# amazon-science/gnn-tail-generalization

Hardware: AMD Instinct MI355X
Metric: teachergnn_fullgraph_train_steps_per_sec (higher is better)
Workload: dtype f32

## Files before the change

gnn-tail-generalization_amd/_lib.py:

```python
import ctypes
import os

import torch

_HERE = os.path.dirname(os.path.abspath(__file__))
LIB_PATH = os.path.join(_HERE, 'lib', 'libcoldbrew_hip.so')

_c_i32p = ctypes.c_void_p
_c_f32p = ctypes.c_void_p
_I64 = ctypes.c_int64
_I32 = ctypes.c_int32
_SZ = ctypes.c_size_t
_P = ctypes.c_void_p


class CsrView(ctypes.Structure):
    _fields_ = [('rowptr', _P), ('col', _P), ('col_flags', _I32), ('n_rows', _I64), ('n_edges', _I64),
                ('hub_threshold', _I32), ('n_hubs', _I32), ('n_chunks', _I32), ('hub_rows', _P), ('hub_chunk_ptr', _P),
                ('ws', _P), ('ws_bytes', _SZ)]


class TrunkStore(ctypes.Structure):
    _fields_ = [('mix_src', _P), ('ld_mix', _I64), ('mix_index', _P), ('c_act', ctypes.c_float), ('c_mix', ctypes.c_float), ('drop_p', ctypes.c_float),
                ('seed', ctypes.c_uint64), ('seed_dev', _P), ('row0', _I64), ('relu_bits', _P), ('bits_relu_only', _I32), ('out_act', _P), ('ld_act', _I64)]


_G = ctypes.POINTER(CsrView)
_S = ctypes.POINTER(TrunkStore)

SIGNATURES = {
    'cb_version': (ctypes.c_int, []),
    'cb_last_error': (ctypes.c_char_p, []),
    'cb_device_status': (ctypes.c_int, []),
    'cb_agg_gemm_handover_selftest': (ctypes.c_int, [_P]),
    'cb_rows_zero_outside_mask_f32': (ctypes.c_int, [_P, _I64, _I64, _I64, _P, _P, _P]),
    'cb_csr_workspace_bytes': (_SZ, [_I64, _I64]),
    'cb_csr_from_coo_i64': (ctypes.c_int, [_P, _P, _I64, _I64, _P, _P, _P, _P, _P, _P, _SZ, _P]),
    'cb_deg_norm_f32': (ctypes.c_int, [_P, _I64, _P, _P]),
    'cb_csr64_from_coo_i64': (ctypes.c_int, [_P, _P, _I64, _I64, _P, _P, _P, _P, _P, _P, _SZ, _P]),
    'cb_csr_rebase_i64': (ctypes.c_int, [_P, _I64, _I64, _P, _P]),
    'cb_deg_norm_i64ptr_f32': (ctypes.c_int, [_P, _I64, _P, _P]),
    'cb_spmm_hub_count': (ctypes.c_int, [_P, _I64, _I32, _P, _P]),
    'cb_spmm_hub_fill_scratch_ints': (_I64, [_I64]),
    'cb_spmm_hub_fill': (ctypes.c_int, [_P, _I64, _I32, _I32, _P, _P, _P, _P]),
    'cb_spmm_workspace_bytes': (_SZ, [_I64, _I64]),
    'cb_spmm_csr_f32': (ctypes.c_int, [_G, _P, _I32, _I64, _I64, _P, _P, _P, ctypes.c_int, _P, _I64, _P, _I64, _P]),
    'cb_dropout_f32': (ctypes.c_int, [_P, _P, _I64, ctypes.c_float, ctypes.c_uint64, _P, _I64, _P]),
    'cb_axpby_f32': (ctypes.c_int, [ctypes.c_float, _P, ctypes.c_float, _P, _P, _I64, _P]),
    'cb_colsum_workspace_bytes': (_SZ, [_I64, _I64]),
    'cb_act_bwd_f32': (ctypes.c_int, [_P, _P, _P, _P, _I64, _I64, _P, _P, _SZ, _P]),
    'cb_reduce_workspace_bytes': (_SZ, []),
    'cb_frobenius_norm_f32': (ctypes.c_int, [_P, _I64, _P, _P, _SZ, _P]),
    'cb_nll_logsoftmax_f32': (ctypes.c_int, [_P, _I64, _P, _P, _I64, _I64, _I64, _P, _P, _P, _SZ, _P]),
    'cb_adam_step_f32': (ctypes.c_int, [_P, _P, _P, _P, _I64, ctypes.c_float, ctypes.c_float, ctypes.c_float,
                                        ctypes.c_float, ctypes.c_float, _I64, _P, _P]),
    'cb_adam_multi_f32': (ctypes.c_int, [_I32, _P, _P, _P, _P, _P, _P, ctypes.c_float, ctypes.c_float, ctypes.c_float, ctypes.c_float,
                                         ctypes.c_float, _I64, _P, _P, _P]),
    'cb_gemm_nn_workspace_bytes': (_SZ, [_I64, _I64]),
    'cb_gemm_nn_splitk_workspace_bytes': (_SZ, [_I64, _I64, _I64]),
    'cb_gemm_nn_f32': (ctypes.c_int, [_P, _I64, _P, _I64, _P, _I64, _I64, _I64, _I64, _P, _P, _I64, _P, ctypes.c_int, _P, _SZ, _P]),
    'cb_gemm_nn_drop2_f32': (ctypes.c_int, [_P, _I64, _P, _I64, _P, _I64, _P, _I64, _I64, _I64, _I64, _P, _P, _I64, _P, ctypes.c_int,
                                            ctypes.c_float, ctypes.c_uint64, _P, _I64, _P, _SZ, _P]),
    'cb_gemm_tn_workspace_bytes': (_SZ, [_I64, _I64, _I64]),
    'cb_gemm_tn_f32': (ctypes.c_int, [_P, _I64, _P, _I64, _P, _P, _I64, _I64, _I64, _P, _SZ, _P]),
    'cb_spmm_csr_fused_f32': (ctypes.c_int, [_G, _P, _P, _I32, _I64, _I64, _P, _P, _P, _I64, _S, _P, _I64, _P]),
    'cb_trunk_layer_bwd_f32': (ctypes.c_int, [_P, _P, _P, _P, ctypes.c_int, _P, ctypes.c_int, _I64, _I64, ctypes.c_float, ctypes.c_uint64,
                                              _P, _I64, ctypes.c_float, ctypes.c_float, _P, ctypes.c_uint64, ctypes.c_float, _P, _P, _P, _SZ, _P]),
    'cb_gemm_nn_bf16out_f32': (ctypes.c_int, [_P, _I64, _P, _I64, _P, _I64, _I64, _I64, _I64, _P, _P, _I64, _P, ctypes.c_int, _P, _SZ, _P]),
    'cb_node_norm_fwd_f32': (ctypes.c_int, [_P, _P, _P, _I64, _I64, ctypes.c_float, ctypes.c_float, ctypes.c_float, _P]),
    'cb_node_norm_bwd_f32': (ctypes.c_int, [_P, _P, _P, _P, _I64, _I64, ctypes.c_float, ctypes.c_float, _P]),
    'cb_colstats_workspace_bytes': (_SZ, [_I64, _I64]),
    'cb_colstats_f32': (ctypes.c_int, [_P, _P, _P, _I64, _I64, _P, _P, _P, _SZ, _P]),
    'cb_col_affine_f32': (ctypes.c_int, [_P, _P, _P, _P, ctypes.c_float, _P, _I64, _I64, _P]),
    'cb_col_bwd_combine_f32': (ctypes.c_int, [_P, _P, _P, _P, _P, _P, ctypes.c_float, ctypes.c_float, _P, _I64, _I64, _P]),
    'cb_topk_replace_workspace_bytes': (_SZ, [_I64, _I64, _I64]),
    'cb_topk_replace_f32': (ctypes.c_int, [_P, _I64, _P, _I64, _I64, _I64, _I64, _I32, _P, _P, _P, _P, _SZ, _P]),
    'cb_gather_rows_f32': (ctypes.c_int, [_P, _I64, _P, _I64, _I64, _P, _P]),
    'cb_gather_rows_bf16_f32': (ctypes.c_int, [_P, _I64, _P, _I64, _I64, _P, _P]),
    'cb_adam_norm_workspace_bytes': (ctypes.c_size_t, [_I32]),
    'cb_adam_multi_norm_f32': (ctypes.c_int, [_I32, _P, _P, _P, _P, _P, _P, _P, ctypes.c_float, ctypes.c_float, ctypes.c_float, ctypes.c_float,
                                              ctypes.c_float, _I64, _P, _P, _P, _SZ, _P]),
    'cb_expand_rows_f32': (ctypes.c_int, [_P, _P, _I64, _I64, ctypes.c_float, _P, _P]),
    'cb_gemm_nn_store_rows_supported': (ctypes.c_int, [_P, _I64, _P, _I64, _P, _I64, _I64, _I64, _I64]),
    'cb_gemm_nn_store_rows_f32': (ctypes.c_int, [_P, _I64, _P, _I64, _P, _I64, _I64, _I64, _I64, _P, _P, _I64, _P, _P, _S, _P, _SZ, _P]),
    'cb_trunk_store_rows_f32': (ctypes.c_int, [_P, _P, _I64, _I64, _S, _P, _P]),
    'cb_agg_gemm_image_bytes': (_SZ, [_I64, _I64]),
    'cb_agg_gemm_image_f32': (ctypes.c_int, [_P, _I64, _I64, _I64, ctypes.c_int, _P, _SZ, _P]),
    'cb_spmm_gemm_f32': (ctypes.c_int, [_G, _P, _I64, _I64, _P, _P, ctypes.c_int, _P, _I64, _P, _I64, _P, _P, _P, _I64, _P, _I64, _P]),
    'cb_spmm_gemm_fused_f32': (ctypes.c_int, [_G, _P, _I64, _P, _I64, _I64, _P, _P, _S, _P, _I64, _I32, _P, _P, _P, _I64, _P, _I64, _P]),
    'cb_agg_gemm_head_image_bytes': (_SZ, [_I64, _I64]),
    'cb_agg_gemm_head_image_f32': (ctypes.c_int, [_P, _I64, _I64, _I64, ctypes.c_int, _P, _SZ, _P]),
    'cb_spmm_gemm_fused_head_f32': (ctypes.c_int, [_G, _P, _I64, _P, _I64, _I64, _P, _P, _S, _P, _I64, _I32, _P, _P, _I64, _P, _I64, _P]),
    'cb_spmm_gemm_store_rows_f32': (ctypes.c_int, [_G, _P, _I64, _I64, _P, _P, _I64, _P, _P, _P, _P, _S, _P, _I64, _P]),
    'cb_spmm_csr_weighted_f32': (ctypes.c_int, [_P, _P, _P, _I64, _I64, _P, _I64, _I64, _P, _P, ctypes.c_int, _P, _I64, _P]),
    'cb_spmm_edge_dot_f32': (ctypes.c_int, [_P, _P, _I64, _I64, _P, _I64, _P, _I64, _I64, _P, _P]),
    'cb_gemm_nn_indrop_supported': (ctypes.c_int, [_P, _I64, _P, _I64, _P, _I64, _P, _I64, _I64, _I64, _I64]),
    'cb_gemm_nn_indrop_drop2_f32': (ctypes.c_int, [_P, _I64, _P, _I64, _P, _I64, _P, _I64, _I64, _I64, _I64, _P, ctypes.c_int, ctypes.c_float,
                                                   ctypes.c_uint64, ctypes.c_float, ctypes.c_uint64, _P, _I64, _P, _P]),
    'cb_gemm_nn_indrop_f32': (ctypes.c_int, [_P, _I64, _P, _I64, _P, _I64, _I64, _I64, _I64, _P, _P, _I64, _P, ctypes.c_int, ctypes.c_float,
                                             ctypes.c_uint64, _P, _I64, _P, _P]),
    'cb_gemm_tn_adrop_supported': (ctypes.c_int, [_P, _I64, _P, _I64, _I64, _I64]),
    'cb_gemm_tn_adrop_f32': (ctypes.c_int, [_P, _I64, _P, _I64, _P, _P, _I64, _I64, _I64, ctypes.c_float, ctypes.c_uint64, _P, _I64, _P, _SZ, _P]),
    'cb_front_image_bytes': (_SZ, [_I64]),
    'cb_front_image_f32': (ctypes.c_int, [_P, _I64, _I64, ctypes.c_int, _P, _SZ, _P]),
    'cb_trunk_front_f32': (ctypes.c_int, [_P, _I64, _I64, _I64, _P, _P, _P, _P, _P, _I64, _P, _I64, _P, _P, _I64, _P, _I64, ctypes.c_float,
                                          ctypes.c_uint64, ctypes.c_uint64, _P, _I64, _P]),
    'cb_gemm_tn_gdrop_supported': (ctypes.c_int, [_P, _I64, _P, _I64, _I64, _I64]),
    'cb_gemm_tn_gdrop_f32': (ctypes.c_int, [_P, _I64, _P, _I64, _P, _I64, _I64, _I64, ctypes.c_float, ctypes.c_uint64, _P, _I64, _P, _SZ, _P]),
    'cb_spmm_csr_lp_f32': (ctypes.c_int, [_G, _P, _I64, _I64, _P, _P, _I64, ctypes.c_float, _P, _P, _I64, _P]),
    'cb_spmm_csr_prop_f32': (ctypes.c_int, [_G, _P, _I64, _I64, _P, _P, _I64, ctypes.c_float, ctypes.c_float, ctypes.c_float, _P, _P, _P, _I64, _P]),
    'cb_cs_workspace_bytes': (_SZ, [_I64, _I64]),
    'cb_cs_residual_init_f32': (ctypes.c_int, [_P, _I64, _P, _P, _I64, _I64, _I64, _P, _P, _P, _P, _P, _SZ, _P]),
    'cb_cs_correct_snap_f32': (ctypes.c_int, [_I32, _P, _I64, _P, _I64, _P, _P, _I64, _I64, _I64, _P, _I64, ctypes.c_float, _P, _P, _I64, _P, _P, _P]),
    'cb_trunk_input_bwd_multi_f32': (ctypes.c_int, [_P, ctypes.c_uint64, _I32, _P, _P, ctypes.c_float, _P, _P, _I64, _I64, ctypes.c_float,
                                                    _P, _I64, _P, _P, _SZ, _P, _P, _P]),
    'cb_trunk_input_bwd_multi_cs_f32': (ctypes.c_int, [_P, ctypes.c_uint64, _I32, _P, _P, ctypes.c_float, _P, _P, _I64, _I64, ctypes.c_float,
                                                       _P, _I64, _P, _P, _SZ, _P, _P, _I32, _P, _P, _P, _P, _P, _SZ, _P]),
    'cb_spmm_csr_store_bwd_f32': (ctypes.c_int, [_G, _P, _I64, _I64, _P, _P, _P, ctypes.c_float, ctypes.c_float, ctypes.c_uint64, _P, _I64, _P, _I64, _P, _I64, _P]),
    'cb_spmm_store_bwd_mix_workspace_bytes': (_SZ, [_I64, _I64, _I64]),
    'cb_spmm_csr_store_bwd_mix_f32': (ctypes.c_int, [_G, _P, _I64, _I64, _P, _P, _P, ctypes.c_float, ctypes.c_float, ctypes.c_uint64, _P, _I64, _P, _I64, _P, _I64,
                                                     _I32, _P, _P, _P, ctypes.c_float, _P, _P, _SZ, _P]),
    'cb_gemm_tn_instage_supported': (ctypes.c_int, [_P, _P, _P, _I64, _I64, _I64]),
    'cb_gemm_tn_instage_workspace_bytes': (_SZ, [_I64, _I64]),
    'cb_gemm_tn_instage_f32': (ctypes.c_int, [_P, _P, _P, _P, _I64, _P, _P, _I64, _I64, ctypes.c_float, ctypes.c_uint64, ctypes.c_float, ctypes.c_uint64, _P, _I64,
                                              _P, _SZ, _P]),
    'cb_trunk_layer_bwd_fold_f32': (ctypes.c_int, [_P, _P, _P, _P, _I64, _I64, ctypes.c_float, ctypes.c_uint64, _P, _I64, ctypes.c_float, ctypes.c_float, _I32, _P, _P, _P,
                                                   _P, _P, _P, _SZ, _I32, _P, ctypes.c_float, _P, _P, _SZ, _P]),
    'cb_trunk_layer_bwd_rows_f32': (ctypes.c_int, [_P, _P, _I64, _P, _P, _P, _I64, ctypes.c_float, ctypes.c_uint64, _P, _I64, ctypes.c_float,
                                                   _P, ctypes.c_uint64, ctypes.c_float, _P, _P, _P, _SZ, _P]),
    'cb_id_count_i64': (ctypes.c_int, [_P, _I64, _I64, _P, _P, _P]),
    'cb_value_hist_i32': (ctypes.c_int, [_P, _I64, _I32, _P, _P, _P]),
    'cb_compact_workspace_bytes': (_SZ, [_I64]),
    'cb_select_range_i32': (ctypes.c_int, [_P, _I64, _I32, _I32, _P, _P, _P, _P, _SZ, _P]),
    'cb_craft_isolation_i64': (ctypes.c_int, [_P, _P, _I64, _P, _I64, _P, _P, _P, _P, _SZ, _P]),
    'cb_symmetrize_workspace_bytes': (_SZ, [_I64, _I64]),
    'cb_symmetrize_i64': (ctypes.c_int, [_P, _P, _I64, _I64, _P, _P, _P, _P, _P, _SZ, _P]),
    'cb_trunk_input_bwd_f32': (ctypes.c_int, [_P, _P, _P, _P, _I64, _I64, ctypes.c_float, ctypes.c_uint64, _P, _I64, _P, _P, _SZ, _P]),
    'cb_ln_gelu_drop_fwd_f32': (ctypes.c_int, [_P, _I64, _I64, _P, _P, ctypes.c_float, ctypes.c_float, ctypes.c_uint64, _P, _P, _P, _P]),
    'cb_ln_gelu_drop_bwd_workspace_bytes': (_SZ, [_I64, _I64]),
    'cb_ln_gelu_drop_bwd_f32': (ctypes.c_int, [_P, _P, _P, _I64, _I64, _P, _P, ctypes.c_float, ctypes.c_uint64, _P, _P, _P, _P, _P, _P, _SZ, _P]),
    'cb_mse_rows_f32': (ctypes.c_int, [_P, _I64, _I64, _P, _I64, _I64, _P, _P, _P, _P, _SZ, _P]),
    'cb_part2_assemble_f32': (ctypes.c_int, [_P, _I64, _P, _P, _I64, _P, _I64, _P, _P]),
    'cb_part2_assemble_bwd_f32': (ctypes.c_int, [_P, _I64, _P, _P, _I64, _I64, _P, _P, _SZ, _P]),
    'cb_ncloss_positions_i64': (ctypes.c_int, [_P, _I64, _I64, _P, _P, _P]),
    'cb_ncloss_row_norms_f32': (ctypes.c_int, [_P, _I64, _I64, _I64, _P, _P, _P]),
    'cb_cosine_scale_f32': (ctypes.c_int, [_P, _I64, _I64, _P, _P]),
    'cb_ncloss_uses_limb_core': (ctypes.c_int, [_P, _I64, _I64]),
    'cb_ncloss_workspace_bytes': (_SZ, [_I64, _I32]),
    'cb_ncloss_fwd_f32': (ctypes.c_int, [_P, _I64, _I64, _I64, ctypes.c_float, _P, _P, _P, _I64, _P, _P, _P, _I32, _P, _P, _P, _P, _P, _P, _P, _P, _SZ, _P]),
    'cb_ncloss_normalize_rows_f32': (ctypes.c_int, [_P, _I64, _I64, _I64, _P, _P, _P]),
    'cb_ncloss_bwd_slab_f32': (ctypes.c_int, [_P, _I64, _I64, _I64, ctypes.c_float, _P, _P, _I64, _I64, _I32, _P, _I64, _P]),
    'cb_ncloss_bwd_finish_f32': (ctypes.c_int, [_P, _I64, _P, _I64, _I64, ctypes.c_float, _P, _P, _P, _P, _P, _P, _P, _P, _I64, _P, _P, _P, _P, _P, _P, _P]),
    'cb_spgemm_offsets_workspace_bytes': (_SZ, [_I64]),
    'cb_spgemm_entry_offsets_i64': (ctypes.c_int, [_P, _I64, _P, _I64, _P, _P, _P, _SZ, _P]),
    'cb_spgemm_chunk_workspace_bytes': (_SZ, [_I64]),
    'cb_spgemm_chunk_count_f32': (ctypes.c_int, [_P, _P, _P, _P, _P, _P, _P, _I64, _I64, _I64, _I64, _I64, _P, _P, _SZ, _P]),
    'cb_spgemm_chunk_emit_f32': (ctypes.c_int, [_P, _SZ, _I64, _I64, _I64, _I64, _I64, _I64, _P, _P, _P, _P]),
    'cb_csr_transpose_workspace_bytes': (_SZ, [_I64]),
    'cb_csr_transpose_f32': (ctypes.c_int, [_P, _P, _P, _I64, _I64, _I64, _P, _P, _P, _P, _SZ, _P]),
    'cb_linkp_max_tries': (ctypes.c_int, []),
    'cb_linkp_valid_counts_i32': (ctypes.c_int, [_P, _P, _I32, _P, _P]),
    'cb_linkp_positives_i32': (ctypes.c_int, [_P, _P, _I32, _P, _I64, _I64, ctypes.c_uint64, _P, _P, _P]),
    'cb_linkp_negatives_i32': (ctypes.c_int, [_P, _P, _I32, _P, _I64, _I64, ctypes.c_uint64, _P, _P, _P, _P]),
    'cb_linkp_loss_fwd_f32': (ctypes.c_int, [_P, _I64, _I64, _I64, _P, _I64, _P, _I64, _P, _P, _P, _P, _P]),
    'cb_linkp_mrr_f32': (ctypes.c_int, [_P, _I64, _P, _I64, _P, _P]),
    'cb_linkp_bwd_workspace_bytes': (_SZ, [_I64, _I64]),
    'cb_linkp_loss_bwd_f32': (ctypes.c_int, [_P, _I64, _I64, _I64, _P, _I64, _P, _I64, _P, _P, _P, _I64, _P, _SZ, _P]),
    'cb_heur_aa_weights_f64': (ctypes.c_int, [_P, _P, _P]),
    'cb_heur_pair_scores_f32': (ctypes.c_int, [_P, _P, _P, _I64, _P, _P, _P]),
    'cb_heur_pair_scores_width_f32': (ctypes.c_int, [_P, _P, _P, _I64, _I32, _P, _P, _P]),
    'cb_rank_counts_workspace_bytes': (_SZ, [_I64, _I64]),
    'cb_rank_counts_f32': (ctypes.c_int, [_P, _I64, _P, _I64, _P, _P, _P, _P, _SZ, _P]),
    'cb_pair_gemm_nn_supported': (ctypes.c_int, [_P, _I64, _P, _I64, _I64, _I64]),
    'cb_pair_gemm_nn_f32': (ctypes.c_int, [_P, _I64, _I64, _P, _I64, _P, _I64, _P, _I64, _P, _I64, _I64, _I64, _P, ctypes.c_int, ctypes.c_float,
                                           ctypes.c_uint64, _P, _I64, _P, _P]),
    'cb_pair_dot_f32': (ctypes.c_int, [_P, _I64, _I64, _I64, _P, _I64, _P, _P, _P]),
    'cb_pair_scatter_workspace_bytes': (_SZ, [_I64]),
    'cb_pair_scatter_f32': (ctypes.c_int, [_P, _I64, _I64, _I64, _P, _I64, _P, _I64, _P, _I64, _P, _SZ, _P]),
    'cb_rank_loss_workspace_bytes': (_SZ, []),
    'cb_rank_loss_fwd_f32': (ctypes.c_int, [_I32, _P, _I64, _P, _I64, _P, _P, _P, _SZ, _P]),
    'cb_rank_loss_bwd_f32': (ctypes.c_int, [_I32, _P, _I64, _P, _I64, _P, _P, _P, _P, _P]),
    'cb_sage_image_bytes': (_SZ, [ctypes.c_int]),
    'cb_sage_image_f32': (ctypes.c_int, [_P, _I64, _P, _I64, ctypes.c_int, _P, _SZ, _P]),
    'cb_sage_layer_supported': (ctypes.c_int, [_I64, _I64, _I32, _P, _I64, _P, _I64, _P, _I64, _P, _I64]),
    'cb_sage_layer_f32': (ctypes.c_int, [_P, _P, _I64, _P, _I64, _P, _P, _P, _P, ctypes.c_int, ctypes.c_float, ctypes.c_uint64, _P, _I64, _P, _I64, _I32,
                                         _P, _I64, _P]),
}

_lib = None


class HipExtensionError(RuntimeError):
    pass


def load():
    global _lib
    if _lib is not None:
        return _lib
    if not os.path.isfile(LIB_PATH):
        raise HipExtensionError(
            f'{LIB_PATH} not found: the HIP extension is required (no CPU fallback). '
            'Build it with `python __graft_entry__.py` or `make -C gnn-tail-generalization_amd/csrc`.')
    lib = ctypes.CDLL(LIB_PATH)
    for name, (res, args) in SIGNATURES.items():
        fn = getattr(lib, name)
        fn.restype = res
        fn.argtypes = args
# ... 69 lines not shown
```

gnn-tail-generalization_amd/csrc/cb_front.hip:

```cpp
#include <type_traits>

#include "cb_common.h"
#include "cb_limb_core.h"
#include "cb_philox.h"
#include "cb_tile_gemm.h"
#include "cb_trunk_store.h"

namespace cb {

struct FrontArgs {
  const float* x;
  int64_t ld_x;
  const uint4* image_in;
  const float* bias_in;
  const uint4* image_0;
  const float* rowscale;
  const float* addend;
  int64_t ld_add;
  float* x0;
  int64_t ld_x0;
  unsigned long long* bits;
  float* x0_drop;
  int64_t ld_drop;
  float* z0;
  int64_t ld_z;
  int64_t M;
  uint32_t thresh;
  float keep_scale;
  uint64_t seed_x, seed_x0;
  const uint64_t* seed_dev;
  int64_t row0;
  int n_tiles;
};

template <int NS1, bool DROP>
__global__ void __launch_bounds__(256, 2) k_front(FrontArgs fa) {
  constexpr int K1 = 16 * NS1, LDX = K1 + 4, NV = kTM * K1 / 4 / 256;
  static_assert(NV >= 1 && kTM * LDX <= kTM * kTLD, "x tile must fit the region of the X0 tile");
  static_assert(NV == NS1 && NS1 <= 8, "mask draws: one quad per K step, P0's bits in one word");
  __shared__ __attribute__((aligned(16))) float tile[kTM * kTLD];
  constexpr int kScratch = 2 * RowOperand<kTM>::BYTES > 4 * 8 * kCLD * 4 ? 2 * RowOperand<kTM>::BYTES : 4 * 8 * kCLD * 4;
  __shared__ __attribute__((aligned(16))) char scratch[kScratch];
  float (*cstrip)[8 * kCLD] = reinterpret_cast<float (*)[8 * kCLD]>(scratch);
  __shared__ float rs_tile[2][kTM];
  const int t = threadIdx.x, lane = t & 63, w = __builtin_amdgcn_readfirstlane(t >> 6);
  const uint64_t sx = fa.seed_dev ? fa.seed_x + *fa.seed_dev : fa.seed_x, s0 = fa.seed_dev ? fa.seed_x0 + *fa.seed_dev : fa.seed_x0;
  float4 xr[NV];
  auto load_x = [&](int tile_id) {
    const int64_t m0 = (int64_t)tile_id * kTM;
#pragma unroll
    for (int j = 0; j < NV; ++j) {
      const int idx = t + 256 * j, row = idx / (K1 / 4), c4 = idx % (K1 / 4);
      const int64_t m = m0 + row;
      xr[j] = (tile_id < fa.n_tiles && m < fa.M) ? *reinterpret_cast<const float4*>(fa.x + m * fa.ld_x + 4 * c4) : make_float4(0.f, 0.f, 0.f, 0.f);
    }
  };
  float rs_next = 1.f;
  auto load_rs = [&](int tile_id) {
    const int64_t m = (int64_t)tile_id * kTM + t;
    rs_next = (t < kTM && fa.rowscale && tile_id < fa.n_tiles && m < fa.M) ? fa.rowscale[m] : 1.f;
  };
  float bvec[4] = {0.f, 0.f, 0.f, 0.f};
  if (fa.bias_in) {
#pragma unroll
    for (int i = 0; i < 4; ++i) bvec[i] = fa.bias_in[4 * lane + i];
  }
  load_rs(blockIdx.x);
  load_x(blockIdx.x);
  uint32_t kx = 0;
  uint64_t k3 = 0;
  int64_t qx = 0, q3 = 0;
  auto aim_x = [&](int tile_id) { qx = (fa.row0 + (int64_t)tile_id * kTM) * (K1 / 4) + t; };
  auto aim_3 = [&](int tile_id) { q3 = (fa.row0 + (int64_t)tile_id * kTM + 16 * w) * (kND / 4) + lane; };
  auto draw_x = [&](int) {
    uint64_t seed = sx;
    asm volatile("" : "+s"(seed));
    kx = (kx >> 4) | (keep4_bits(seed, qx, fa.thresh) << 28);
    qx += 256;
    asm volatile("" : "+v"(kx));
  };
  auto draw_3 = [&](int) {
    uint64_t seed = s0;
    asm volatile("" : "+s"(seed));
    k3 = (k3 >> 4) | ((uint64_t)keep4_bits(seed, q3, fa.thresh) << 60);
    q3 += kND / 4;
    asm volatile("" : "+v"(k3));
  };
  if constexpr (DROP) {
    aim_x(blockIdx.x);
    aim_3(blockIdx.x);
#pragma unroll 1
    for (int s = 0; s < 16; ++s) {
      if (s < NS1) draw_x(s);
      draw_3(s);
    }
  }
  int par = 0;
  for (int tile_id = blockIdx.x; tile_id < fa.n_tiles; tile_id += gridDim.x, par ^= 1) {
    const int64_t m0 = (int64_t)tile_id * kTM;
#pragma unroll
    for (int j = 0; j < NV; ++j) {
      const int idx = t + 256 * j, row = idx / (K1 / 4), c4 = idx % (K1 / 4);
      float v[4] = {xr[j].x, xr[j].y, xr[j].z, xr[j].w};
      if constexpr (DROP) {
#pragma unroll
        for (int i = 0; i < 4; ++i) v[i] = mul_rounded(v[i], (kx >> (32 - 4 * NV + 4 * j + i)) & 1u ? fa.keep_scale : 0.f);
      }
      *reinterpret_cast<float4*>(tile + row * LDX + 4 * c4) = make_float4(v[0], v[1], v[2], v[3]);
    }
    if constexpr (DROP) aim_x(tile_id + (int)gridDim.x);
    if (t < kTM) rs_tile[par][t] = rs_next;
    __syncthreads();
    f32x16 acc[2][2];
    if constexpr (DROP) tile_times_image_coop<NS1, LDX, 1>(tile, scratch, fa.image_in, w, lane, t, acc, draw_x);
    else tile_times_image_coop<NS1, LDX, 1>(tile, scratch, fa.image_in, w, lane, t, acc);
    {
      const int l31 = lane & 31, lh = lane >> 5;
#pragma unroll
      for (int i = 0; i < 2; ++i)
#pragma unroll
        for (int j = 0; j < 2; ++j)
#pragma unroll
          for (int reg = 0; reg < 16; ++reg)
            tile[(32 * i + (reg & 3) + 8 * (reg >> 2) + 4 * lh) * kTLD + 64 * w + 32 * j + l31] = acc[i][j][reg];
    }
    __syncthreads();
#pragma unroll 4
    for (int r = 0; r < 16; ++r) {
      const int row = 16 * w + r;
      const int64_t m = m0 + row;
      float* tp = tile + row * kTLD + 4 * lane;
      const float4 v = *reinterpret_cast<const float4*>(tp);
      float o[4] = {v.x, v.y, v.z, v.w};
#pragma unroll
      for (int i = 0; i < 4; ++i) o[i] = fmaxf(o[i] + bvec[i], 0.f);
      float xd[4] = {o[0], o[1], o[2], o[3]};
      if constexpr (DROP) {
#pragma unroll
        for (int i = 0; i < 4; ++i) xd[i] = o[i] * ((uint32_t)k3 >> i & 1u ? fa.keep_scale : 0.f);
        k3 >>= 4;
      }
      *reinterpret_cast<float4*>(tp) = make_float4(xd[0], xd[1], xd[2], xd[3]);
      if (m < fa.M) {
        store_stream4(fa.x0 + m * fa.ld_x0 + 4 * lane, o);
        if (fa.bits) {
          const bool pos[4] = {o[0] > 0.f, o[1] > 0.f, o[2] > 0.f, o[3] > 0.f};
          write_row_mask_words(fa.bits + m * 4, lane, pos);
        }
        if (fa.x0_drop) store_stream4(fa.x0_drop + m * fa.ld_drop + 4 * lane, xd);
      }
    }
    __syncthreads();
    if constexpr (DROP) aim_3(tile_id + (int)gridDim.x);
    if constexpr (DROP) tile_times_image_coop<kNS, kTLD, 1>(tile, scratch, fa.image_0, w, lane, t, acc, draw_3);
    else tile_times_image_coop<kNS, kTLD, 1>(tile, scratch, fa.image_0, w, lane, t, acc);
    load_rs(tile_id + gridDim.x);
    load_x(tile_id + gridDim.x);
    auto z0_epilogue = [&](auto HAS_ADD) {
      acc_rows_through_strip(acc, cstrip[w], w, lane, [&](int row, int n, const float4& v) {
        const int64_t m = m0 + row;
        if (m < fa.M) {
          const float rs = rs_tile[par][row];
          float ad[4] = {0.f, 0.f, 0.f, 0.f};
          if constexpr (decltype(HAS_ADD)::value) {
            const float4 a4 = *reinterpret_cast<const float4*>(fa.addend + m * fa.ld_add + n);
            ad[0] = a4.x; ad[1] = a4.y; ad[2] = a4.z; ad[3] = a4.w;
          }
          const float zero_bias = 0.f;
          float o[4] = {v.x, v.y, v.z, v.w};
#pragma unroll
          for (int e = 0; e < 4; ++e) o[e] = o[e] * rs + ad[e] + zero_bias;
          store_stream4(fa.z0 + m * fa.ld_z + n, o);
        }
      });
    };
    if (fa.addend) z0_epilogue(std::true_type{});
    else z0_epilogue(std::false_type{});
  }
}

}

using namespace cb;

extern "C" size_t cb_front_image_bytes(int64_t K) {
  if (K != 64 && K != 128) return 0;
  return (size_t)(K / 16) * kNT * 3 * 64 * sizeof(uint4);
}

extern "C" int cb_front_image_f32(const float* W, int64_t ld, int64_t K, int transpose, void* image, size_t image_bytes, void* stream) {
  CB_CHECK_ARG(cb_front_image_bytes(K) > 0, CB_E_INVALID, "cb_front_image_f32: K must be 64 or 128 (got %lld)", (long long)K);
  CB_CHECK_ARG(W && image && ld >= (transpose ? K : kND), CB_E_INVALID, "cb_front_image_f32: null pointer / bad leading dimension");
  CB_CHECK_ARG(image_bytes >= cb_front_image_bytes(K) && aligned16(image), CB_E_WORKSPACE, "cb_front_image_f32: image buffer too small or misaligned");
  const int64_t sk = transpose ? 1 : ld, sn = transpose ? ld : 1;
  const int ns = (int)(K / 16);
  hipLaunchKernelGGL(k_weight_image, dim3(ns * kNT * 64 / 256), dim3(256), 0, (hipStream_t)stream, W, sk, sn, (uint4*)image, ns);
  CB_LAUNCH_CHECK();
  return CB_OK;
}

extern "C" int cb_trunk_front_f32(const float* x, int64_t ld_x, int64_t M, int64_t K, const void* image_in, const float* bias_in, const void* image_0,
                                  const float* rowscale, const float* addend, int64_t ld_add, float* x0, int64_t ld_x0, uint64_t* relu_bits,
                                  float* x0_drop, int64_t ld_drop, float* z0, int64_t ld_z, float drop_p, uint64_t seed_x, uint64_t seed_x0,
                                  const uint64_t* seed_dev, int64_t row0, void* stream) {
  CB_CHECK_ARG(M >= 0 && cb_front_image_bytes(K) > 0 && drop_p >= 0.f && drop_p < 1.f && row0 >= 0, CB_E_INVALID,
               "cb_trunk_front_f32: bad size (K must be 64 or 128; hidden width 256) or p");
  CB_CHECK_ARG(M < ((int64_t)1 << 31) * kTM / 2, CB_E_RANGE, "cb_trunk_front_f32: size out of range");
  if (M == 0) return CB_OK;
  CB_CHECK_ARG(x && image_in && image_0 && x0 && z0, CB_E_INVALID, "cb_trunk_front_f32: null pointer");
  CB_CHECK_ARG(aligned16(x) && ld_x % 4 == 0 && ld_x >= K && aligned16(image_in) && aligned16(image_0) && aligned16(x0) && ld_x0 % 4 == 0 && ld_x0 >= kND &&
                   aligned16(z0) && ld_z % 4 == 0 && ld_z >= kND && (!addend || (aligned16(addend) && ld_add % 4 == 0 && ld_add >= kND)) &&
                   (!x0_drop || (aligned16(x0_drop) && ld_drop % 4 == 0 && ld_drop >= kND)) && (!relu_bits || (uintptr_t)relu_bits % 8 == 0),
               CB_E_INVALID, "cb_trunk_front_f32: 16-byte aligned rows required");
  FrontArgs fa{x, ld_x, (const uint4*)image_in, bias_in, (const uint4*)image_0, rowscale, addend, ld_add, x0, ld_x0, (unsigned long long*)relu_bits,
               x0_drop, ld_drop, z0, ld_z, M};
  fa.thresh = drop_p > 0.f ? dropout_threshold(drop_p) : 0u;
  fa.keep_scale = 1.f / (1.f - drop_p);
  fa.seed_x = seed_x; fa.seed_x0 = seed_x0; fa.seed_dev = seed_dev; fa.row0 = row0;
  fa.n_tiles = (int)((M + kTM - 1) / kTM);
  int dev = 0, n_cu = 0;
  if (hipGetDevice(&dev) != hipSuccess || hipDeviceGetAttribute(&n_cu, hipDeviceAttributeMultiprocessorCount, dev) != hipSuccess || n_cu <= 0) n_cu = 256;
  const int blocks = fa.n_tiles < 2 * n_cu ? fa.n_tiles : 2 * n_cu;
  const dim3 grid((unsigned)blocks), blk(256);
  hipStream_t st = (hipStream_t)stream;
  if (K == 64 && fa.thresh) hipLaunchKernelGGL((k_front<4, true>), grid, blk, 0, st, fa);
  else if (K == 64) hipLaunchKernelGGL((k_front<4, false>), grid, blk, 0, st, fa);
  else if (fa.thresh) hipLaunchKernelGGL((k_front<8, true>), grid, blk, 0, st, fa);
  else hipLaunchKernelGGL((k_front<8, false>), grid, blk, 0, st, fa);
  CB_LAUNCH_CHECK();
  return CB_OK;
}
```

gnn-tail-generalization_amd/csrc/cb_gemm.hip:

```cpp
#include <stdlib.h>

#include "cb_common.h"
#include "cb_gemm_core.h"
#include "cb_gemm_limb.h"

namespace cb {

template <int WM, int WN, bool ALIGNED, bool OUT_BF16, int BKT = BK, int WTN = 2>
__global__ void __launch_bounds__(256) k_gemm_nn(const float* __restrict__ A, int64_t lda, const float* __restrict__ B, int64_t ldb,
                                                 void* __restrict__ Cv, int64_t ldc, int64_t M, int N, int K, GemmEpilogue ep,
                                                 int n_row_blocks, int n_col_blocks, int c_vec_ok, int k_chunk) {
  using T = Tile<WM, WN, BKT, WTN>;
  if (k_chunk) {
    const int k0 = blockIdx.y * k_chunk;
    A += k0;
    B += (int64_t)k0 * ldb;
    Cv = reinterpret_cast<float*>(Cv) + (int64_t)blockIdx.y * M * ldc;
    K = min(k_chunk, K - k0);
  }
  constexpr int BM = T::BM, BN = T::BN, LDA = T::LDA, LDB = T::LDB;
  __shared__ __attribute__((aligned(16))) float smem[T::SMEM_FLOATS];
  auto As = [&](int b) { return smem + b * (BKT * LDA); };
  auto Bs = [&](int b) { return smem + 2 * BKT * LDA + b * (BKT * LDB); };
  const int per_group = 8 * n_col_blocks;
// ... 324 lines not shown
                                               int64_t K) {
  return use_limb3() && N == 256 && M > 0 && limb3_nn_eligible(A, lda, B, ldb, N, K) && aligned16(C) && ldc % 4 == 0 ? 1 : 0;
}

extern "C" int cb_gemm_nn_store_rows_f32(const float* A, int64_t lda, const float* B, int64_t ldb, float* C, int64_t ldc, int64_t M, int64_t N, int64_t K,
                                         const float* rowscale, const float* addend, int64_t ld_add, const float* bias, const int64_t* row_index,
                                         const cb_trunk_store* store, void* ws, size_t ws_bytes, void* stream) {
  CB_CHECK_ARG(M >= 0 && N == 256 && K > 0, CB_E_INVALID, "cb_gemm_nn_store_rows_f32: bad size (N must be 256)");
  CB_CHECK_ARG(K < (1 << 24) && (M + 63) / 64 < (1 << 24), CB_E_RANGE, "cb_gemm_nn_store_rows_f32: size out of range");
  if (M == 0) return CB_OK;
  CB_CHECK_ARG(A && B && C && row_index && lda >= K && ldb >= N && ldc >= N && (!addend || ld_add >= N), CB_E_INVALID,
               "cb_gemm_nn_store_rows_f32: null pointer or leading dimension too small");
  const int rcs = check_trunk_store("cb_gemm_nn_store_rows_f32", store, N);
  if (rcs != CB_OK) return rcs;
  CB_CHECK_ARG(cb_gemm_nn_store_rows_supported(A, lda, B, ldb, C, ldc, M, N, K) && (!addend || (aligned16(addend) && ld_add % 4 == 0)), CB_E_INVALID,
               "cb_gemm_nn_store_rows_f32: shape / alignment outside the fused form (cb_gemm_nn_store_rows_supported)");
  GemmEpilogue ep{rowscale, addend, ld_add, bias, 1, nullptr, 0, 0u, 1.f, 0ull, nullptr, 0, 0};
  ep.row_ids = row_index; ep.st = make_trunk_store(*store);
  return launch_nn_limb3(A, lda, B, ldb, C, ldc, M, N, K, ep, false, (hipStream_t)stream, ws, ws_bytes);
}

extern "C" int cb_gemm_tn_f32(const float* A, int64_t lda, const float* G, int64_t ldg, const float* rowscale, float* C, int64_t M,
                              int64_t K1, int64_t K2, void* ws, size_t ws_bytes, void* stream) {
  CB_CHECK_ARG(M >= 0 && K1 >= 0 && K2 >= 0, CB_E_INVALID, "cb_gemm_tn_f32: negative size");
  CB_CHECK_ARG(K1 < (1 << 20) && K2 < (1 << 20), CB_E_RANGE, "cb_gemm_tn_f32: size out of range");
  if (K1 == 0 || K2 == 0) return CB_OK;
  CB_CHECK_ARG(C && (M == 0 || (A && G)) && lda >= K1 && ldg >= K2, CB_E_INVALID, "cb_gemm_tn_f32: null pointer or bad ld");
  hipStream_t st = (hipStream_t)stream;
  if (M == 0) {
    CB_HIP(hipMemsetAsync(C, 0, (size_t)K1 * K2 * sizeof(float), st));
    return CB_OK;
  }
  CB_CHECK_ARG(ws && ws_bytes >= cb_gemm_tn_workspace_bytes(M, K1, K2), CB_E_WORKSPACE, "cb_gemm_tn_f32: workspace too small");
  int bm, bn;
  tn_tile(K1, K2, bm, bn);
  if (bm == 64) return launch_tn<1, 4>(A, lda, G, ldg, rowscale, C, M, K1, K2, (float*)ws, st);
  if (bm == 256) return launch_tn<4, 1>(A, lda, G, ldg, rowscale, C, M, K1, K2, (float*)ws, st);
  return launch_tn<2, 2>(A, lda, G, ldg, rowscale, C, M, K1, K2, (float*)ws, st);
}

extern "C" int cb_gemm_tn_gdrop_supported(const float* A, int64_t lda, const float* G, int64_t ldg, int64_t K1, int64_t K2) {
  return use_limb3() && K2 % 4 == 0 && limb3_tn_eligible(A, lda, G, ldg, K1, K2) ? 1 : 0;
}

extern "C" int cb_gemm_tn_gdrop_f32(const float* A, int64_t lda, const float* G, int64_t ldg, float* C, int64_t M, int64_t K1, int64_t K2,
                                    float g_drop_p, uint64_t g_seed, const uint64_t* seed_dev, int64_t row0, void* ws, size_t ws_bytes,
                                    void* stream) {
  CB_CHECK_ARG(M >= 0 && K1 >= 0 && K2 >= 0 && g_drop_p > 0.f && g_drop_p < 1.f && row0 >= 0, CB_E_INVALID, "cb_gemm_tn_gdrop_f32: bad size or p");
  CB_CHECK_ARG(K1 < (1 << 20) && K2 < (1 << 20), CB_E_RANGE, "cb_gemm_tn_gdrop_f32: size out of range");
  if (K1 == 0 || K2 == 0) return CB_OK;
  CB_CHECK_ARG(C && (M == 0 || (A && G)) && lda >= K1 && ldg >= K2, CB_E_INVALID, "cb_gemm_tn_gdrop_f32: null pointer or bad ld");
  hipStream_t st = (hipStream_t)stream;
  if (M == 0) {
    CB_HIP(hipMemsetAsync(C, 0, (size_t)K1 * K2 * sizeof(float), st));
    return CB_OK;
  }
  CB_CHECK_ARG(cb_gemm_tn_gdrop_supported(A, lda, G, ldg, K1, K2), CB_E_INVALID, "cb_gemm_tn_gdrop_f32: operands outside the three-limb path");
  CB_CHECK_ARG(ws && ws_bytes >= cb_gemm_tn_workspace_bytes(M, K1, K2), CB_E_WORKSPACE, "cb_gemm_tn_gdrop_f32: workspace too small");
  const DropSpec gd{dropout_threshold(g_drop_p), 1.f / (1.f - g_drop_p), g_seed, seed_dev, row0, K2};
  int bm, bn;
  tn_tile(K1, K2, bm, bn);
  if (bm == 64) return launch_tn<1, 4>(A, lda, G, ldg, nullptr, C, M, K1, K2, (float*)ws, st, &gd);
  if (bm == 256) return launch_tn<4, 1>(A, lda, G, ldg, nullptr, C, M, K1, K2, (float*)ws, st, &gd);
  return launch_tn<2, 2>(A, lda, G, ldg, nullptr, C, M, K1, K2, (float*)ws, st, &gd);
}

static inline int instage_splits(int64_t M) { return tn_splits(M, 2); }

extern "C" int cb_gemm_tn_instage_supported(const float* g, const float* mfold, const float* X, int64_t ldx, int64_t M, int64_t K2) {
  return use_limb3() && K2 > 64 && K2 <= 128 && K2 % 4 == 0 && ldx % 4 == 0 && ldx >= K2 && ldx < (1 << 22) && aligned16(g) && aligned16(mfold) && aligned16(X) && M > 0 &&
                 instage_splits(M) >= 256
             ? 1
             : 0;
}

extern "C" size_t cb_gemm_tn_instage_workspace_bytes(int64_t M, int64_t K2) {
  if (M <= 0 || K2 <= 0) return 0;
  return (size_t)instage_splits(M) * (size_t)256 * (size_t)(K2 + 1) * sizeof(float);
}

extern "C" int cb_gemm_tn_instage_f32(const float* g, const float* mfold, const uint64_t* x0_bits, const float* X, int64_t ldx, float* C, float* colsum, int64_t M,
                                      int64_t K2, float g_drop_p, uint64_t g_seed, float x_drop_p, uint64_t x_seed, const uint64_t* seed_dev, int64_t row0, void* ws,
                                      size_t ws_bytes, void* stream) {
  CB_CHECK_ARG(M > 0 && K2 > 0 && g_drop_p > 0.f && g_drop_p < 1.f && x_drop_p > 0.f && x_drop_p < 1.f && row0 >= 0, CB_E_INVALID,
               "cb_gemm_tn_instage_f32: bad size or p (both dropouts must be active)");
  CB_CHECK_ARG(g && mfold && x0_bits && X && C && colsum && (uintptr_t)x0_bits % 8 == 0, CB_E_INVALID, "cb_gemm_tn_instage_f32: null or misaligned pointer");
  CB_CHECK_ARG(cb_gemm_tn_instage_supported(g, mfold, X, ldx, M, K2), CB_E_INVALID, "cb_gemm_tn_instage_f32: shape / alignment outside the fused form (cb_gemm_tn_instage_supported)");
  CB_CHECK_ARG(ws && ws_bytes >= cb_gemm_tn_instage_workspace_bytes(M, K2), CB_E_WORKSPACE, "cb_gemm_tn_instage_f32: workspace too small");
  hipStream_t st = (hipStream_t)stream;
  const int nsplit = instage_splits(M);
  int64_t rows_per_split = (M + nsplit - 1) / nsplit;
  rows_per_split = (rows_per_split + 31) / 32 * 32;
  const DropSpec xd{dropout_threshold(x_drop_p), 1.f / (1.f - x_drop_p), x_seed, seed_dev, row0, K2};
  const DropSpec gd{dropout_threshold(g_drop_p), 1.f / (1.f - g_drop_p), g_seed, seed_dev, row0, 256};
  float* partial = (float*)ws;
  float* cs_partial = partial + (size_t)nsplit * 256 * K2;
  const int rc = launch_tn_instage(g, mfold, x0_bits, X, ldx, partial, cs_partial, M, K2, nsplit, rows_per_split, st, xd, gd);
  if (rc != CB_OK) return rc;
  const int64_t n = 256 * K2;
  hipLaunchKernelGGL(k_sum_partials, dim3((unsigned)((n + 255) / 256)), dim3(256), 0, st, (const float*)partial, nsplit, n, C);
  CB_LAUNCH_CHECK();
  hipLaunchKernelGGL(k_sum_partials, dim3(1), dim3(256), 0, st, (const float*)cs_partial, nsplit, (int64_t)256, colsum);
  CB_LAUNCH_CHECK();
  return CB_OK;
}

extern "C" int cb_gemm_nn_indrop_f32(const float* A, int64_t lda, const float* B, int64_t ldb, float* C, int64_t ldc, int64_t M, int64_t N, int64_t K,
                                     const float* rowscale, const float* addend, int64_t ld_add, const float* bias, int relu, float a_drop_p,
                                     uint64_t a_seed, const uint64_t* seed_dev, int64_t row0, uint64_t* relu_bits, void* stream) {
  CB_CHECK_ARG(M >= 0 && N >= 0 && K >= 0 && a_drop_p > 0.f && a_drop_p < 1.f && row0 >= 0, CB_E_INVALID, "cb_gemm_nn_indrop_f32: bad size or p");
  CB_CHECK_ARG(!relu_bits || (N == 256 && relu && (uintptr_t)relu_bits % 8 == 0), CB_E_INVALID,
               "cb_gemm_nn_indrop_f32: mask words of the ReLU exist for N == 256 with relu only");
  CB_CHECK_ARG(N < (1 << 24) && K < (1 << 24) && (M + 63) / 64 < (1 << 24), CB_E_RANGE, "cb_gemm_nn_indrop_f32: size out of range");
  if (M == 0 || N == 0) return CB_OK;
  CB_CHECK_ARG(C && A && B && lda >= K && ldb >= N && ldc >= N && (!addend || ld_add >= N), CB_E_INVALID, "cb_gemm_nn_indrop_f32: null pointer or bad ld");
  CB_CHECK_ARG(cb_gemm_nn_indrop_supported(A, lda, B, ldb, C, ldc, C, ldc, M, N, K) && (!addend || (aligned16(addend) && ld_add % 4 == 0)), CB_E_INVALID,
               "cb_gemm_nn_indrop_f32: shape / alignment outside the fused form (cb_gemm_nn_indrop_supported)");
  GemmEpilogue ep{rowscale, addend, ld_add, bias, relu, nullptr, 0, 0u, 1.f, 0ull, nullptr, 0, gemm_nt_store(M, N)};
  ep.adrop = DropSpec{dropout_threshold(a_drop_p), 1.f / (1.f - a_drop_p), a_seed, seed_dev, row0, K};
  ep.relu_bits_out = (unsigned long long*)relu_bits;
  return launch_nn_limb3(A, lda, B, ldb, C, ldc, M, N, K, ep, false, (hipStream_t)stream, nullptr, 0);
}

extern "C" int cb_gemm_tn_adrop_supported(const float* A, int64_t lda, const float* G, int64_t ldg, int64_t K1, int64_t K2) {
  int bm, bn;
  tn_tile(K1, K2, bm, bn);
  return use_limb3() && K1 % 4 == 0 && bm == 128 && limb3_tn_eligible(A, lda, G, ldg, K1, K2) ? 1 : 0;
}

extern "C" int cb_gemm_tn_adrop_f32(const float* A, int64_t lda, const float* G, int64_t ldg, const float* rowscale, float* C, int64_t M, int64_t K1,
                                    int64_t K2, float a_drop_p, uint64_t a_seed, const uint64_t* seed_dev, int64_t row0, void* ws, size_t ws_bytes,
                                    void* stream) {
  CB_CHECK_ARG(M >= 0 && K1 >= 0 && K2 >= 0 && a_drop_p > 0.f && a_drop_p < 1.f && row0 >= 0, CB_E_INVALID, "cb_gemm_tn_adrop_f32: bad size or p");
  CB_CHECK_ARG(K1 < (1 << 20) && K2 < (1 << 20), CB_E_RANGE, "cb_gemm_tn_adrop_f32: size out of range");
  if (K1 == 0 || K2 == 0) return CB_OK;
  CB_CHECK_ARG(C && (M == 0 || (A && G)) && lda >= K1 && ldg >= K2, CB_E_INVALID, "cb_gemm_tn_adrop_f32: null pointer or bad ld");
  hipStream_t st = (hipStream_t)stream;
  if (M == 0) {
    CB_HIP(hipMemsetAsync(C, 0, (size_t)K1 * K2 * sizeof(float), st));
    return CB_OK;
  }
  CB_CHECK_ARG(cb_gemm_tn_adrop_supported(A, lda, G, ldg, K1, K2), CB_E_INVALID, "cb_gemm_tn_adrop_f32: operands outside the three-limb 128-row tile path");
  CB_CHECK_ARG(ws && ws_bytes >= cb_gemm_tn_workspace_bytes(M, K1, K2), CB_E_WORKSPACE, "cb_gemm_tn_adrop_f32: workspace too small");
  const DropSpec ad{dropout_threshold(a_drop_p), 1.f / (1.f - a_drop_p), a_seed, seed_dev, row0, K1};
  return launch_tn<2, 2>(A, lda, G, ldg, rowscale, C, M, K1, K2, (float*)ws, st, nullptr, &ad);
}
```

gnn-tail-generalization_amd/csrc/cb_gemm_core.h:

```cpp
#pragma once
#include "cb_common.h"
#include "cb_philox.h"
#include "cb_trunk_store.h"

namespace cb {

typedef float f32x16 __attribute__((ext_vector_type(16)));

constexpr int BK = 16;

struct DropSpec {
  uint32_t thresh;
  float scale;
  uint64_t seed;
  const uint64_t* seed_dev;
  int64_t row0;
  int64_t width;
};

struct GemmEpilogue {
  const float* rowscale;
  const float* addend;
  int64_t ld_add;
  const float* bias;
  int relu;
  float* out2;
  int64_t ld_out2;
  uint32_t thresh;
  float keep_scale;
  uint64_t seed;
  const uint64_t* seed_dev;
  int64_t row0;
  int nt_store;
  DropSpec adrop;
  unsigned long long* relu_bits_out;
  const int64_t* row_ids;
  TrunkStore st;
};

template <int WM, int WN, int BKT = BK, int WTN = 2>
struct Tile {
  static constexpr int BM = 64 * WM, BN = 32 * WTN * WN, LDA = BM + 4, LDB = BN + 4;
  static constexpr int SMEM_FLOATS = 2 * BKT * (LDA + LDB);
  static_assert(WM * WN == 4, "four wavefronts per block");
  static_assert(32 * LDB <= SMEM_FLOATS, "epilogue staging (32 rows) must fit the operand buffers");
};

template <int LDA, int LDB, int BKT, int WTN>
__device__ __forceinline__ void mfma_tile_step(const float* __restrict__ As, const float* __restrict__ Bs, int wr, int wc,
                                               int lane, f32x16 (&acc)[2][WTN]) {
  const int l31 = lane & 31, kh = lane >> 5;
  const float* ar = As + kh * LDA + wr * 64 + l31;
  const float* br = Bs + kh * LDB + wc * (32 * WTN) + l31;
  float a[2], b[WTN];
  a[0] = ar[0]; a[1] = ar[32];
#pragma unroll
  for (int j = 0; j < WTN; ++j) b[j] = br[32 * j];
#pragma unroll
  for (int kk = 0; kk < BKT; kk += 2) {
    float na[2] = {0.f, 0.f}, nb[WTN];
#pragma unroll
    for (int j = 0; j < WTN; ++j) nb[j] = 0.f;
    if (kk + 2 < BKT) {
      na[0] = ar[(kk + 2) * LDA];
      na[1] = ar[(kk + 2) * LDA + 32];
#pragma unroll
      for (int j = 0; j < WTN; ++j) nb[j] = br[(kk + 2) * LDB + 32 * j];
    }
#pragma unroll
    for (int i = 0; i < 2; ++i)
#pragma unroll
      for (int j = 0; j < WTN; ++j) acc[i][j] = __builtin_amdgcn_mfma_f32_32x32x2f32(a[i], b[j], acc[i][j], 0, 0, 0);
    a[0] = na[0]; a[1] = na[1];
#pragma unroll
    for (int j = 0; j < WTN; ++j) b[j] = nb[j];
  }
}

template <int BMT, int BKT>
struct RowFrag {
  float v[BMT * BKT / 1024][4];
};
template <bool ALIGNED, int BMT, int BKT>
__device__ __forceinline__ void load_rowmajor(RowFrag<BMT, BKT>& f, const float* __restrict__ A, int64_t lda, int64_t m0, int64_t M,
                                              int k0, int K, int t) {
  constexpr int TPR = BKT / 4, RPP = 256 / TPR;
  const int k = k0 + (t % TPR) * 4;
#pragma unroll
  for (int j = 0; j < BMT / RPP; ++j) {
    const int64_t m = m0 + t / TPR + RPP * j;
    if (ALIGNED && m < M && k + 4 <= K) {
      const float4 x = *reinterpret_cast<const float4*>(A + m * lda + k);
      f.v[j][0] = x.x; f.v[j][1] = x.y; f.v[j][2] = x.z; f.v[j][3] = x.w;
    } else {
#pragma unroll
      for (int i = 0; i < 4; ++i) f.v[j][i] = (m < M && k + i < K) ? A[m * lda + k + i] : 0.f;
    }
  }
}
template <int BMT, int BKT>
// ... 220 lines not shown
```

gnn-tail-generalization_amd/csrc/cb_gemm_limb.hip:

```cpp
#include <utility>

#include "cb_common.h"
#include "cb_gemm_core.h"
#include "cb_gemm_limb.h"
#include "cb_limb_core.h"

namespace cb {

template <int WM, int WN, int WTN = 2, int PD = 1>
struct LTile {
  static constexpr int BM = 64 * WM, BN = 32 * WTN * WN;
  static constexpr int MINW = (WM == 2 && WTN == 2 && PD < 3 ? 3 : 2);
  static constexpr int NTHR = 64 * WM * WN;
  static_assert(WM * WN == 4 || WM * WN == 8, "four or eight wavefronts per block");
};

template <int WM, int WN, bool OUT_BF16, int WTN = 2, int PD = 1, int EPI = 0, bool ADROP = false>
__global__ void __launch_bounds__(256, (LTile<WM, WN, WTN, PD>::MINW)) k_gemm_nn_l3(const float* __restrict__ A, int64_t lda,
                                                                                 const float* __restrict__ B, int64_t ldb,
                                                                                 void* __restrict__ Cv, int64_t ldc, int64_t M, int N,
                                                                                 int K, GemmEpilogue ep, int n_row_blocks,
                                                                                 int n_col_blocks, int c_vec_ok) {
  using T = LTile<WM, WN, WTN>;
  using OA = RowOperand<T::BM, ADROP>;
  using OB = ColOperand<T::BN, false>;
  constexpr int BM = T::BM, BN = T::BN;
  constexpr int SMEM = 2 * (OA::BYTES + OB::BYTES);
  static_assert(32 * (BN + 4) * 4 <= SMEM, "epilogue staging must fit");
  __shared__ __attribute__((aligned(16))) char smem[SMEM];
  const int per_group = 8 * n_col_blocks;
  const int grp = blockIdx.x / per_group, r = blockIdx.x % per_group;
  const int row_blk = grp * 8 + (r & 7), col_blk = r >> 3;
  if (row_blk >= n_row_blocks) return;
  const int64_t m0 = (int64_t)row_blk * BM;
  const int n0 = col_blk * BN;
  const int t = threadIdx.x, lane = t & 63, w = t >> 6, wr = w / WN, wc = w % WN;

  f32x16 acc[2][WTN];
  zero_acc_n<WTN>(acc);
  OA oa;
  OB ob;
  oa.init(lda, M - m0, t);
  if constexpr (ADROP) oa.set_drop(ep.adrop, m0, K, t);
  ob.init(ldb, N - n0, t);
  const uint32_t aaddr[2] = {OA::frag_addr(wr * 64, lane), OA::frag_addr(wr * 64 + 32, lane)};
  uint32_t baddr[WTN];
#pragma unroll
  for (int j = 0; j < WTN; ++j) baddr[j] = OB::frag_addr(wc * (32 * WTN) + 32 * j, lane);
  limb_k_loop<WTN, PD, OA, OB>(oa, ob, smem, A + m0 * lda, KS, lda, B + n0, (int64_t)KS * ldb, ldb, nullptr, K, aaddr, baddr, acc, t);
  nn_epilogue<WM, WN, WTN, OUT_BF16, EPI>(acc, reinterpret_cast<float*>(smem), Cv, ldc, m0, n0, M, N, ep, c_vec_ok, t);
}

template <int WM, int WN, bool SCALED, int WTN = 2, int PD = 1, bool GDROP = false, bool ADROP = false>
__global__ void __launch_bounds__((LTile<WM, WN, WTN, PD>::NTHR), (LTile<WM, WN, WTN, PD>::MINW)) k_gemm_tn_l3(const float* __restrict__ A, int64_t lda,
                                                                                 const float* __restrict__ G, int64_t ldg,
                                                                                 const float* __restrict__ rowscale,
                                                                                 float* __restrict__ partial, int64_t M, int K1, int K2,
                                                                                 int64_t rows_per_split, int tiles_j, int n_tiles,
                                                                                 int nsplit, DropSpec gd) {
  using T = LTile<WM, WN, WTN>;
  using OA = ColOperand<T::BM, false, ADROP, T::NTHR>;
  using OB = ColOperand<T::BN, SCALED, GDROP, T::NTHR>;
  constexpr int BM = T::BM, BN = T::BN;
  __shared__ __attribute__((aligned(16))) char smem[2 * (OA::BYTES + OB::BYTES)];
  const int b = blockIdx.x;
  const int tile = (b >> 3) % n_tiles, split = (b & 7) + 8 * (b / (8 * n_tiles));
  if (split >= nsplit) return;
  const int i0 = (tile / tiles_j) * BM, j0 = (tile % tiles_j) * BN;
  const int64_t r_begin = (int64_t)split * rows_per_split;
  const int64_t r_end = min(M, r_begin + rows_per_split);
  const int t = threadIdx.x, lane = t & 63, w = t >> 6, wr = w / WN, wc = w % WN;

  f32x16 acc[2][WTN];
  zero_acc_n<WTN>(acc);
  OA oa;
  OB ob;
  oa.init(lda, K1 - i0, t);
  ob.init(ldg, K2 - j0, t);
  if constexpr (GDROP) ob.set_drop(gd, r_begin, r_end - r_begin, j0, t);
  if constexpr (ADROP) oa.set_drop(gd, r_begin, r_end - r_begin, i0, t);
  const uint32_t aaddr[2] = {OA::frag_addr(wr * 64, lane), OA::frag_addr(wr * 64 + 32, lane)};
  uint32_t baddr[WTN];
#pragma unroll
  for (int j = 0; j < WTN; ++j) baddr[j] = OB::frag_addr(wc * (32 * WTN) + 32 * j, lane);
  limb_k_loop<WTN, PD, OA, OB>(oa, ob, smem, A + r_begin * lda + i0, (int64_t)KS * lda, lda, G + r_begin * ldg + j0, (int64_t)KS * ldg, ldg,
                           SCALED ? rowscale + r_begin : nullptr, r_end - r_begin, aaddr, baddr, acc, t);
  const int l31 = lane & 31, lh = lane >> 5;
  float* P = partial + (int64_t)split * K1 * K2;
#pragma unroll
  for (int ti = 0; ti < 2; ++ti)
#pragma unroll
    for (int tj = 0; tj < WTN; ++tj) {
      const int n = j0 + wc * (32 * WTN) + tj * 32 + l31;
      if (n >= K2) continue;
#pragma unroll
      for (int reg = 0; reg < 16; ++reg) {
        const int m = i0 + wr * 64 + ti * 32 + (reg & 3) + 8 * (reg >> 2) + 4 * lh;
        if (m < K1) P[(int64_t)m * K2 + n] = acc[ti][tj][reg];
      }
    }
}

__global__ void __launch_bounds__(512, 2) k_gemm_tn_instage(const float* __restrict__ g, const float* __restrict__ mfold,
                                                            const unsigned long long* __restrict__ x0_bits, const float* __restrict__ X, int64_t ldx,
                                                            float* __restrict__ partial, float* __restrict__ cs_partial, int64_t M, int K2,
                                                            int64_t rows_per_split, int nsplit, DropSpec xd, DropSpec gd) {
  using T = LTile<4, 2, 2>;
  using OA = ColOperandInStage<T::NTHR>;
  using OB = ColOperand<T::BN, false, true, T::NTHR>;
  constexpr int K1 = 256;
  __shared__ __attribute__((aligned(16))) char smem[2 * (OA::BYTES + OB::BYTES)];
  const int split = blockIdx.x;
  if (split >= nsplit) return;
  const int64_t r_begin = (int64_t)split * rows_per_split;
  const int64_t r_end = min(M, r_begin + rows_per_split);
  const int t = threadIdx.x, lane = t & 63, w = t >> 6, wr = w / 2, wc = w % 2;

  f32x16 acc[2][2];
  zero_acc_n<2>(acc);
  OA oa;
  OB ob;
  oa.init(K1, K1, t);
  ob.init(ldx, K2, t);
  oa.set_stage(g, mfold, x0_bits + r_begin * 4, gd, r_begin, r_end - r_begin, t);
  ob.set_drop(xd, r_begin, r_end - r_begin, 0, t);
  const uint32_t aaddr[2] = {OA::frag_addr(wr * 64, lane), OA::frag_addr(wr * 64 + 32, lane)};
  uint32_t baddr[2];
#pragma unroll
  for (int j = 0; j < 2; ++j) baddr[j] = OB::frag_addr(wc * 64 + 32 * j, lane);
  limb_k_loop<2, 1, OA, OB>(oa, ob, smem, g + r_begin * K1, (int64_t)KS * K1, K1, X + r_begin * ldx, (int64_t)KS * ldx, ldx, nullptr, r_end - r_begin, aaddr, baddr,
                            acc, t);
  const int l31 = lane & 31, lh = lane >> 5;
  float* P = partial + (int64_t)split * K1 * K2;
#pragma unroll
  for (int ti = 0; ti < 2; ++ti)
#pragma unroll
    for (int tj = 0; tj < 2; ++tj) {
      const int n = wc * 64 + tj * 32 + l31;
      if (n >= K2) continue;
#pragma unroll
      for (int reg = 0; reg < 16; ++reg) {
        const int m = wr * 64 + ti * 32 + (reg & 3) + 8 * (reg >> 2) + 4 * lh;
        P[(int64_t)m * K2 + n] = acc[ti][tj][reg];
      }
    }
  float* red = reinterpret_cast<float*>(smem);
#pragma unroll
  for (int i = 0; i < 4; ++i) red[w * 256 + lane * 4 + i] = oa.cs[i];
  __syncthreads();
  if (t < 256) {
    float s = 0.f;
#pragma unroll
    for (int j = 0; j < 8; ++j) s += red[j * 256 + t];
    cs_partial[(int64_t)split * 256 + t] = s;
  }
}

int launch_tn_instage(const float* g, const float* mfold, const uint64_t* x0_bits, const float* X, int64_t ldx, float* partial, float* cs_partial, int64_t M, int64_t K2,
                      int nsplit, int64_t rows_per_split, hipStream_t st, const DropSpec& xd, const DropSpec& gd) {
  hipLaunchKernelGGL(k_gemm_tn_instage, dim3((unsigned)nsplit), dim3(512), 0, st, g, mfold, (const unsigned long long*)x0_bits, X, ldx, partial, cs_partial, M, (int)K2,
                     rows_per_split, nsplit, xd, gd);
  CB_LAUNCH_CHECK();
  return CB_OK;
}

template <int WM, int WN, bool OUT_BF16, int WTN = 2>
static int launch_nn_l3_t(const float* A, int64_t lda, const float* B, int64_t ldb, void* C, int64_t ldc, int64_t M, int64_t N,
                          int64_t K, GemmEpilogue ep, hipStream_t st, void* ws = nullptr, size_t ws_bytes = 0) {
  using T = LTile<WM, WN, WTN>;
  const int nrb = (int)((M + T::BM - 1) / T::BM), ncb = (int)((N + T::BN - 1) / T::BN);
  const int64_t groups = (nrb + 7) / 8;
  const int c_vec_ok = ((uintptr_t)C % (OUT_BF16 ? 8 : 16) == 0) && ldc % 4 == 0 && (!ep.addend || (aligned16(ep.addend) && ep.ld_add % 4 == 0));
  const dim3 grid((unsigned)(groups * 8 * ncb));
  if constexpr (!OUT_BF16 && WM == 2 && WTN == 4) {
    if (ep.out2) {
      if (ep.adrop.thresh)
        hipLaunchKernelGGL((k_gemm_nn_l3<WM, WN, false, WTN, 1, 1, true>), grid, dim3(256), 0, st, A, lda, B, ldb, C, ldc, M, (int)N, (int)K, ep,
                           nrb, ncb, c_vec_ok);
      else
        hipLaunchKernelGGL((k_gemm_nn_l3<WM, WN, false, WTN, 1, 1>), grid, dim3(256), 0, st, A, lda, B, ldb, C, ldc, M, (int)N, (int)K, ep, nrb,
                           ncb, c_vec_ok);
      CB_LAUNCH_CHECK();
      return CB_OK;
    }
    if (ep.row_ids) {
      hipLaunchKernelGGL((k_gemm_nn_l3<WM, WN, false, WTN, 1, 2>), grid, dim3(256), 0, st, A, lda, B, ldb, C, ldc, M, (int)N, (int)K, ep, nrb, ncb, c_vec_ok);
      CB_LAUNCH_CHECK();
      return CB_OK;
    }
    if (ep.adrop.thresh) {
      hipLaunchKernelGGL((k_gemm_nn_l3<WM, WN, false, WTN, 1, 0, true>), grid, dim3(256), 0, st, A, lda, B, ldb, C, ldc, M, (int)N, (int)K, ep, nrb,
                         ncb, c_vec_ok);
      CB_LAUNCH_CHECK();
      return CB_OK;
    }
  }
  CB_CHECK_ARG(!ep.adrop.thresh, CB_E_INVALID, "NN contraction with operand dropout: wide fp32 tile only (check cb_gemm_nn_indrop_supported first)");
  hipLaunchKernelGGL((k_gemm_nn_l3<WM, WN, OUT_BF16, WTN, 1>), grid, dim3(256), 0, st, A, lda, B, ldb, C, ldc, M, (int)N, (int)K, ep, nrb, ncb,
                     c_vec_ok);
  CB_LAUNCH_CHECK();
  return CB_OK;
}

bool limb3_nn_eligible(const float* A, int64_t lda, const float* B, int64_t ldb, int64_t N, int64_t K) {
  return aligned16(A) && aligned16(B) && lda % 4 == 0 && ldb % 4 == 0 && K % 4 == 0 && N % 4 == 0 && K > 0 && lda < (1 << 22) && ldb < (1 << 22);
}

bool limb3_nn_dual_eligible(const float* A, int64_t lda, const float* B, int64_t ldb, const float* C, int64_t ldc, const float* C2, int64_t ldc2,
                            int64_t M, int64_t N, int64_t K, const GemmEpilogue& ep) {
  return N > 128 && ((M + 127) / 128) * ((N + 255) / 256) >= 256 && limb3_nn_eligible(A, lda, B, ldb, N, K) && aligned16(C) && aligned16(C2) && ldc % 4 == 0 && ldc2 % 4 == 0 &&
         (!ep.addend || (aligned16(ep.addend) && ep.ld_add % 4 == 0));
}

size_t limb3_nn_workspace_bytes(int64_t, int64_t) { return 0; }

int launch_nn_limb3(const float* A, int64_t lda, const float* B, int64_t ldb, void* C, int64_t ldc, int64_t M, int64_t N, int64_t K,
                    const GemmEpilogue& ep, bool out_bf16, hipStream_t st, void* ws, size_t ws_bytes) {
  if (N <= 64) {
    return out_bf16 ? launch_nn_l3_t<4, 1, true>(A, lda, B, ldb, C, ldc, M, N, K, ep, st)
                    : launch_nn_l3_t<4, 1, false>(A, lda, B, ldb, C, ldc, M, N, K, ep, st);
  }
  const bool fills = ((M + 127) / 128) * ((N + 255) / 256) >= 256 || ep.out2 || ep.adrop.thresh || ep.row_ids;
  if (N > 128 && fills)
    return out_bf16 ? launch_nn_l3_t<2, 2, true, 4>(A, lda, B, ldb, C, ldc, M, N, K, ep, st, ws, ws_bytes)
                    : launch_nn_l3_t<2, 2, false, 4>(A, lda, B, ldb, C, ldc, M, N, K, ep, st, ws, ws_bytes);
  return out_bf16 ? launch_nn_l3_t<2, 2, true>(A, lda, B, ldb, C, ldc, M, N, K, ep, st, ws, ws_bytes)
                  : launch_nn_l3_t<2, 2, false>(A, lda, B, ldb, C, ldc, M, N, K, ep, st, ws, ws_bytes);
}

template <int WM, int WN, int WTN = 2>
static void launch_tn_l3_t(const float* A, int64_t lda, const float* G, int64_t ldg, const float* rowscale, float* partial, int64_t M,
                           int64_t K1, int64_t K2, int nsplit, int64_t rows_per_split, hipStream_t st, const DropSpec& gd, const DropSpec& ad) {
  using T = LTile<WM, WN, WTN>;
  const int ti = (int)((K1 + T::BM - 1) / T::BM), tj = (int)((K2 + T::BN - 1) / T::BN);
  const dim3 grid((unsigned)(((nsplit + 7) / 8) * 8 * ti * tj));
#define CB_TN_LAUNCH(SC_, GD_, AD_)                                                                                                  \
  hipLaunchKernelGGL((k_gemm_tn_l3<WM, WN, SC_, WTN, 1, GD_, AD_>), grid, dim3(T::NTHR), 0, st, A, lda, G, ldg, rowscale, partial, M, (int)K1, \
                     (int)K2, rows_per_split, tj, ti * tj, nsplit, gd.thresh ? gd : ad)
  if (gd.thresh) CB_TN_LAUNCH(false, true, false);
  else if (ad.thresh) {
    if constexpr (WM == 2 && WN == 2 && WTN == 2) { if (rowscale) CB_TN_LAUNCH(true, false, true); else CB_TN_LAUNCH(false, false, true); }
  } else if (rowscale) CB_TN_LAUNCH(true, false, false);
  else CB_TN_LAUNCH(false, false, false);
#undef CB_TN_LAUNCH
}

bool limb3_tn_eligible(const float* A, int64_t lda, const float* G, int64_t ldg, int64_t K1, int64_t K2) {
  return aligned16(A) && aligned16(G) && lda % 4 == 0 && ldg % 4 == 0 && K1 % 4 == 0 && K2 % 4 == 0 && lda < (1 << 22) && ldg < (1 << 22);
}

int launch_tn_limb3(const float* A, int64_t lda, const float* G, int64_t ldg, const float* rowscale, float* partial, int64_t M,
                    int64_t K1, int64_t K2, int bm, int nsplit, int64_t rows_per_split, hipStream_t st, const DropSpec* gdrop, const DropSpec* adrop) {
  const DropSpec gd = gdrop ? *gdrop : DropSpec{};
  const DropSpec ad = adrop ? *adrop : DropSpec{};
  CB_CHECK_ARG(!gd.thresh || (!rowscale && gd.width % 4 == 0 && !ad.thresh), CB_E_INVALID,
               "TN contraction: dropout of the G operand needs width %% 4 == 0, no row scale and no dropout of A");
  CB_CHECK_ARG(!ad.thresh || (ad.width % 4 == 0 && bm == 128), CB_E_INVALID, "TN contraction: dropout of the A operand needs width %% 4 == 0 and the 128-row tile");
  if (bm == 64) launch_tn_l3_t<1, 4>(A, lda, G, ldg, rowscale, partial, M, K1, K2, nsplit, rows_per_split, st, gd, ad);
  else if (bm == 256) launch_tn_l3_t<4, 1>(A, lda, G, ldg, rowscale, partial, M, K1, K2, nsplit, rows_per_split, st, gd, ad);
  else {
    if (!ad.thresh && !gd.thresh && K1 == 256 && K2 == 256 && nsplit >= 256) {
      launch_tn_l3_t<4, 2, 4>(A, lda, G, ldg, rowscale, partial, M, K1, K2, nsplit, rows_per_split, st, gd, ad);
      CB_LAUNCH_CHECK();
      return CB_OK;
    }
    if (gd.thresh && !ad.thresh && !rowscale && K1 == 256 && K2 <= 128 && K2 > 64 && nsplit >= 256) {
      launch_tn_l3_t<4, 2, 2>(A, lda, G, ldg, rowscale, partial, M, K1, K2, nsplit, rows_per_split, st, gd, ad);
      CB_LAUNCH_CHECK();
      return CB_OK;
    }
    if (!ad.thresh && K2 > 128 && ((K1 + 127) / 128) * ((K2 + 255) / 256) * nsplit >= 256) launch_tn_l3_t<2, 2, 4>(A, lda, G, ldg, rowscale, partial, M, K1, K2, nsplit, rows_per_split, st, gd, ad);
    else launch_tn_l3_t<2, 2>(A, lda, G, ldg, rowscale, partial, M, K1, K2, nsplit, rows_per_split, st, gd, ad);
  }
  CB_LAUNCH_CHECK();
  return CB_OK;
}

}
```

gnn-tail-generalization_amd/csrc/cb_limb_core.h:

```cpp
#pragma once
#include <utility>

#include "cb_common.h"
#include "cb_gemm_core.h"
#include "cb_philox.h"

namespace cb {

typedef __bf16 bf16x8 __attribute__((ext_vector_type(8)));

typedef float f32x2 __attribute__((ext_vector_type(2)));
typedef __bf16 bf16x2 __attribute__((ext_vector_type(2)));
__device__ __forceinline__ uint32_t cvt_pk_bf16(float x0, float x1) {
  const f32x2 v = {x0, x1};
  return __builtin_bit_cast(uint32_t, __builtin_convertvector(v, bf16x2));
}
__device__ __forceinline__ void split3x2(float a0, float a1, uint32_t& hi, uint32_t& mid, uint32_t& lo) {
  hi = cvt_pk_bf16(a0, a1);
  const float r0 = a0 - __uint_as_float(hi << 16), r1 = a1 - __uint_as_float(hi & 0xffff0000u);
  mid = cvt_pk_bf16(r0, r1);
  const float s0 = r0 - __uint_as_float(mid << 16), s1 = r1 - __uint_as_float(mid & 0xffff0000u);
  lo = cvt_pk_bf16(s0, s1);
}

// ... 47 lines not shown
      const bool in = row + 64 * j < rows_left;
      rmask |= in ? (1u << j) : 0u;
      voff[j] = in ? (uint32_t)((row + 64 * j) * ld + kq * 4) : 0u;
    }
  }
  template <int J>
  __device__ __forceinline__ void load(float4 (&f)[NV], const float* __restrict__ base, int64_t , int64_t k_left, const float*,
                                       int t) const {
    f[J] = *reinterpret_cast<const float4*>(base + ((t & 3) * 4 < k_left ? voff[J] : 0u));
  }
  template <int J>
  __device__ __forceinline__ void stage(const float4 (&f)[NV], char* __restrict__ S, int64_t k_left, int t) const {
    const bool live = ((rmask >> J) & 1) && (t & 3) * 4 < k_left;
    float v[4] = {live ? f[J].x : 0.f, live ? f[J].y : 0.f, live ? f[J].z : 0.f, live ? f[J].w : 0.f};
    if constexpr (DROP) {
      float mk[4];
      keep4(dseed, (dbase[J] + (dK - k_left)) >> 2, dthresh, dscale, mk);
#pragma unroll
      for (int i = 0; i < 4; ++i) v[i] = mul_rounded(v[i], mk[i]);
    }
    uint2 pl[3];
    split4(v, pl);
#pragma unroll
    for (int p = 0; p < 3; ++p) *reinterpret_cast<uint2*>(S + p * PLANE + woff + J * (64 * 32)) = pl[p];
  }
  static __device__ __forceinline__ uint32_t frag_addr(int r0, int lane) {
    const int row = r0 + (lane & 31);
    return row * 32 + (((lane >> 5) ^ ((row >> 3) & 1)) << 4);
  }
  static __device__ __forceinline__ bf16x8 frag(const char* __restrict__ S, uint32_t addr, int plane) {
    return __builtin_bit_cast(bf16x8, *reinterpret_cast<const uint4*>(S + plane * PLANE + addr));
  }
};

template <int R>
struct PairRowOperand {
  static constexpr int PLANE = R * 32, BYTES = 3 * PLANE, NV = R / 64;
  static_assert(NV >= 1, "tile rows");
  int32_t nu[NV], nv[NV];
  uint32_t woff;
  static constexpr bool HAS_SC = false;
  float sc[1];
  float4 fv[NV];
  static __device__ __forceinline__ bool pair_of(const int32_t* __restrict__ pairs, int64_t S, int64_t rows_left, int64_t N, int row, int& u, int& v, bool& in) {
    in = row < rows_left;
    u = in ? pairs[row] : 0;
    v = in ? pairs[S + row] : 0;
    return in && u >= 0 && u < N && v >= 0 && v < N;
  }
  __device__ __forceinline__ void init(const int32_t* __restrict__ pairs, int64_t S, int64_t rows_left, int64_t N, int t) {
    const int row = t >> 2, kq = t & 3;
    woff = row * 32 + (((kq >> 1) ^ ((row >> 3) & 1)) << 4) + ((kq & 1) << 3);
#pragma unroll
    for (int j = 0; j < NV; ++j) {
      int u, v;
      bool in;
      const bool ok = pair_of(pairs, S, rows_left, N, row + 64 * j, u, v, in);
      nu[j] = ok ? u : -1;
      nv[j] = ok ? v : 0;
    }
  }
  template <int J>
  __device__ __forceinline__ void load(float4 (&f)[NV], const float* __restrict__ base, int64_t ld, int64_t k_left, const float*, int t) {
    const int kq4 = (t & 3) * 4 < k_left ? (t & 3) * 4 : 0;
    f[J] = *reinterpret_cast<const float4*>(base + ((int64_t)(nu[J] < 0 ? 0 : nu[J]) * ld + kq4));
    fv[J] = *reinterpret_cast<const float4*>(base + ((int64_t)nv[J] * ld + kq4));
  }
  template <int J>
  __device__ __forceinline__ void stage(const float4 (&f)[NV], char* __restrict__ S, int64_t k_left, int t) const {
    const bool live = nu[J] >= 0 && (t & 3) * 4 < k_left;
    const float a[4] = {f[J].x, f[J].y, f[J].z, f[J].w}, b[4] = {fv[J].x, fv[J].y, fv[J].z, fv[J].w};
    float v[4];
#pragma unroll
    for (int i = 0; i < 4; ++i) v[i] = live ? mul_rounded(a[i], b[i]) : 0.f;
    uint2 pl[3];
    split4(v, pl);
#pragma unroll
    for (int p = 0; p < 3; ++p) *reinterpret_cast<uint2*>(S + p * PLANE + woff + J * (64 * 32)) = pl[p];
  }
  static __device__ __forceinline__ uint32_t frag_addr(int r0, int lane) { return RowOperand<R>::frag_addr(r0, lane); }
  static __device__ __forceinline__ bf16x8 frag(const char* __restrict__ S, uint32_t addr, int plane) { return RowOperand<R>::frag(S, addr, plane); }
};

template <int C, bool SCALED, bool DROP = false, int NT = 256>
struct ColOperand {
  static constexpr int ROWB = C * 2, PLANE = 16 * ROWB, BYTES = 3 * PLANE;
  static constexpr int TPR = C / 4, KPP = NT / TPR, NV = 16 / KPP;
  static_assert(KPP >= 4 && KPP % 4 == 0 && NV >= 1, "staging map: whole swizzle groups of k rows per pass");
  static constexpr int NC = C / 32;
  static_assert(NC == 2 || NC == 4 || NC == 8, "tile widths 64 / 128 / 256");
  static __device__ __forceinline__ int swz(int k) { return NC == 2 ? ((k >> 1) & 1) : (k & 3); }
  uint32_t voff[NV];
  uint32_t woff;
  bool cok;
  static constexpr bool HAS_SC = SCALED;
  float sc[SCALED ? NV : 1];
  uint64_t dseed;
  uint32_t dthresh;
  float dscale;
  int64_t drow, dtot, dwidth;
  int dcol;
  __device__ __forceinline__ void set_drop(const DropSpec& d, int64_t r_begin, int64_t total, int j0, int t) {
    dseed = d.seed_dev ? d.seed + *d.seed_dev : d.seed;
    dthresh = d.thresh;
    dscale = d.scale;
    drow = d.row0 + r_begin + t / TPR;
    dtot = total;
    dwidth = d.width;
    dcol = j0 + (t % TPR) * 4;
  }
  __device__ __forceinline__ void init(int64_t ld, int cols_left, int t) {
    const int k = t / TPR, nq = t % TPR;
    cok = nq * 4 < cols_left;
#pragma unroll
    for (int j = 0; j < NV; ++j) voff[j] = (uint32_t)((k + KPP * j) * ld + (cok ? nq * 4 : 0));
    woff = k * ROWB + ((((nq >> 3) ^ swz(k)) & (NC - 1)) << 6) + ((nq & 7) << 3);
  }
  template <int J>
  __device__ __forceinline__ void load(float4 (&f)[NV], const float* __restrict__ base, int64_t , int64_t k_left,
                                       const float* __restrict__ kscale, int t) {
    const int k = t / TPR + KPP * J;
    const bool kin = k < k_left;
    f[J] = *reinterpret_cast<const float4*>(base + (kin ? voff[J] : 0u));
    if constexpr (SCALED) sc[J] = kscale[kin ? k : 0];
  }
  template <int J>
  __device__ __forceinline__ void stage(const float4 (&f)[NV], char* __restrict__ S, int64_t k_left, int t) const {
    const bool live = cok && t / TPR + KPP * J < k_left;
    const float m = SCALED ? sc[SCALED ? J : 0] : 1.f;
    float v[4] = {live ? f[J].x * m : 0.f, live ? f[J].y * m : 0.f, live ? f[J].z * m : 0.f, live ? f[J].w * m : 0.f};
    if constexpr (DROP) {
      static_assert(!SCALED, "dropout of a row-scaled operand is not needed anywhere");
      float mk[4];
      keep4(dseed, ((drow + KPP * J + (dtot - k_left)) * dwidth + dcol) >> 2, dthresh, dscale, mk);
#pragma unroll
      for (int i = 0; i < 4; ++i) v[i] = mul_rounded(v[i], mk[i]);
    }
    uint2 pl[3];
    split4(v, pl);
#pragma unroll
    for (int p = 0; p < 3; ++p) *reinterpret_cast<uint2*>(S + p * PLANE + woff + J * (KPP * ROWB)) = pl[p];
  }
  static __device__ __forceinline__ uint32_t frag_addr(int c0, int lane) {
    const int L = lane & 15, k = 8 * (lane >> 5) + (L >> 2);
    return k * ROWB + ((((c0 >> 5) ^ swz(k)) & (NC - 1)) << 6) + (((lane >> 4) & 1) << 5) + ((L & 3) << 3);
  }
  static __device__ __forceinline__ bf16x8 frag(const char* __restrict__ S, uint32_t addr, int plane) {
    const char* q = S + plane * PLANE + addr;
    const s16x4 lo = __builtin_amdgcn_ds_read_tr16_b64_v4i16((lds_s16x4*)(q));
    const s16x4 hi = __builtin_amdgcn_ds_read_tr16_b64_v4i16((lds_s16x4*)(q + 4 * ROWB));
    typedef short s16x8 __attribute__((ext_vector_type(8)));
    const s16x8 v = __builtin_shufflevector(lo, hi, 0, 1, 2, 3, 4, 5, 6, 7);
    return __builtin_bit_cast(bf16x8, v);
  }
};

template <int NT = 512>
struct ColOperandInStage {
  static constexpr int C = 256;
  static constexpr int ROWB = C * 2, PLANE = 16 * ROWB, BYTES = 3 * PLANE;
  static constexpr int TPR = C / 4, KPP = NT / TPR, NV = 16 / KPP;
  static_assert(TPR == 64 && KPP >= 4 && KPP % 4 == 0 && NV >= 1, "one wavefront per k row");
  static constexpr int NC = C / 32;
  static __device__ __forceinline__ int swz(int k) { return k & 3; }
  uint32_t voff[NV];
  uint32_t woff;
  bool cok;
  static constexpr bool HAS_SC = false;
  float sc[1];
  int64_t mdelta;
  const unsigned long long* bits;
  float4 fm[NV];
  unsigned long long bw[NV][4];
  uint64_t dseed;
  uint32_t dthresh;
  float dscale;
  int64_t drow, dtot, dwidth;
  int dcol, kw;
  float cs[4];
  __device__ __forceinline__ void set_stage(const float* g, const float* mfold, const unsigned long long* bits_block, const DropSpec& d, int64_t r_begin, int64_t total,
                                            int t) {
    mdelta = mfold - g;
    bits = bits_block;
    dseed = d.seed_dev ? d.seed + *d.seed_dev : d.seed;
    dthresh = d.thresh;
    dscale = d.scale;
    kw = __builtin_amdgcn_readfirstlane(t / TPR);
    drow = d.row0 + r_begin + kw;
    dtot = total;
    dwidth = d.width;
    dcol = (t % TPR) * 4;
#pragma unroll
    for (int i = 0; i < 4; ++i) cs[i] = 0.f;
  }
  __device__ __forceinline__ void init(int64_t ld, int cols_left, int t) {
    const int k = t / TPR, nq = t % TPR;
    cok = nq * 4 < cols_left;
#pragma unroll
    for (int j = 0; j < NV; ++j) voff[j] = (uint32_t)((k + KPP * j) * ld + (cok ? nq * 4 : 0));
    woff = k * ROWB + ((((nq >> 3) ^ swz(k)) & (NC - 1)) << 6) + ((nq & 7) << 3);
  }
  template <int J>
  __device__ __forceinline__ void load(float4 (&f)[NV], const float* __restrict__ base, int64_t , int64_t k_left, const float* __restrict__, int ) {
    const int k = kw + KPP * J;
    const bool kin = k < k_left;
    const float* p = base + (kin ? voff[J] : 0u);
    f[J] = *reinterpret_cast<const float4*>(p);
    fm[J] = *reinterpret_cast<const float4*>(p + mdelta);
    const unsigned long long* b = bits + ((dtot - k_left) + (kin ? k : 0)) * 4;
#pragma unroll
    for (int i = 0; i < 4; ++i) bw[J][i] = b[i];
  }
  template <int J>
  __device__ __forceinline__ void stage(const float4 (&f)[NV], char* __restrict__ S, int64_t k_left, int t) {
    const bool live = cok && kw + KPP * J < k_left;
    const int lane = t & 63;
    float mk[4];
    keep4(dseed, ((drow + KPP * J + (dtot - k_left)) * dwidth + dcol) >> 2, dthresh, dscale, mk);
    const float gv[4] = {f[J].x, f[J].y, f[J].z, f[J].w}, mv[4] = {fm[J].x, fm[J].y, fm[J].z, fm[J].w};
    float v[4];
#pragma unroll
    for (int i = 0; i < 4; ++i) {
      const float tsum = mul_rounded(gv[i], mk[i]) + mv[i];
      v[i] = (live && ((bw[J][i] >> lane) & 1ull)) ? tsum : 0.f;
      cs[i] += v[i];
    }
    uint2 pl[3];
    split4(v, pl);
#pragma unroll
    for (int p = 0; p < 3; ++p) *reinterpret_cast<uint2*>(S + p * PLANE + woff + J * (KPP * ROWB)) = pl[p];
  }
  static __device__ __forceinline__ uint32_t frag_addr(int c0, int lane) {
    const int L = lane & 15, k = 8 * (lane >> 5) + (L >> 2);
    return k * ROWB + ((((c0 >> 5) ^ swz(k)) & (NC - 1)) << 6) + (((lane >> 4) & 1) << 5) + ((L & 3) << 3);
  }
  static __device__ __forceinline__ bf16x8 frag(const char* __restrict__ S, uint32_t addr, int plane) {
    const char* q = S + plane * PLANE + addr;
    const s16x4 lo = __builtin_amdgcn_ds_read_tr16_b64_v4i16((lds_s16x4*)(q));
    const s16x4 hi = __builtin_amdgcn_ds_read_tr16_b64_v4i16((lds_s16x4*)(q + 4 * ROWB));
    typedef short s16x8 __attribute__((ext_vector_type(8)));
    const s16x8 v = __builtin_shufflevector(lo, hi, 0, 1, 2, 3, 4, 5, 6, 7);
    return __builtin_bit_cast(bf16x8, v);
  }
};

template <class OPA, class OPB>
struct Producer {
  OPA& oa;
  OPB& ob;
  float4 (&fa)[OPA::NV];
  float4 (&fb)[OPB::NV];
  char* dstA;
  char* dstB;
  const float* abase;
  const float* bbase;
  const float* bscale;
  int64_t lda, ldb;
  int64_t left1, left2;
  int t;
  bool do_stage = true;
  static constexpr int P = OPA::NV + OPB::NV;
  template <int PIECE>
  __device__ __forceinline__ void one() {
    if constexpr (PIECE < OPA::NV) {
      if (do_stage) oa.template stage<PIECE>(fa, dstA, left1, t);
      oa.template load<PIECE>(fa, abase, lda, left2, nullptr, t);
    } else {
      constexpr int J = PIECE - OPA::NV;
      if (do_stage) ob.template stage<J>(fb, dstB, left1, t);
      ob.template load<J>(fb, bbase, ldb, left2, bscale, t);
    }
  }
  template <int G, int NG, int... Is>
  __device__ __forceinline__ void group_impl(std::integer_sequence<int, Is...>) {
    ((Is * NG / P == G ? one<Is>() : void()), ...);
  }
  template <int G, int NG>
  __device__ __forceinline__ void group() { group_impl<G, NG>(std::make_integer_sequence<int, P>{}); }
};

template <int WTN, class OPA, class OPB, class PR>
__device__ __forceinline__ void limb_tile_step(const char* __restrict__ As, const char* __restrict__ Bs, const uint32_t (&aaddr)[2],
                                               const uint32_t (&baddr)[WTN], f32x16 (&acc)[2][WTN], PR& pr) {
  constexpr int NH = WTN / 2, NG = 6 * NH;
#define CB_MFMA4(A_, B_, H_, G_)                                                                             \
  _Pragma("unroll") for (int i = 0; i < 2; ++i) _Pragma("unroll") for (int j = 0; j < 2; ++j)               \
      acc[i][2 * H_ + j] = __builtin_amdgcn_mfma_f32_32x32x16_bf16(A_[i], B_[j], acc[i][2 * H_ + j], 0, 0, 0); \
  pr.template group<G_, NG>();
#define CB_HALF(H_)                                                                                                          \
  {                                                                                                                          \
    bf16x8 b_hi[2], b_mid[2], b_lo[2];                                                                                       \
    if (H_ == 0) { _Pragma("unroll") for (int i = 0; i < 2; ++i) a_lo[i] = OPA::frag(As, aaddr[i], 2); }                     \
    _Pragma("unroll") for (int j = 0; j < 2; ++j) b_hi[j] = OPB::frag(Bs, baddr[2 * H_ + j], 0);                             \
    if (H_ == 0) { _Pragma("unroll") for (int i = 0; i < 2; ++i) a_hi[i] = OPA::frag(As, aaddr[i], 0); }                     \
    _Pragma("unroll") for (int j = 0; j < 2; ++j) b_lo[j] = OPB::frag(Bs, baddr[2 * H_ + j], 2);                             \
    if (H_ == 0) { _Pragma("unroll") for (int i = 0; i < 2; ++i) a_mid[i] = OPA::frag(As, aaddr[i], 1); }                    \
    _Pragma("unroll") for (int j = 0; j < 2; ++j) b_mid[j] = OPB::frag(Bs, baddr[2 * H_ + j], 1);                            \
    CB_MFMA4(a_lo, b_hi, H_, H_ * 6 + 0)                                                                                     \
    CB_MFMA4(a_hi, b_lo, H_, H_ * 6 + 1)                                                                                     \
    CB_MFMA4(a_mid, b_mid, H_, H_ * 6 + 2)                                                                                   \
    CB_MFMA4(a_mid, b_hi, H_, H_ * 6 + 3)                                                                                    \
// ... 72 lines not shown
```

gnn-tail-generalization_amd/gemm.py:

```python
import torch

from . import _lib


def _rowmajor(t):
    if t.dim() != 2:
        raise ValueError('expected a matrix')
    if t.shape[1] > 1 and t.stride(1) != 1:
        t = t.contiguous()
    elif t.shape[0] > 1 and t.stride(0) < t.shape[1]:
        t = t.contiguous()
    return t


def _ld(t):
    return t.stride(0) if t.shape[0] > 1 else max(t.shape[1], 1)


def _b_workspace(lib, N, K, M, device):
    wsb = lib.cb_gemm_nn_splitk_workspace_bytes(M, N, K) if K >= 512 else 0
    return (torch.empty(wsb, dtype=torch.uint8, device=device), wsb) if wsb else (None, 0)


def mm_nn(a, b, rowscale=None, addend=None, bias=None, relu=False, out_bf16=False, out=None):
# ... 33 lines not shown
        return None
    out = torch.empty((M, N), dtype=torch.float32, device=a.device)
    if not lib.cb_gemm_nn_store_rows_supported(_lib.ptr(a), _ld(a), _lib.ptr(b), _ld(b), _lib.ptr(out), _ld(out), M, N, K):
        return None
    if addend is not None:
        addend = _rowmajor(addend)
    act = torch.empty_like(out) if want_act else None
    with torch.cuda.device(a.device):
        _lib.check(lib.cb_gemm_nn_store_rows_f32(_lib.ptr(a), _ld(a), _lib.ptr(b), _ld(b), _lib.ptr(out), _ld(out), M, N, K, _lib.ptr(rowscale), _lib.ptr(addend),
                                                 _ld(addend) if addend is not None else 0, _lib.ptr(bias), _lib.ptr(row_index),
                                                 ops.store_args(mix, mix_index, c_act, c_mix, p, seed, row0, bits, relu_only, act), None, 0,
                                                 _lib.stream_ptr()), 'cb_gemm_nn_store_rows_f32')
    return out, act


def mm_nn_drop2(a, b, p, seed, row0=0, bias=None, relu=False):
    import ctypes
    from . import ops
    lib = _lib.load()
    _lib.require_device(a, b, bias)
    a, b = _rowmajor(a), _rowmajor(b)
    M, K = a.shape
    K2, N = b.shape
    if K != K2 or a.dtype != torch.float32 or b.dtype != torch.float32:
        raise ValueError(f'mm_nn_drop2: bad operands {tuple(a.shape)} @ {tuple(b.shape)}')
    y = torch.empty((M, N), dtype=torch.float32, device=a.device)
    yd = torch.empty((M, N), dtype=torch.float32, device=a.device)
    ws, wsb = _b_workspace(lib, N, K, M, a.device)
    with torch.cuda.device(a.device):
        _lib.check(lib.cb_gemm_nn_drop2_f32(_lib.ptr(a), _ld(a), _lib.ptr(b), _ld(b), _lib.ptr(y), N, _lib.ptr(yd), N, M, N, K, None, None, 0,
                                            _lib.ptr(bias), int(bool(relu)), float(p), ctypes.c_uint64(seed), ops.seed_dev_ptr(), int(row0),
                                            _lib.ptr(ws), wsb, _lib.stream_ptr()), 'cb_gemm_nn_drop2_f32')
    return y, yd


def mm_nn_indrop_drop2(a, b, p, a_seed, seed, row0=0, bias=None, relu=False, want_bits=False):
    import ctypes
    from . import ops
    lib = _lib.load()
    _lib.require_device(a, b, bias)
    a, b = _rowmajor(a), _rowmajor(b)
    M, K = a.shape
    K2, N = b.shape
    if K != K2 or a.dtype != torch.float32 or b.dtype != torch.float32 or not (0.0 < p < 1.0):
        return None
    y = torch.empty((M, N), dtype=torch.float32, device=a.device)
    yd = torch.empty((M, N), dtype=torch.float32, device=a.device)
    if not lib.cb_gemm_nn_indrop_supported(_lib.ptr(a), _ld(a), _lib.ptr(b), _ld(b), _lib.ptr(y), N, _lib.ptr(yd), N, M, N, K):
        return None
    bits = torch.empty((M, 1, 4), dtype=torch.int64, device=a.device) if (want_bits and N == 256 and relu) else None
    with torch.cuda.device(a.device):
        _lib.check(lib.cb_gemm_nn_indrop_drop2_f32(_lib.ptr(a), _ld(a), _lib.ptr(b), _ld(b), _lib.ptr(y), N, _lib.ptr(yd), N, M, N, K, _lib.ptr(bias),
                                                   int(bool(relu)), float(p), ctypes.c_uint64(a_seed), float(p), ctypes.c_uint64(seed),
                                                   ops.seed_dev_ptr(), int(row0), _lib.ptr(bits), _lib.stream_ptr()), 'cb_gemm_nn_indrop_drop2_f32')
    return (y, yd, bits) if want_bits else (y, yd)


def mm_nn_indrop(a, b, p, a_seed, row0=0, rowscale=None, addend=None, bias=None, relu=False, want_bits=False, out=None):
    import ctypes
    from . import ops
    lib = _lib.load()
    _lib.require_device(a, b, rowscale, addend, bias, out)
    a, b = _rowmajor(a), _rowmajor(b)
    M, K = a.shape
    K2, N = b.shape
    if K != K2 or a.dtype != torch.float32 or b.dtype != torch.float32 or not (0.0 < p < 1.0):
        return None
    if addend is not None:
        addend = _rowmajor(addend)
        if addend.data_ptr() % 16 or _ld(addend) % 4:
            return None
    y = out if out is not None else torch.empty((M, N), dtype=torch.float32, device=a.device)
    if not lib.cb_gemm_nn_indrop_supported(_lib.ptr(a), _ld(a), _lib.ptr(b), _ld(b), _lib.ptr(y), _ld(y), _lib.ptr(y), _ld(y), M, N, K):
        return None
    bits = torch.empty((M, 1, 4), dtype=torch.int64, device=a.device) if (want_bits and N == 256 and relu) else None
    with torch.cuda.device(a.device):
        _lib.check(lib.cb_gemm_nn_indrop_f32(_lib.ptr(a), _ld(a), _lib.ptr(b), _ld(b), _lib.ptr(y), _ld(y), M, N, K, _lib.ptr(rowscale), _lib.ptr(addend),
                                             _ld(addend) if addend is not None else 0, _lib.ptr(bias), int(bool(relu)), float(p),
                                             ctypes.c_uint64(a_seed), ops.seed_dev_ptr(), int(row0), _lib.ptr(bits), _lib.stream_ptr()),
                   'cb_gemm_nn_indrop_f32')
    return (y, bits) if want_bits else y


def trunk_front(x, w_in, b_in, w0, rowscale, addend, p, seed_x, seed_x0, row0=0, want_bits=False, want_drop=False, z_out=None):
    import ctypes
    from . import ops
    lib = _lib.load()
    _lib.require_device(x, w_in, b_in, w0, rowscale, addend)
    if x.dim() != 2 or x.dtype != torch.float32 or tuple(w_in.shape) != (256, x.shape[1]) or tuple(w0.shape) != (256, 256):
        return None
    M, K = x.shape
    nb_in = lib.cb_front_image_bytes(K)
    if not nb_in or w_in.dtype != torch.float32 or w0.dtype != torch.float32:
        return None
    x, w_in, w0 = _rowmajor(x), _rowmajor(w_in), _rowmajor(w0)
    if addend is not None:
        addend = _rowmajor(addend)
    if x.data_ptr() % 16 or _ld(x) % 4 or (addend is not None and (addend.data_ptr() % 16 or _ld(addend) % 4)):
        return None
    dev = x.device
    img_in = torch.empty(nb_in, dtype=torch.uint8, device=dev)
    nb0 = lib.cb_agg_gemm_image_bytes(256, 256)
    img0 = torch.empty(nb0, dtype=torch.uint8, device=dev)
    x0 = torch.empty((M, 256), dtype=torch.float32, device=dev)
    z0 = z_out if z_out is not None else torch.empty((M, 256), dtype=torch.float32, device=dev)
    bits = torch.empty((M, 1, 4), dtype=torch.int64, device=dev) if want_bits else None
    xd = torch.empty((M, 256), dtype=torch.float32, device=dev) if want_drop else None
    with torch.cuda.device(dev):
        _lib.check(lib.cb_front_image_f32(_lib.ptr(w_in), _ld(w_in), K, 1, _lib.ptr(img_in), nb_in, _lib.stream_ptr()), 'cb_front_image_f32')
        _lib.check(lib.cb_agg_gemm_image_f32(_lib.ptr(w0), _ld(w0), 256, 256, 0, _lib.ptr(img0), nb0, _lib.stream_ptr()), 'cb_agg_gemm_image_f32')
        _lib.check(lib.cb_trunk_front_f32(_lib.ptr(x), _ld(x), M, K, _lib.ptr(img_in), _lib.ptr(b_in), _lib.ptr(img0), _lib.ptr(rowscale),
                                          _lib.ptr(addend), _ld(addend) if addend is not None else 0, _lib.ptr(x0), 256, _lib.ptr(bits),
                                          _lib.ptr(xd), 256, _lib.ptr(z0), 256, float(p), ctypes.c_uint64(seed_x), ctypes.c_uint64(seed_x0),
                                          ops.seed_dev_ptr(), int(row0), _lib.stream_ptr()), 'cb_trunk_front_f32')
    return x0, bits, xd, z0


def mm_tn_adrop(a, g, p, a_seed, row0=0, rowscale=None):
    import ctypes
    from . import ops
    lib = _lib.load()
    _lib.require_device(a, g, rowscale)
    a, g = _rowmajor(a), _rowmajor(g)
    M, K1 = a.shape
    M2, K2 = g.shape
    if M != M2 or not (0.0 < p < 1.0) or not lib.cb_gemm_tn_adrop_supported(_lib.ptr(a), _ld(a), _lib.ptr(g), _ld(g), K1, K2):
        return None
    out = torch.empty((K1, K2), dtype=torch.float32, device=a.device)
    wsb = lib.cb_gemm_tn_workspace_bytes(M, K1, K2)
    ws = torch.empty(max(wsb, 16), dtype=torch.uint8, device=a.device)
    with torch.cuda.device(a.device):
        _lib.check(lib.cb_gemm_tn_adrop_f32(_lib.ptr(a), _ld(a), _lib.ptr(g), _ld(g), _lib.ptr(rowscale), _lib.ptr(out), M, K1, K2, float(p),
                                            ctypes.c_uint64(a_seed), ops.seed_dev_ptr(), int(row0), _lib.ptr(ws), wsb, _lib.stream_ptr()),
                   'cb_gemm_tn_adrop_f32')
    return out


def mm_tn_gdrop(a, g, p, g_seed, row0=0):
    import ctypes
    from . import ops
    lib = _lib.load()
    _lib.require_device(a, g)
    a, g = _rowmajor(a), _rowmajor(g)
    M, K1 = a.shape
    M2, K2 = g.shape
    if M != M2 or not (0.0 < p < 1.0) or not lib.cb_gemm_tn_gdrop_supported(_lib.ptr(a), _ld(a), _lib.ptr(g), _ld(g), K1, K2):
        return None
    out = torch.empty((K1, K2), dtype=torch.float32, device=a.device)
    wsb = lib.cb_gemm_tn_workspace_bytes(M, K1, K2)
    ws = torch.empty(max(wsb, 16), dtype=torch.uint8, device=a.device)
    with torch.cuda.device(a.device):
        _lib.check(lib.cb_gemm_tn_gdrop_f32(_lib.ptr(a), _ld(a), _lib.ptr(g), _ld(g), _lib.ptr(out), M, K1, K2, float(p), ctypes.c_uint64(g_seed),
                                            ops.seed_dev_ptr(), int(row0), _lib.ptr(ws), wsb, _lib.stream_ptr()), 'cb_gemm_tn_gdrop_f32')
    return out


def mm_tn_instage_supported(g_like, x, M):
    lib = _lib.load()
    return (g_like.dim() == 2 and g_like.shape[1] == 256 and g_like.is_contiguous() and x.dim() == 2 and x.stride(1) == 1
            and bool(lib.cb_gemm_tn_instage_supported(_lib.ptr(g_like), _lib.ptr(g_like), _lib.ptr(x), _ld(x), int(M), int(x.shape[1]))))


def mm_tn_instage(g, mfold, x0_bits, x, p_g, g_seed, p_x, x_seed, row0=0):
    import ctypes
    from . import ops
    lib = _lib.load()
    _lib.require_device(g, mfold, x0_bits, x)
    M, K2 = x.shape
    if (tuple(g.shape) != (M, 256) or tuple(mfold.shape) != (M, 256) or not g.is_contiguous() or not mfold.is_contiguous() or x0_bits.numel() != 4 * M
            or not x0_bits.is_contiguous() or x0_bits.dtype != torch.int64):
        raise ValueError('mm_tn_instage: contiguous [M, 256] gradients, [M, 1, 4] int64 mask words and [M, F] features expected')
    out = torch.empty((256, K2), dtype=torch.float32, device=g.device)
    colsum = torch.empty(256, dtype=torch.float32, device=g.device)
    wsb = lib.cb_gemm_tn_instage_workspace_bytes(M, K2)
    ws = torch.empty(max(wsb, 16), dtype=torch.uint8, device=g.device)
    with torch.cuda.device(g.device):
        _lib.check(lib.cb_gemm_tn_instage_f32(_lib.ptr(g), _lib.ptr(mfold), _lib.ptr(x0_bits), _lib.ptr(x), _ld(x), _lib.ptr(out), _lib.ptr(colsum), M, K2,
                                              float(p_g), ctypes.c_uint64(g_seed), float(p_x), ctypes.c_uint64(x_seed), ops.seed_dev_ptr(), int(row0),
                                              _lib.ptr(ws), wsb, _lib.stream_ptr()), 'cb_gemm_tn_instage_f32')
    return out, colsum


def mm_tn(a, g, rowscale=None):
    lib = _lib.load()
    _lib.require_device(a, g, rowscale)
    a, g = _rowmajor(a), _rowmajor(g)
    M, K1 = a.shape
    M2, K2 = g.shape
    if M != M2:
        raise ValueError(f'shape mismatch: {tuple(a.shape)}^T @ {tuple(g.shape)}')
    out = torch.empty((K1, K2), dtype=torch.float32, device=a.device)
    wsb = lib.cb_gemm_tn_workspace_bytes(M, K1, K2)
    ws = torch.empty(max(wsb, 16), dtype=torch.uint8, device=a.device)
    with torch.cuda.device(a.device):
        _lib.check(lib.cb_gemm_tn_f32(_lib.ptr(a), _ld(a), _lib.ptr(g), _ld(g), _lib.ptr(rowscale), _lib.ptr(out), M, K1, K2,
                                      _lib.ptr(ws), wsb, _lib.stream_ptr()), 'cb_gemm_tn_f32')
    return out


class _LinearRowscaleFn(torch.autograd.Function):

    @staticmethod
    def forward(ctx, x, w, rowscale, addend):
        ctx.save_for_backward(x, w, rowscale)
        ctx.has_addend = addend is not None
        return mm_nn(x, w, rowscale=rowscale, addend=addend)

    @staticmethod
    def backward(ctx, g):
        x, w, rowscale = ctx.saved_tensors
        g = _rowmajor(g)
        dx = mm_nn(g, w.t().contiguous(), rowscale=rowscale) if ctx.needs_input_grad[0] else None
        dw = mm_tn(x, g, rowscale=rowscale) if ctx.needs_input_grad[1] else None
        de = g if (ctx.has_addend and ctx.needs_input_grad[3]) else None
        return dx, dw, None, de


def linear_rowscale(x, w, rowscale=None, addend=None):
    return _LinearRowscaleFn.apply(x, w, rowscale, addend)


class _LinearFn(torch.autograd.Function):

    @staticmethod
    def forward(ctx, x, weight, bias, relu):
        y = mm_nn(x, weight.t().contiguous(), bias=bias, relu=relu)
        ctx.relu, ctx.has_bias = relu, bias is not None
        ctx.save_for_backward(x, weight, y if relu else None)
        return y

    @staticmethod
    def backward(ctx, g):
        from .ops import act_bwd
        x, weight, y = ctx.saved_tensors
        need_b = ctx.has_bias and ctx.needs_input_grad[2]
        g = _rowmajor(g)
        if ctx.relu or need_b:
            gm, db = act_bwd(g, y if ctx.relu else None, None, want_out=ctx.relu, want_colsum=need_b)
            if gm is None:
                gm = g
        else:
            gm, db = g, None
        dx = mm_nn(gm, weight) if ctx.needs_input_grad[0] else None
        dw = mm_tn(gm, x) if ctx.needs_input_grad[1] else None
        return dx, dw, db, None


def linear(x, weight, bias=None, relu=False):
    _lib.require_device(x, weight)
    return _LinearFn.apply(x, weight, bias, bool(relu))
```

gnn-tail-generalization_amd/trunk.py:

```python
import ctypes
import os
from typing import NamedTuple

import torch

from . import _lib, gemm, ops
from .graph import head_image, prof_rec, weight_image
from .tuning import T


def _switch(name, default):
    return os.environ.get(name, default)


TrunkCfg = NamedTuple('TrunkCfg', [('L', int), ('alpha', float), ('p', float), ('seeds', tuple), ('agg_bf16', bool), ('track', bool), ('loss_rows', object),
                                   ('residual', bool), ('rows_only', bool)])
TrunkCfg.__doc__ = """What one call of the trunk was asked for (second argument of _TrunkFn.apply).  L: number of GCNConv layers; alpha: weight of the mix
source in a layer's output (res_tricks.py); p: the one dropout rate (0 in evaluation); seeds: L + 2 dropout seeds (features, X0, one per layer); agg_bf16:
the gathered rows Z_l are stored as bf16; track: autograd was recording when the trunk was called (inside a Function's forward it never is, and
needs_input_grad does not know about no_grad); loss_rows: None or (bool mask [N], count), the caller's promise that the output receives gradient in those
rows only (ops.py); residual: the 'Residual' connection (mix source of layer l > 0 = the previous layer's ReLU output) instead of 'Initial' (X0);
rows_only: the second promise — the caller READS the output in the rows of loss_rows only (the others: ops.unread_rows_fill)."""


# ... 352 lines not shown

def _store_rows(y, idx, mix, c_act, c_mix, p, seed, row0, bits, relu_only, mix_index=None, want_act=False):
    lib = _lib.load()
    out = torch.empty_like(y)
    act = torch.empty_like(y) if want_act else None
    with torch.cuda.device(y.device):
        _lib.check(lib.cb_trunk_store_rows_f32(_lib.ptr(y), _lib.ptr(idx), y.shape[0], y.shape[1],
                                               ops.store_args(mix, mix_index, c_act, c_mix, p, seed, row0, bits, relu_only, act), _lib.ptr(out),
                                               _lib.stream_ptr()), 'cb_trunk_store_rows_f32')
    return out, act


def _layer_on_rows(graph, space, fwd, col_scale, cur, w, b, mix, mix_index, alpha, p, seed, row0, residual, want_act=False, le=None, fwd_le=None):
    fwd.profile = getattr(graph, 'profile', None)
    b_rows = space.norm_in_of(graph)
    bits = torch.empty((graph.N, w.shape[1] // 256, 4), dtype=torch.int64, device=cur.device)
    if (le is None and tuple(w.shape) == (256, 256) and hasattr(fwd, 'spmm_gemm_store_rows') and fwd.E >= T.agg_gemm_store_rows_min_edges
            and agg_gemm_eligible(graph, 256, False)):
        h_agg, x_next, act = fwd.spmm_gemm_store_rows(cur, col_scale, weight_image(w), b_rows, b, space.idx, mix, mix_index, 1 - alpha, alpha, p, seed,
                                                      row0, bits, residual, want_act)
        return bits, x_next, act, h_agg
    h_agg = fwd.spmm(cur, col_scale=col_scale)
    le_sum = None
    if le is not None:
        fwd_le.profile = fwd.profile
        le_sum = fwd_le.spmm(le, row_scale=b_rows)
    fused = gemm.mm_nn_store_rows(h_agg, w, b_rows, le_sum, b, space.idx, mix, mix_index, 1 - alpha, alpha, p, seed, row0, bits, residual, want_act)
    if fused is not None:
        return bits, fused[0], fused[1], h_agg
    y = gemm.mm_nn(h_agg, w, rowscale=b_rows, addend=le_sum, bias=b)
    del le_sum
    x_next, act = _store_rows(y, space.idx, mix, 1 - alpha, alpha, p, seed, row0, bits, residual, mix_index, want_act)
    return bits, x_next, act, h_agg


def _last_layer_on_loss_rows(graph, plan, cur, w, b, mix, alpha, p, seed, row0, residual, w_out, b_out, below=None, le=None):
    sp = plan.space0
    fwd0 = graph.loss_rows_fwd(plan) if below is None else below.fwd0c
    mix_index = None
    if below is not None and residual:
        mix_index = getattr(plan, '_pos0_in_1', None)
        if mix_index is None:
            mix_index = plan._pos0_in_1 = below.s1.pos[sp.idx].long().contiguous()
    bits, x_l, _act, h_agg = _layer_on_rows(graph, sp, fwd0, graph.norm_out if below is None else below.s1.a, cur, w, b, mix, mix_index, alpha, p, seed, row0,
                                           residual, le=le, fwd_le=graph.loss_rows_fwd(plan) if le is not None else None)
    n = graph.N
    logits_c = gemm.mm_nn(x_l, w_out.t().contiguous(), bias=b_out)
    out = ops.expand_unread(logits_c, sp, n)
    graph.rows_only_forwards = getattr(graph, 'rows_only_forwards', 0) + 1
    return bits, x_l, (out, logits_c), h_agg


def _last_layer_on_loss_rows_sharded(graph, s0, orient, cur, w, b, mix, alpha, p, seed, row0, residual, w_out, b_out, le=None):
    lib = _lib.load()
    xs = _exchanged(graph, cur.shape[0], cur.shape[1])
    with torch.cuda.device(cur.device):
        _lib.check(lib.cb_act_bwd_f32(_lib.ptr(cur), None, _lib.ptr(graph.norm_out), _lib.ptr(xs), cur.shape[0], cur.shape[1], None, None, 0,
                                      _lib.stream_ptr()), 'cb_act_bwd_f32')
    h_agg = graph.aggregate_finish(graph.aggregate_start(xs, False, orient=orient), False)
    del xs
    b0 = s0.norm_in_of(graph)
    le_sum = graph.aggregate_finish(graph.aggregate_start(le, False, orient=orient), False, row_scale=b0) if le is not None else None
    y = gemm.mm_nn(h_agg, w, rowscale=b0, addend=le_sum, bias=b)
    del h_agg, le_sum
    n, d = graph.N, w.shape[1]
    bits = torch.empty((n, d // 256, 4), dtype=torch.int64, device=cur.device)
    x_l, _act = _store_rows(y, s0.idx, mix, 1 - alpha, alpha, p, seed, row0, bits, residual)
    del y
    logits_c = gemm.mm_nn(x_l, w_out.t().contiguous(), bias=b_out)
    out = ops.expand_unread(logits_c, s0, n)
    graph.rows_only_forwards += 1
    return bits, x_l, out


class _Forward:

    def __init__(self, ctx, graph, cfg, x, w_in, b_in, w_out, b_out, layer_params):
        self.graph, self.cfg, self.x = graph, cfg, x.contiguous()
        self.w_in, self.b_in, self.w_out, self.b_out = w_in, b_in, w_out, b_out
        self.layer_params, self.layers = layer_params, _layers(layer_params)
        self.row0, self.a = int(getattr(graph, 'row_offset', 0)), graph.norm_out
        self.bwd = bool(cfg.track) and any(ctx.needs_input_grad)
        self.z_ready = self.out_head = self.out_rows = self.h_last = self.h_below = None

    def run(self):
        cfg, graph = self.cfg, self.graph
        (self.xd, self.x0, self.x0_bits, self.cur, self.z_front), self.indrop = self._front()
        h = self.x0.shape[1]
        self.saved_in, self.saved_bits = [self.cur], []
        self.ag = agg_gemm_eligible(graph, h, cfg.agg_bf16)
        self.ro = _rows_only_decision(graph, cfg, self.x, self.x0, h, self.ag, self.bwd, self.layer_params)
        self.mix, self.kw = self.x0, dict(want_bits=self.bwd, relu_only=cfg.residual)
        for l in range(cfg.L):
            self.st = (self.layers[l][1], self.mix, 1 - cfg.alpha, cfg.alpha, cfg.p, cfg.seeds[l + 2] if cfg.p > 0 else 0)
            self.keep_act = cfg.residual and l + 1 < cfg.L
            z0 = self._z0() if l == 0 else None
            bits, self.cur, act = self._form(l, z0 is not None)(l, z0)
            del z0
            if cfg.residual:
                self.mix = act
            if self.bwd:
                self.saved_bits.append(bits)
                self.saved_in.append(self.cur)
        self.mix = None
        return self.out_head if self.out_head is not None else gemm.mm_nn(self.cur, self.w_out.t().contiguous(), bias=self.b_out)

    def _front(self):
        c, x, w_in, b_in, row0, bwd, p, seeds = self.cfg, self.x, self.w_in, self.b_in, self.row0, self.bwd, self.cfg.p, self.cfg.seeds
        indrop = p > 0 and _switch('CB_TRUNK_INDROP', '1') != '0'
        copy = _switch('CB_TRUNK_X0_COPY', '1') == '1'
        if (indrop or p == 0) and not c.agg_bf16 and c.L >= 1 and w_in.shape[0] == 256 and _switch('CB_TRUNK_FRONT', '1') != '0':
            w0, _b0, le0 = self.layers[0]
            fr = gemm.trunk_front(x, w_in, b_in, w0, self.a, le0, p, seeds[0], seeds[1], row0, want_bits=bwd, want_drop=bwd and p > 0 and copy,
                                  z_out=_exchanged(self.graph, x.shape[0]) if hasattr(self.graph, 'part') else None)
            if fr is not None:
                x0, x0_bits, cur, z_front = fr
                return (x, x0, x0_bits, x0 if p == 0 else cur, z_front), True
        if indrop:
            wb = bwd and w_in.shape[0] == 256
            r = None if copy else gemm.mm_nn_indrop(x, w_in.t().contiguous(), p, seeds[0], row0, bias=b_in, relu=True, want_bits=wb)
            if r is not None:
                return (x, *(r if wb else (r, None)), None, None), True
            r = gemm.mm_nn_indrop_drop2(x, w_in.t().contiguous(), p, seeds[0], seeds[1], row0, bias=b_in, relu=True, want_bits=wb)
            if r is not None:
                return (x, r[0], r[2] if len(r) > 2 else None, r[1], None), True
        xd = ops._dropout_raw(x, p, seeds[0], row0 * x.shape[1]) if p > 0 else x
        if p > 0:
            x0, cur = gemm.mm_nn_drop2(xd, w_in.t().contiguous(), p, seeds[1], row0, bias=b_in, relu=True)
        else:
            x0 = cur = gemm.mm_nn(xd, w_in.t().contiguous(), bias=b_in, relu=True)
        return (xd, x0, None, cur, None), False

    def dropped_x0(self):
        return ops._dropout_raw(self.x0, self.cfg.p, self.cfg.seeds[1], self.row0 * self.x0.shape[1])

    def _z0(self):
        z0, self.z_front = self.z_front, None
        if z0 is not None or self.cur is not None:
            return z0
        c, (w, _b, le) = self.cfg, self.layers[0]
        if not (c.agg_bf16 or (not self.ag and _chunked(self.graph, c.agg_bf16))):
            z0 = gemm.mm_nn_indrop(self.x0, w, c.p, c.seeds[1], self.row0, rowscale=self.a, addend=le, out=_exchanged(self.graph, self.x0.shape[0], w.shape[1]))
        if z0 is None:
            self.cur = self.saved_in[0] = self.dropped_x0()
        return z0

    def _form(self, l, have_z0):
        L, ro = self.cfg.L, self.ro
        if self.ag and ro.sum_first_below and l == L - 2:
            return self._form_sum_first_below
        if self.ag and ro.sharded is not None and l == L - 1:
            return self._form_last_on_loss_rows_sharded
        if ro.plan is not None and l == L - 1:
            return self._form_last_on_loss_rows
        if self.ag:
            if ro.sum_first_below and l + 3 == L:
                return self._form_store
            if ro.plan is not None and l + 2 == L and ro.below is not None:
                return self._form_store_on_s1
            if (ro.plan is not None or ro.sharded is not None) and l + 2 == L:
                return self._form_store
            return self._form_store_gemm if l + 1 < L else self._form_store_head
        if not have_z0 and _chunked(self.graph, self.cfg.agg_bf16):
            return self._form_chunked
        return self._form_store

    def _z(self, l, z0):
        z, self.z_ready = self.z_ready, None
        if z is None and z0 is None:
            (w, _b, le), bf = self.layers[l], self.cfg.agg_bf16
            return gemm.mm_nn(self.cur, w, rowscale=self.a, addend=le, out_bf16=bf, out=None if bf else _exchanged(self.graph, self.cur.shape[0], w.shape[1]))
        return z if z is not None else z0

    def _form_sum_first_below(self, l, z0):
        c, below, (w, b, _le) = self.cfg, self.ro.below, self.layers[l]
        bits, cur, act, self.h_below = _layer_on_rows(self.graph, below.s1, below.fwd1, self.a, self.cur, w, b, self.mix, None, c.alpha, c.p,
                                                      self.st[5], self.row0, c.residual, want_act=self.keep_act)
        self.saved_in[l] = None
        return bits, cur, act

    def _form_last_on_loss_rows_sharded(self, l, z0):
        c, (s0, orient), (w, b, le) = self.cfg, self.ro.sharded, self.layers[l]
        bits, cur, self.out_head = _last_layer_on_loss_rows_sharded(self.graph, s0, orient, self.cur, w, b, self.mix, c.alpha, c.p, self.st[5],
                                                                    self.row0, c.residual, self.w_out, self.b_out, le=le)
        return bits, cur, None

    def _form_last_on_loss_rows(self, l, z0):
        c, (w, b, le) = self.cfg, self.layers[l]
        bits, cur, (self.out_head, self.out_rows), self.h_last = _last_layer_on_loss_rows(
            self.graph, self.ro.plan, self.cur, w, b, self.mix, c.alpha, c.p, self.st[5], self.row0, c.residual, self.w_out, self.b_out,
            below=self.ro.below, le=le)
        if le is None:
            self.saved_in[l] = None
        else:
            self.h_last = None
        return bits, cur, None

    def _form_store(self, l, z0):
        return _fused_spmm(self.graph, self._z(l, z0), *self.st, want_act=self.keep_act, **self.kw)

    def _form_store_on_s1(self, l, z0):
        below, z = self.ro.below, self._z(l, z0)
        below.fwd1.profile = getattr(self.graph, 'profile', None)
        return _fused_launch(_lib.load(), self.graph, below.fwd1, z, None, *self.st, self.keep_act, row_ids=below.ids1, row_scale=below.b1, **self.kw)

    def _form_store_gemm(self, l, z0):
        w1, _, le1 = self.layers[l + 1]
        res = _fused_gemm(self.graph, self._z(l, z0), *self.st, weight_image(w1), self.a, le1, want_act=self.keep_act, **self.kw)
        self.z_ready = res[2]
        return res[0], res[1], res[3] if self.keep_act else None

    def _form_store_head(self, l, z0):
        z = self._z(l, z0)
        himg = head_image(self.w_out) if head_tail_enabled(self.bwd) else None
        if himg is None:
            return _fused_spmm(self.graph, z, *self.st, **self.kw)
        bits, cur, self.out_head = _fused_gemm(self.graph, z, *self.st, himg, None, None, head=(self.b_out, self.w_out.shape[0]), **self.kw)[:3]
        return bits, cur, None

    def _form_chunked(self, l, z0):
        (w, _b, le), cur, a = self.layers[l], self.cur, self.a
        z = _exchanged(self.graph, cur.shape[0], w.shape[1])

        def produce(k, r0, r1):
            if r1 > r0:
                gemm.mm_nn(cur[r0:r1], w, rowscale=a[r0:r1], addend=le[r0:r1] if le is not None else None, out=z[r0:r1])
        return _fused_spmm(self.graph, z, *self.st, want_act=self.keep_act, produce=produce, **self.kw)


class _TrunkFn(torch.autograd.Function):
    @staticmethod
    def forward(ctx, graph, cfg, x, w_in, b_in, w_out, b_out, *layer_params):
        f = _Forward(ctx, graph, cfg, x, w_in, b_in, w_out, b_out, layer_params)
        out = f.run()
        ctx.graph, ctx.cfg, ctx.row0, ctx.indrop, ctx.n_layer_params = graph, cfg, f.row0, f.indrop, len(layer_params)
        if f.bwd:
            _save(ctx, xd=f.xd, x0=f.x0, w_in=w_in, w_out=w_out, saved_in=f.saved_in, saved_bits=f.saved_bits, layer_params=layer_params,
                  h_last=f.h_last, h_below=f.h_below, x0_bits=f.x0_bits)
            ro = f.ro
            ctx.saved_rows = SavedRows('S0' if (ro.plan is not None or ro.sharded is not None) else 'all',
                                       'absent' if f.h_last is not None else 'S1' if (ro.plan is not None and ro.below is not None) else 'all')
        ctx.set_materialize_grads(False)
        return out, f.out_rows

    @staticmethod
    def backward(ctx, gout, gout_rows=None):
        if gout is None and gout_rows is None:
            return (None,) * (7 + ctx.n_layer_params)
        return _Backward(ctx, gout, gout_rows).run()


class _Carry:
    __slots__ = ('g', 'gr', 'dbias', 'handle', 'space', 'g_above', 'deferred')

    def __init__(self, g, gr, dbias, handle, space):
        self.g, self.gr, self.dbias, self.handle, self.space, self.g_above, self.deferred = g, gr, dbias, handle, space, None, None


class _Backward:

    def __init__(self, ctx, gout, gout_rows=None):
        self.gout_rows = gemm._rowmajor(gout_rows) if gout_rows is not None else None
        self.ctx, graph, c = ctx, ctx.graph, ctx.cfg
        self.graph, self.row0, self.L, self.alpha, self.p, self.seeds = graph, ctx.row0, c.L, c.alpha, c.p, c.seeds
        self.agg_bf16, self.residual = c.agg_bf16, c.residual
        sv = _saved(ctx)
        self.xd, self.x0, self.w_in, self.w_out = sv['xd'], sv['x0'], sv['w_in'], sv['w_out']
        self.saved_in, self.saved_bits, self.x0_bits = sv['saved_in'], sv['saved_bits'], sv['x0_bits']
        self.h_last, self.h_below = sv['h_last'], sv['h_below']
        self.lp, self.where = _layers(sv['layer_params']), ctx.saved_rows
        self.a, self.bnorm = graph.norm_out, graph.norm_in
        self.need = ctx.needs_input_grad
        self.gout = gemm._rowmajor(gout) if gout is not None else None
        self.n_rows, self.h = self.x0.shape
        self.sharded, loss_rows = hasattr(graph, 'part'), c.loss_rows
        if loss_rows is not None and self.where.x_last != 'S0' and (not ops.loss_rows_enabled() or loss_rows[0].shape[0] != self.x0.shape[0]):
            loss_rows = None
        self.loss_rows = loss_rows
        self.gather = _gather(graph, c.L, c.residual, self.x0)
        self.gx0 = None if self.gather else torch.empty_like(self.x0)
        self.g_mix, self.seeds_mix, self.mix_pos = [], [], []
        self.cs = []
        self.grads_layers = [None] * (3 * c.L)
        self.ag = agg_gemm_eligible(graph, self.h, c.agg_bf16)
        self.chunked = (self.gather and _chunked(graph, c.agg_bf16) and graph.b.plan.n_slices > 1 and not self.ag)
        self.fold_ok = (_switch('CB_INSTAGE_FOLD', '1') != '0' and self.gather and not c.residual and not c.agg_bf16 and c.p > 0
                        and ctx.indrop and self.need[3] and not self.need[2] and self.x0_bits is not None and self.h == 256
                        and gemm.mm_tn_instage_supported(self.x0, self.xd, self.x0.shape[0]))
        self.mfold, self.plan_taken = None, False

    def seed(self, i):
        return self.seeds[i] if self.p > 0 else 0

    def need_w(self, l):
        return self.need[7 + 3 * l]

    def need_b(self, l):
        return self.need[7 + 3 * l + 1]

    def need_le(self, l):
        return self.lp[l][2] is not None and self.need[7 + 3 * l + 2]

    def _dw(self, l, x_in, gz):
        if x_in is not None:
            return gemm.mm_tn(x_in, gz, rowscale=self.a)
        return _dw_regen(self.x0, gz, self.p, self.seed(1), self.row0, self.a)

    def _second(self, below, g_above, pos_above=None):
        if not self.residual or g_above is None:
            return {}
        return dict(g2=g_above, seed2=self.seed(below + 3), c2=self.alpha, **({'g2_pos': pos_above} if pos_above is not None else {}))

    def _dx_and_store_bwd(self, src, wt, rowscale, below, g_ready=None, g_above=None, orient=None, pos_above=None):
        p, alpha, row0, bnorm = self.p, self.alpha, self.row0, self.bnorm
        sd, want_b, bits = self.seed(below + 2), self.need_b(below), self.saved_bits[below]
        if self.chunked:
            g_ = torch.empty((src.shape[0], wt.shape[1]), dtype=torch.float32, device=src.device)
            gr_ = _exchanged(self.graph, g_.shape[0], g_.shape[1])
            colsums = []
            sec = self._second(below, g_above, pos_above)

            def produce(k, r0, r1):
                if r1 <= r0:
                    return
                gemm.mm_nn(src[r0:r1], wt, rowscale=rowscale[r0:r1] if rowscale is not None else None, out=g_[r0:r1])
                sec_k = dict(sec, g2=sec['g2'][r0:r1]) if sec else {}
                _, cs = _layer_bwd(g_[r0:r1], bits[r0:r1], bnorm[r0:r1], None, False, p, sd, row0 + r0, 1 - alpha, alpha, want_b, out=gr_[r0:r1], **sec_k)
                if want_b:
                    colsums.append(cs)
            h_ = self.graph.aggregate_start(gr_, True, produce=produce, orient=orient)
            db_ = None
            if want_b:
                db_ = (torch.zeros(wt.shape[1], dtype=torch.float32, device=src.device) if not colsums
                       else colsums[0] if len(colsums) == 1 else torch.stack(colsums).sum(0))
            return g_, gr_, db_, h_
        g_ = g_ready if g_ready is not None else gemm.mm_nn(src, wt, rowscale=rowscale)
        cs_ = self.cs
        if (below == 0 and self.fold_ok and self.mfold is None and self.plan_taken and len(self.g_mix) <= 2 and len(cs_) <= 1
                and all(t.is_contiguous() for t in self.g_mix) and g_.is_contiguous()):
            res = _layer_bwd_fold(g_, bits, bnorm, p, sd, row0, 1 - alpha, alpha, want_b, self.g_mix, self.mix_pos, self.seeds_mix,
                                  out=_exchanged(self.graph, g_.shape[0], g_.shape[1]) if self.sharded else None, cs=cs_[0][:3] if cs_ else None)
            gr_, db_, self.mfold = res[:3]
            if cs_:
                self.grads_layers[3 * cs_[0][3] + 1] = res[3]
                self.cs = []
            self.g_mix, self.mix_pos, self.seeds_mix = [], [], []
            return None, gr_, db_, None
        gr_, db_ = _layer_bwd(g_, bits, bnorm, self.gx0, below != self.L - 1, p, sd, row0, 1 - alpha, alpha, want_b, out_bf16=self.agg_bf16,
                              out=_exchanged(self.graph, g_.shape[0], g_.shape[1]) if (self.sharded and not self.agg_bf16) else None,
                              **self._second(below, g_above, pos_above))
        return g_, gr_, db_, None

    def _head(self, space):
        L, need, gout, xl = self.L, self.need, self.gout, self.saved_in[self.L]
        if space is not None:
            gout = ops.gather_rows_by_index(gout, space.idx) if gout is not None else None
            if self.gout_rows is not None:
                gout = self.gout_rows if gout is None else gout + self.gout_rows
            xl = xl if self.where.x_last == 'S0' else ops.gather_rows_by_index(xl, space.idx)
        self.d_w_out = gemm.mm_tn(gout, xl) if need[5] else None
        self.d_b_out = ops.act_bwd(gout, None, None, want_out=False, want_colsum=True)[1] if need[6] else None
        if space is None:
            return _Carry(*self._dx_and_store_bwd(gout, self.w_out, None, L - 1, orient=self._orient_of(L - 1)), None)
        g = gemm.mm_nn(gout, self.w_out)
        gr, dbias = _layer_bwd_rows(g, space.idx, self.saved_bits[L - 1], self.bnorm, self.p, self.seed(L + 1), self.row0, 1 - self.alpha,
                                    self.need_b(L - 1), out=_exchanged(self.graph, g.shape[0], g.shape[1]) if self.sharded else None)
        return _Carry(g, gr, dbias, None, space)

    def _sh_level(self, layer):
        j = self.L - 1 - layer
        return self.sh_levels[j] if 0 <= j < len(self.sh_levels) else None

    def _orient_of(self, layer):
        return getattr(self._sh_level(layer), 'orient', None)

    def _dw_rows(self, l, x_in, gz, dst):
        if dst is None:
            return self._dw(l, x_in, gz)
        return gemm.mm_tn(ops.gather_rows_by_index(x_in, dst.idx), gz, rowscale=dst.a)

    def _layer_source_side(self, l, gr, level, fwd_j):
        w = self.lp[l][0]
        dst = level[1]
        level[0].profile = getattr(self.graph, 'profile', None)
        if fwd_j is not None:
            fwd_j.profile = level[0].profile
        t = gemm.mm_nn(gr, w.t().contiguous())
        fused = None
        if (l > 0 and not self.residual and self.gather and len(self.cs) < 2 and dst is None
                and hasattr(level[0], 'spmm_store_bwd') and t.shape[1] % 256 == 0):
            fold = self.fold_ok and l == 1 and len(self.g_mix) <= 2 and all(q is not None for q in self.mix_pos) and not self.cs
            if fold:
                self.mfold, gr_below, db0 = level[0].spmm_store_bwd(t, self.a, self.saved_bits[0], self.bnorm, 1 - self.alpha, self.p, self.seed(2), self.row0,
                                                                    mix=(self.g_mix, self.mix_pos, self.seeds_mix, self.alpha, self.need_b(0)))
                self.grads_layers[1] = db0
                self.g_mix, self.mix_pos, self.seeds_mix = [], [], []
                g_new = None
            else:
                g_new, gr_below = level[0].spmm_store_bwd(t, self.a, self.saved_bits[l - 1], self.bnorm, 1 - self.alpha, self.p, self.seed(l + 1), self.row0)
            fused = (gr_below, l - 1)
        else:
            g_new = level[0].spmm(t, row_scale=dst.a if dst is not None else self.a)
        del t
        if self.need_w(l):
            x_agg = (self.h_last if (self.where.x_below == 'absent' and l == self.L - 1) else self.h_below if (self.h_below is not None and l == self.L - 2)
                     else fwd_j.spmm(self.saved_in[l], col_scale=self.a))
            self.grads_layers[3 * l] = gemm.mm_tn(x_agg, gr)
        return None, g_new, fused

    def _layer_compact(self, l, gr, level):
        w = self.lp[l][0]
        dst = level[1]
        level[0].profile = getattr(self.graph, 'profile', None)
        gz, g_new = level[0].spmm_gemm(gr, weight_image(w, transpose=True), transpose=False, g_rowscale=dst.a if dst is not None else self.a)
        if self.need_w(l):
            if dst is not None:
                on_s1 = self.where.x_below == 'S1' and l == self.L - 1
                x_rows = self.saved_in[l] if on_s1 else ops.gather_rows_by_index(self.saved_in[l], dst.idx)
                self.grads_layers[3 * l] = gemm.mm_tn(x_rows, gz, rowscale=dst.a)
            else:
                self.grads_layers[3 * l] = self._dw(l, self.saved_in[l], gz)
        return gz, g_new

    def _layer_fused(self, l, gr, handle, dst=None):
        graph = self.graph
        a = dst.a if dst is not None else self.a
        img = weight_image(self.lp[l][0], transpose=True)

        def tail(csr, src, acc, tr):
            csr.profile = getattr(graph, 'profile', None)
            return csr.spmm_gemm(src, img, transpose=tr, g_rowscale=a, acc_init=acc)
        return (graph.aggregate_finish(handle, True, last_pass=lambda csr, recv, acc: tail(csr, recv, acc, False)) if self.sharded
                else tail(graph, gr, None, True))

    def _layer_plain(self, gr, handle):
        return self.graph.aggregate_finish(handle, True) if self.sharded else _spmm_t(self.graph, gr)

    def _resolve_plan(self):
        graph, L, gout, xl_compact = self.graph, self.L, self.gout, self.where.x_last == 'S0'
        self.sh_levels = []
        if self.gout_rows is not None and not xl_compact:
            raise RuntimeError('gradient for the compact loss-row logits, but the forward did not run rows-only')
        if self.sharded and hasattr(graph, 'support_levels') and self.loss_rows is not None:
            ops.check_rows_zero(gout, self.loss_rows[0])
            self.sh_levels = graph.support_levels(self.loss_rows[0], L, compact=self.ag and self.gather, cumulative=self.residual)
        plan = None
        hint = None if self.sharded else _support_plan(graph, self.loss_rows, self.n_rows, L, self.residual, self.h, self.x0, committed=xl_compact)
        if hint is not None:
            if gout is not None:
                ops.check_rows_zero(gout, hint[0])
            plan = graph.grad_support_plan(hint[0], L, max_frac=T.rowsparse_max_frac, cumulative=self.residual, count=not xl_compact)
        self.plan_taken = plan is not None or bool(self.sh_levels)
        if self.where.x_below == 'absent' and plan is None:
            raise RuntimeError('the forward evaluated its last layer on the loss rows (rows_only), but its backward finds no row-support plan: '
                               'CB_LOSS_ROWS / tuning.T / the mask changed between the forward and the backward')
        space0 = plan.space0 if plan is not None else (self.sh_levels[0].src if self.sh_levels else None)
        if xl_compact and space0 is None:
            raise RuntimeError('the forward evaluated its last layer on the loss rows (rows_only), but its backward has no compact level 0')
        return plan, space0

    def _layer(self, l, c, plan):
        L, graph, sharded = self.L, self.graph, self.sharded
        j = L - 1 - l
        level = plan.levels[j] if (plan is not None and j < len(plan.levels)) else None
        lv = self._sh_level(l)
        dst = level[1] if level is not None else lv.dst if lv is not None else None
        if sharded and c.handle is None:
            c.handle = graph.aggregate_start(c.gr, True, orient=self._orient_of(l))
        if c.deferred is not None:
            self.grads_layers[3 * c.deferred[0]] = self._dw_rows(*c.deferred)
            c.deferred = None
        fwd_j = plan.fwd[j] if (level is not None and j < len(plan.fwd)) else None
        source_side = ((self.where.x_below == 'absent' and l == L - 1) or (self.h_below is not None and l == L - 2)
                       or (T.rowsparse_loss_side and fwd_j is not None and not self.need_le(l)
                           and not (self.need_w(l) and self.saved_in[l] is None)
                           and not (self.where.x_below == 'S1' and l == L - 1)))
        if source_side:
            _gz, g_new, fused = self._layer_source_side(l, c.gr, level, fwd_j)
            return None, g_new, dst, fused
        if level is not None:
            return (*self._layer_compact(l, c.gr, level), dst, None)
        gz, g_new = self._layer_fused(l, c.gr, c.handle, dst) if self.ag else (self._layer_plain(c.gr, c.handle), None)
        if self.need_w(l):
            if sharded:
                c.deferred = (l, self.saved_in[l], gz, dst if self.ag else None)
            else:
                self.grads_layers[3 * l] = self._dw(l, self.saved_in[l], gz)
        return gz, g_new, dst, None

    def _store_bwd_below(self, l, c, gz, g_new, dst, fused, pos_above):
        w = self.lp[l][0]
        if l > 0 and fused is not None:
            c.g, (c.gr, _below), c.dbias = g_new, fused, None
            if self.mfold is not None:
                c.dbias = self.grads_layers[3 * (l - 1) + 1]
            elif self.need_b(l - 1):
                self.cs = self.cs + [(len(self.g_mix), self.saved_bits[l - 1], 1 - self.alpha, l - 1)]
        elif l > 0 and dst is not None:
            c.g = g_new
            c.gr, c.dbias = _layer_bwd_rows(g_new, dst.idx, self.saved_bits[l - 1], self.bnorm, self.p, self.seed(l + 1), self.row0, 1 - self.alpha,
                                            self.need_b(l - 1), out=_exchanged(self.graph, g_new.shape[0], g_new.shape[1]) if self.sharded else None,
                                            **self._second(l - 1, c.g_above, pos_above))
        elif l > 0:
            c.g, c.gr, c.dbias, c.handle = self._dx_and_store_bwd(gz, w.t().contiguous(), self.a, l - 1, g_new, c.g_above, orient=self._orient_of(l - 1),
                                                                  pos_above=pos_above)
        else:
            c.g = g_new if g_new is not None else gemm.mm_nn(gz, w.t().contiguous(), rowscale=self.a)

    def run(self):
        plan, space0 = self._resolve_plan()
        c = self._head(space0)
        for l in range(self.L - 1, -1, -1):
            if self.gather and (not self.residual or l == 0) and self.mfold is None:
                self.g_mix.append(c.g)
                self.mix_pos.append(c.space.pos if c.space is not None else None)
                self.seeds_mix.append(self.seed(l + 2))
            gz, g_new, dst, fused = self._layer(l, c, plan)
            c.g_above = c.g if self.residual else None
            pos_above = c.space.pos if (self.residual and c.space is not None) else None
            c.g = c.gr = c.handle = None
            self.grads_layers[3 * l + 1] = c.dbias
            c.space = dst
            self._store_bwd_below(l, c, gz, g_new, dst, fused, pos_above)
            c.g_above = None
            if self.need_le(l):
                if dst is not None:
                    gz = ops.expand_rows(gz, dst.pos)
                self.grads_layers[3 * l + 2] = gz
            del gz, g_new
        if c.deferred is not None:
            self.grads_layers[3 * c.deferred[0]] = self._dw_rows(*c.deferred)
        return self._input_stage(c)

    def _input_stage(self, c):
        graph, p, need, xd, row0 = self.graph, self.p, self.need, self.xd, self.row0
        g, c.g = c.g, None
        if self.mfold is not None:
            d_w_in, d_b_in = gemm.mm_tn_instage(g, self.mfold, self.x0_bits, xd, p, self.seed(1), p, self.seeds[0], row0)
            del g
            self.gx0 = self.g_mix = self.mfold = None
            graph.instage_folds = getattr(graph, 'instage_folds', 0) + 1
            return (None, None, None, d_w_in, d_b_in if need[4] else None, self.d_w_out, self.d_b_out, *self.grads_layers)
        if self.gather:
            res = _input_bwd_multi(g, self.seed(1), self.g_mix, self.seeds_mix, self.alpha, self.x0, p, row0, act_bits=self.x0_bits,
                                   mix_pos=self.mix_pos, cs=[q[:3] for q in self.cs])
            gpre, d_b_in = res[0], res[1]
            for q, db in zip(self.cs, res[2] if self.cs else []):
                self.grads_layers[3 * q[3] + 1] = db
        else:
            gpre, d_b_in = _input_bwd(g, self.gx0, self.x0, p, self.seed(1), row0)
        del g
        self.gx0 = self.g_mix = None
        d_w_in = None
        if need[3]:
            if self.ctx.indrop and p > 0:
                d_w_in = gemm.mm_tn_gdrop(gpre, xd, p, self.seeds[0], row0)
                if d_w_in is None:
                    d_w_in = gemm.mm_tn(gpre, ops._dropout_raw(xd, p, self.seeds[0], row0 * xd.shape[1]))
            else:
                d_w_in = gemm.mm_tn(gpre, xd)
        d_x = None
        if need[2]:
            d_x = gemm.mm_nn(gpre, self.w_in)
            if p > 0:
                d_x = ops._dropout_raw(d_x, p, self.seeds[0], row0 * d_x.shape[1])
        return (None, None, d_x, d_w_in, d_b_in if need[4] else None, self.d_w_out, self.d_b_out, *self.grads_layers)


def forward(tc, x, graph, loss_rows=None, rows_only=False):
    L = tc.num_layers
    p = float(tc.dropout) if tc.training else 0.0
    seeds = tuple(ops.next_seed() for _ in range(L + 2)) if p > 0 else (0,) * (L + 2)
    params, se_reg_all = _collect_layer_params(tc, graph)
    agg_bf16 = getattr(tc.args, 'agg_dtype', 'f32') == 'bf16'
    if loss_rows is not None:
        mask, count = loss_rows if isinstance(loss_rows, (tuple, list)) else (loss_rows, None)
        if count is None:
            count = int(mask.sum().item())
        if mask.dtype != torch.bool or mask.dim() != 1 or mask.shape[0] != x.shape[0]:
            raise ValueError(f'loss_rows: a bool mask over the {x.shape[0]} rows expected, got {tuple(mask.shape)} {mask.dtype}')
        loss_rows = (mask, int(count))
    cfg = TrunkCfg(L, float(tc.alpha), p, seeds, agg_bf16, torch.is_grad_enabled(), loss_rows, connection(tc) == 'residual',
                   bool(rows_only) and loss_rows is not None)
    out, out_rows = _TrunkFn.apply(graph, cfg, x, tc.layers_MLP[0].weight, tc.layers_MLP[0].bias, tc.layers_MLP[1].weight, tc.layers_MLP[1].bias, *params)
    if out_rows is not None:
        out._cb_rows = (out_rows, loss_rows[0])
    return out, se_reg_all
```

include/coldbrew_hip.h:

```cpp
#ifndef COLDBREW_HIP_H
#define COLDBREW_HIP_H

#include <stddef.h>
#include <stdint.h>

#ifdef __cplusplus
extern "C" {
#endif

#define CB_OK 0
#define CB_E_INVALID (-1)
#define CB_E_RANGE (-2)
#define CB_E_WORKSPACE (-3)
#define CB_E_HIP (-4)
#define CB_E_DEVICE (-5)

#define CB_DEVERR_HANDOVER 1
#define CB_DEVERR_GRADROWS 2

int cb_version(void);
const char* cb_last_error(void);
int cb_device_status(void);

int cb_rows_zero_outside_mask_f32(const float* g, int64_t ld, int64_t rows, int64_t d, const uint8_t* mask, int32_t* guard, void* stream);
// ... 91 lines not shown
                                const uint64_t* cs_bits, float cs_c, float* colsum2, void* ws2, size_t ws2_bytes, void* stream);
int cb_trunk_layer_bwd_rows_f32(const float* g, const int64_t* row_index, int64_t n_rows, const uint64_t* relu_bits, const float* row_scale, float* out,
                                int64_t d, float drop_p, uint64_t seed, const uint64_t* seed_dev, int64_t row0, float c_act, const float* g2, uint64_t seed2,
                                float c2, const int32_t* g2_pos, float* colsum, void* ws, size_t ws_bytes, void* stream);

int cb_trunk_input_bwd_f32(const float* g, const float* add, const float* act, float* out, int64_t rows, int64_t d, float drop_p,
                           uint64_t seed, const uint64_t* seed_dev, int64_t row0, float* colsum, void* ws, size_t ws_bytes,
                           void* stream);

int cb_trunk_input_bwd_multi_f32(const float* g, uint64_t seed, int32_t n_mix, const float* const* g_mix, const uint64_t* seeds_mix,
                                 float c_mix, const float* act, float* out, int64_t rows, int64_t d, float drop_p,
                                 const uint64_t* seed_dev, int64_t row0, float* colsum, void* ws, size_t ws_bytes,
                                 const uint64_t* act_bits, const int32_t* const* g_mix_pos, void* stream);
int cb_trunk_input_bwd_multi_cs_f32(const float* g, uint64_t seed, int32_t n_mix, const float* const* g_mix, const uint64_t* seeds_mix,
                                    float c_mix, const float* act, float* out, int64_t rows, int64_t d, float drop_p,
                                    const uint64_t* seed_dev, int64_t row0, float* colsum, void* ws, size_t ws_bytes,
                                    const uint64_t* act_bits, const int32_t* const* g_mix_pos, int32_t n_cs, const int32_t* cs_src,
                                    const uint64_t* const* cs_bits, const float* cs_c, float* const* colsum2, void* ws2, size_t ws2_bytes, void* stream);
int cb_spmm_csr_store_bwd_f32(const cb_csr_view* g, const float* h, int64_t ld_h, int64_t d, const float* row_scale, const uint64_t* relu_bits,
                              const float* bwd_rowscale, float c_act, float drop_p, uint64_t seed, const uint64_t* seed_dev, int64_t row0,
                              float* out_g, int64_t ld_g, float* out_gr, int64_t ld_gr, void* stream);
size_t cb_spmm_store_bwd_mix_workspace_bytes(int64_t N, int64_t n_hubs, int64_t d);
int cb_spmm_csr_store_bwd_mix_f32(const cb_csr_view* g, const float* h, int64_t ld_h, int64_t d, const float* row_scale, const uint64_t* relu_bits,
                                  const float* bwd_rowscale, float c_act, float drop_p, uint64_t seed, const uint64_t* seed_dev, int64_t row0,
                                  float* out_m, int64_t ld_m, float* out_gr, int64_t ld_gr, int32_t n_mix, const float* const* mix_g,
                                  const int32_t* const* mix_pos, const uint64_t* mix_seeds, float c_mix, float* colsum, void* ws2, size_t ws2_bytes,
                                  void* stream);

int cb_gemm_nn_bf16out_f32(const float* A, int64_t lda, const float* B, int64_t ldb, uint16_t* C, int64_t ldc, int64_t M, int64_t N,
                           int64_t K, const float* rowscale, const float* addend, int64_t ld_add, const float* bias, int relu,
                           void* ws, size_t ws_bytes, void* stream);

int cb_node_norm_fwd_f32(const float* x, float* y, float* stats2, int64_t rows, int64_t d, float c, float q, float eps, void* stream);
int cb_node_norm_bwd_f32(const float* x, const float* g, const float* stats2, float* dx, int64_t rows, int64_t d, float c, float q,
                         void* stream);
size_t cb_colstats_workspace_bytes(int64_t rows, int64_t d);
int cb_colstats_f32(const float* x, const float* w, const float* shift, int64_t rows, int64_t d, float* colsum, float* colsum2,
                    void* ws, size_t ws_bytes, void* stream);
int cb_col_affine_f32(const float* x, const float* shift, const float* scale, const float* bias, float gscale, float* y, int64_t rows,
                      int64_t d, void* stream);
int cb_col_bwd_combine_f32(const float* g, const float* xh, const float* xs, const float* a, const float* b, const float* e, float ga,
                           float gb, float* dx, int64_t rows, int64_t d, void* stream);

size_t cb_topk_replace_workspace_bytes(int64_t B, int64_t N, int64_t K);
int cb_topk_replace_f32(const float* q, int64_t ldq, const float* t, int64_t ldt, int64_t B, int64_t N, int64_t D, int32_t K,
                        float* out, int32_t* out_idx, float* out_w, void* ws, size_t ws_bytes, void* stream);

int cb_id_count_i64(const int64_t* ids, int64_t E, int64_t N, int32_t* counts, int32_t* n_bad, void* stream);
int cb_value_hist_i32(const int32_t* vals, int64_t N, int32_t n_bins, int32_t* hist, int32_t* n_bad, void* stream);
size_t cb_compact_workspace_bytes(int64_t n);
int cb_select_range_i32(const int32_t* vals, int64_t N, int32_t lo, int32_t hi, int64_t* out_idx, uint8_t* out_mask, int64_t* count,
                        void* ws, size_t ws_bytes, void* stream);
int cb_craft_isolation_i64(const int64_t* src, const int64_t* dst, int64_t E, const uint8_t* node_flag, int64_t N, int64_t* out_src,
                           int64_t* out_dst, int64_t* count, void* ws, size_t ws_bytes, void* stream);
size_t cb_symmetrize_workspace_bytes(int64_t E, int64_t N);
int cb_symmetrize_i64(const int64_t* src, const int64_t* dst, int64_t E, int64_t N, int64_t* out_row, int64_t* out_col, int64_t* count,
                      int32_t* n_bad, void* ws, size_t ws_bytes, void* stream);

int cb_gather_rows_f32(const float* src, int64_t ld, const int64_t* idx, int64_t n_idx, int64_t d, float* out, void* stream);

size_t cb_agg_gemm_image_bytes(int64_t K, int64_t N);
int cb_agg_gemm_image_f32(const float* W, int64_t ld, int64_t K, int64_t N, int transpose, void* image, size_t image_bytes, void* stream);
int cb_spmm_gemm_f32(const cb_csr_view* g, const float* h, int64_t ld_h, int64_t d, const float* row_scale, const float* bias, int relu,
                     const float* acc_init, int64_t ld_init, float* out, int64_t ld_out, const void* image, const float* g_rowscale,
                     const float* g_addend, int64_t ld_add, float* g_out, int64_t ld_gout, void* stream);
int cb_spmm_gemm_fused_f32(const cb_csr_view* g, const float* acc_init, int64_t ld_init, const float* h, int64_t ld_h, int64_t d,
                           const float* row_scale, const float* bias, const cb_trunk_store* store, float* out_next, int64_t ld_next,
                           int32_t skip_next, const void* image, const float* g_rowscale, const float* g_addend, int64_t ld_add, float* g_out,
                           int64_t ld_gout, void* stream);
size_t cb_agg_gemm_head_image_bytes(int64_t K, int64_t C);
int cb_agg_gemm_head_image_f32(const float* W, int64_t ld, int64_t K, int64_t C, int transpose, void* image, size_t image_bytes, void* stream);
int cb_spmm_gemm_fused_head_f32(const cb_csr_view* g, const float* acc_init, int64_t ld_init, const float* h, int64_t ld_h, int64_t d,
                                const float* row_scale, const float* bias, const cb_trunk_store* store, float* out_next, int64_t ld_next,
                                int32_t skip_next, const void* head_image, const float* head_bias, int64_t C, float* logits, int64_t ld_logits,
                                void* stream);
int cb_agg_gemm_handover_selftest(void* stream);

size_t cb_front_image_bytes(int64_t K);
int cb_front_image_f32(const float* W, int64_t ld, int64_t K, int transpose, void* image, size_t image_bytes, void* stream);
int cb_trunk_front_f32(const float* x, int64_t ld_x, int64_t M, int64_t K, const void* image_in, const float* bias_in, const void* image_0,
                       const float* rowscale, const float* addend, int64_t ld_add, float* x0, int64_t ld_x0, uint64_t* relu_bits, float* x0_drop,
                       int64_t ld_drop, float* z0, int64_t ld_z, float drop_p, uint64_t seed_x, uint64_t seed_x0, const uint64_t* seed_dev,
                       int64_t row0, void* stream);

int cb_spmm_csr_weighted_f32(const int32_t* rowptr, const int32_t* col, const float* w, int64_t N, int64_t E, const float* h, int64_t ld_h,
                             int64_t d, const float* row_scale, const float* bias, int relu, float* out, int64_t ld_out, void* stream);
int cb_spmm_edge_dot_f32(const int32_t* rowptr, const int32_t* col, int64_t N, int64_t E, const float* h, int64_t ld_h, const float* g,
                         int64_t ld_g, int64_t d, float* dw, void* stream);

int cb_gemm_nn_indrop_supported(const float* A, int64_t lda, const float* B, int64_t ldb, const float* C, int64_t ldc, const float* C2, int64_t ldc2,
                                int64_t M, int64_t N, int64_t K);
int cb_gemm_nn_indrop_drop2_f32(const float* A, int64_t lda, const float* B, int64_t ldb, float* C, int64_t ldc, float* C2, int64_t ldc2,
                                int64_t M, int64_t N, int64_t K, const float* bias, int relu, float a_drop_p, uint64_t a_seed, float drop_p,
                                uint64_t seed, const uint64_t* seed_dev, int64_t row0, uint64_t* relu_bits, void* stream);
int cb_gemm_nn_indrop_f32(const float* A, int64_t lda, const float* B, int64_t ldb, float* C, int64_t ldc, int64_t M, int64_t N, int64_t K,
                          const float* rowscale, const float* addend, int64_t ld_add, const float* bias, int relu, float a_drop_p, uint64_t a_seed,
                          const uint64_t* seed_dev, int64_t row0, uint64_t* relu_bits, void* stream);
int cb_gemm_tn_adrop_supported(const float* A, int64_t lda, const float* G, int64_t ldg, int64_t K1, int64_t K2);
int cb_gemm_tn_adrop_f32(const float* A, int64_t lda, const float* G, int64_t ldg, const float* rowscale, float* C, int64_t M, int64_t K1, int64_t K2,
                         float a_drop_p, uint64_t a_seed, const uint64_t* seed_dev, int64_t row0, void* ws, size_t ws_bytes, void* stream);
int cb_gemm_tn_gdrop_supported(const float* A, int64_t lda, const float* G, int64_t ldg, int64_t K1, int64_t K2);
int cb_gemm_tn_gdrop_f32(const float* A, int64_t lda, const float* G, int64_t ldg, float* C, int64_t M, int64_t K1, int64_t K2, float g_drop_p,
                         uint64_t g_seed, const uint64_t* seed_dev, int64_t row0, void* ws, size_t ws_bytes, void* stream);
int cb_gemm_tn_instage_supported(const float* g, const float* mfold, const float* X, int64_t ldx, int64_t M, int64_t K2);
size_t cb_gemm_tn_instage_workspace_bytes(int64_t M, int64_t K2);
int cb_gemm_tn_instage_f32(const float* g, const float* mfold, const uint64_t* x0_bits, const float* X, int64_t ldx, float* C, float* colsum, int64_t M, int64_t K2,
                           float g_drop_p, uint64_t g_seed, float x_drop_p, uint64_t x_seed, const uint64_t* seed_dev, int64_t row0, void* ws, size_t ws_bytes,
                           void* stream);

int cb_spmm_gemm_store_rows_f32(const cb_csr_view* g, const float* h, int64_t ld_h, int64_t d, const float* col_scale, float* out, int64_t ld_out,
                                const void* image, const float* g_rowscale, const float* bias, const int64_t* row_ids, const cb_trunk_store* store,
                                float* g_out, int64_t ld_gout, void* stream);

int cb_spmm_csr_lp_f32(const cb_csr_view* g, const float* h, int64_t ld_h, int64_t d, const float* row_scale, const float* mix, int64_t ld_mix,
                       float c_mix, const float* post_scale, float* out, int64_t ld_out, void* stream);

int cb_spmm_csr_prop_f32(const cb_csr_view* g, const float* h, int64_t ld_h, int64_t d, const float* row_scale, const float* mix, int64_t ld_mix,
                         float c_mix, float lo, float hi, const uint8_t* fix_rows, const float* post_scale, float* out, int64_t ld_out,
                         void* stream);

size_t cb_cs_workspace_bytes(int64_t N, int64_t Cp);
int cb_cs_residual_init_f32(const float* P, int64_t ld_p, const int64_t* labels, const uint8_t* label_rows, int64_t N, int64_t C, int64_t Cp,
                            const float* state_scale, float* E0, float* state, float* abs_sum, void* ws, size_t ws_bytes, void* stream);
int cb_cs_correct_snap_f32(int32_t mode, const float* P, int64_t ld_p, const float* resid, int64_t ld_r, const int64_t* labels,
                           const uint8_t* label_rows, int64_t N, int64_t C, int64_t Cp, const float* abs_sum, int64_t n_label, float scale,
                           const float* state_scale, float* res_result, int64_t ld_res, float* y2, float* state, void* stream);

int cb_gather_rows_bf16_f32(const float* src, int64_t ld, const int64_t* idx, int64_t n_idx, int64_t d, uint16_t* out, void* stream);
int cb_expand_rows_f32(const float* src, const int32_t* pos, int64_t n_rows, int64_t d, float fill, float* out, void* stream);
int cb_trunk_store_rows_f32(const float* y, const int64_t* row_index, int64_t n_rows, int64_t d, const cb_trunk_store* store, float* out, void* stream);
int cb_gemm_nn_store_rows_supported(const float* A, int64_t lda, const float* B, int64_t ldb, const float* C, int64_t ldc, int64_t M, int64_t N, int64_t K);
int cb_gemm_nn_store_rows_f32(const float* A, int64_t lda, const float* B, int64_t ldb, float* C, int64_t ldc, int64_t M, int64_t N, int64_t K,
                              const float* rowscale, const float* addend, int64_t ld_add, const float* bias, const int64_t* row_index,
                              const cb_trunk_store* store, void* ws, size_t ws_bytes, void* stream);


int cb_ln_gelu_drop_fwd_f32(const float* z, int64_t rows, int64_t d, const float* gamma, const float* beta, float eps, float p,
                            uint64_t seed, const uint64_t* seed_dev, float* out, float* stats, void* stream);
size_t cb_ln_gelu_drop_bwd_workspace_bytes(int64_t rows, int64_t d);
int cb_ln_gelu_drop_bwd_f32(const float* dy, const float* z, const float* stats, int64_t rows, int64_t d, const float* gamma,
                            const float* beta, float p, uint64_t seed, const uint64_t* seed_dev, float* dz, float* dgamma,
                            float* dbeta, float* dbias, void* ws, size_t ws_bytes, void* stream);

int cb_mse_rows_f32(const float* pred, int64_t B, int64_t D, const float* target, int64_t ld_t, int64_t n_target_rows,
                    const int64_t* row_index, float* loss, float* grad, void* ws, size_t ws_bytes, void* stream);

int cb_part2_assemble_f32(const float* x, int64_t F, const float* replaced, const float* part1_out, int64_t D, const float* alphas,
                          int64_t B, float* out, void* stream);
int cb_part2_assemble_bwd_f32(const float* g, int64_t F, const float* replaced, const float* part1_out, int64_t D, int64_t B,
                              float* dalphas, void* ws, size_t ws_bytes, void* stream);


int cb_ncloss_positions_i64(const int64_t* batch_idx, int64_t B, int64_t n, int32_t* pos, int32_t* rep, void* stream);

int cb_ncloss_row_norms_f32(const float* x, int64_t ldx, int64_t rows, int64_t D, float* nrm, float* rinv, void* stream);

int cb_cosine_scale_f32(float* s, int64_t ld, int64_t N, const float* nrm, void* stream);

int cb_ncloss_uses_limb_core(const float* z, int64_t ldz, int64_t D);

size_t cb_ncloss_workspace_bytes(int64_t B, int32_t max_splits);
int cb_ncloss_fwd_f32(const float* z, int64_t ldz, int64_t B, int64_t D, float tau, const int32_t* rowptr, const int32_t* col,
                      const float* val, int64_t n, const int64_t* batch_idx, const int32_t* pos, const int32_t* rep, int32_t max_splits,
                      float* rinv, float* num, float* den, float* w, float* u, float* loss, int32_t* m_count, void* ws, size_t ws_bytes,
                      void* stream);

int cb_ncloss_normalize_rows_f32(const float* z, int64_t ldz, int64_t B, int64_t D, const float* rinv, float* zhat, void* stream);
int cb_ncloss_bwd_slab_f32(const float* z, int64_t ldz, int64_t B, int64_t D, float tau, const float* rinv, const float* w, int64_t row0,
                           int64_t rows, int32_t max_splits, float* P, int64_t ldp, void* stream);
int cb_ncloss_bwd_finish_f32(const float* z, int64_t ldz, const float* zhat, int64_t B, int64_t D, float tau, const float* rinv, const float* u,
                             const int32_t* rowptr, const int32_t* col, const float* val, const int32_t* rowptr_t, const int32_t* col_t,
                             const float* val_t, int64_t n, const int64_t* batch_idx, const int32_t* pos, const int32_t* rep, const float* g,
                             float* dzh, float* dz, void* stream);


size_t cb_spgemm_offsets_workspace_bytes(int64_t nnz_a);
int cb_spgemm_entry_offsets_i64(const int32_t* col_a, int64_t nnz_a, const int32_t* rowptr_b, int64_t k, int64_t* ent_off, int32_t* n_bad,
                                void* ws, size_t ws_bytes, void* stream);

size_t cb_spgemm_chunk_workspace_bytes(int64_t n_products);
int cb_spgemm_chunk_count_f32(const int32_t* rowptr_a, const int32_t* col_a, const float* val_a, const int32_t* rowptr_b, const int32_t* col_b,
                              const float* val_b, const int64_t* ent_off, int64_t row0, int64_t row1, int64_t k, int64_t n_cols,
                              int64_t n_products, int64_t* count, void* ws, size_t ws_bytes, void* stream);

int cb_spgemm_chunk_emit_f32(const void* ws, size_t ws_bytes, int64_t row0, int64_t row1, int64_t n_cols, int64_t n_products, int64_t count,
                             int64_t nnz_base, int32_t* rowptr, int32_t* col_out, float* val_out, void* stream);

size_t cb_csr_transpose_workspace_bytes(int64_t nnz);
int cb_csr_transpose_f32(const int32_t* rowptr, const int32_t* col, const float* val, int64_t m, int64_t n, int64_t nnz, int32_t* rowptr_t,
                         int32_t* col_t, float* val_t, void* ws, size_t ws_bytes, void* stream);

// ... 69 lines not shown
```

Baseline: 9.646.

## Record dropout keep masks in the front kernel and reuse them in backward

The fused trunk-front kernel now optionally writes packed dropout keep words for the input x and the layer-0 activation x0. Backward GEMMs (the input-stage TN contraction and a new kdrop TN weight-gradient path) read these words instead of regenerating Philox masks, and the forward no longer materialises the dropped x0 copy when kdrop is eligible. This trades extra mask memory traffic and storage for fewer RNG recomputations and one fewer dense activation buffer, and adds new template variants and eligibility checks.

Result: no change. 9.700, median of 6 (+0.6%).

```diff
diff --git a/gnn-tail-generalization_amd/_lib.py b/gnn-tail-generalization_amd/_lib.py
--- a/gnn-tail-generalization_amd/_lib.py
+++ b/gnn-tail-generalization_amd/_lib.py
@@ -105,6 +105,12 @@
     'cb_front_image_f32': (ctypes.c_int, [_P, _I64, _I64, ctypes.c_int, _P, _SZ, _P]),
     'cb_trunk_front_f32': (ctypes.c_int, [_P, _I64, _I64, _I64, _P, _P, _P, _P, _P, _I64, _P, _I64, _P, _P, _I64, _P, _I64, ctypes.c_float,
                                           ctypes.c_uint64, ctypes.c_uint64, _P, _I64, _P]),
+    'cb_front_keep_x0_bytes': (_SZ, [_I64]),
+    'cb_front_keep_x_bytes': (_SZ, [_I64]),
+    'cb_trunk_front_words_f32': (ctypes.c_int, [_P, _I64, _I64, _I64, _P, _P, _P, _P, _P, _I64, _P, _I64, _P, _P, _I64, _P, _I64, ctypes.c_float,
+                                                ctypes.c_uint64, ctypes.c_uint64, _P, _I64, _P, _P, _P]),
+    'cb_gemm_tn_kdrop_supported': (ctypes.c_int, [_P, _I64, _P, _I64, _I64, _I64, _I64]),
+    'cb_gemm_tn_kdrop_f32': (ctypes.c_int, [_P, _I64, _P, _I64, _P, _P, _I64, _I64, _I64, ctypes.c_float, _P, _P, _SZ, _P]),
     'cb_gemm_tn_gdrop_supported': (ctypes.c_int, [_P, _I64, _P, _I64, _I64, _I64]),
     'cb_gemm_tn_gdrop_f32': (ctypes.c_int, [_P, _I64, _P, _I64, _P, _I64, _I64, _I64, ctypes.c_float, ctypes.c_uint64, _P, _I64, _P, _SZ, _P]),
     'cb_spmm_csr_lp_f32': (ctypes.c_int, [_G, _P, _I64, _I64, _P, _P, _I64, ctypes.c_float, _P, _P, _I64, _P]),
@@ -124,6 +130,8 @@
     'cb_gemm_tn_instage_workspace_bytes': (_SZ, [_I64, _I64]),
     'cb_gemm_tn_instage_f32': (ctypes.c_int, [_P, _P, _P, _P, _I64, _P, _P, _I64, _I64, ctypes.c_float, ctypes.c_uint64, ctypes.c_float, ctypes.c_uint64, _P, _I64,
                                               _P, _SZ, _P]),
+    'cb_gemm_tn_instage_words_f32': (ctypes.c_int, [_P, _P, _P, _P, _I64, _P, _P, _I64, _I64, ctypes.c_float, ctypes.c_uint64, ctypes.c_float, ctypes.c_uint64, _P,
+                                                    _I64, _P, _P, _P, _SZ, _P]),
     'cb_trunk_layer_bwd_fold_f32': (ctypes.c_int, [_P, _P, _P, _P, _I64, _I64, ctypes.c_float, ctypes.c_uint64, _P, _I64, ctypes.c_float, ctypes.c_float, _I32, _P, _P, _P,
                                                    _P, _P, _P, _SZ, _I32, _P, ctypes.c_float, _P, _P, _SZ, _P]),
     'cb_trunk_layer_bwd_rows_f32': (ctypes.c_int, [_P, _P, _I64, _P, _P, _P, _I64, ctypes.c_float, ctypes.c_uint64, _P, _I64, ctypes.c_float,
diff --git a/gnn-tail-generalization_amd/csrc/cb_front.hip b/gnn-tail-generalization_amd/csrc/cb_front.hip
--- a/gnn-tail-generalization_amd/csrc/cb_front.hip
+++ b/gnn-tail-generalization_amd/csrc/cb_front.hip
@@ -31,6 +31,8 @@
   const uint64_t* seed_dev;
   int64_t row0;
   int n_tiles;
+  unsigned long long* keep_x0;
+  uint32_t* keep_x;
 };
 
 template <int NS1, bool DROP>
@@ -108,7 +110,10 @@
       }
       *reinterpret_cast<float4*>(tile + row * LDX + 4 * c4) = make_float4(v[0], v[1], v[2], v[3]);
     }
-    if constexpr (DROP) aim_x(tile_id + (int)gridDim.x);
+    if constexpr (DROP) {
+      if (fa.keep_x) fa.keep_x[(int64_t)tile_id * 256 + t] = kx >> (32 - 4 * NV);
+      aim_x(tile_id + (int)gridDim.x);
+    }
     if (t < kTM) rs_tile[par][t] = rs_next;
     __syncthreads();
     f32x16 acc[2][2];
@@ -125,6 +130,9 @@
             tile[(32 * i + (reg & 3) + 8 * (reg >> 2) + 4 * lh) * kTLD + 64 * w + 32 * j + l31] = acc[i][j][reg];
     }
     __syncthreads();
+    if constexpr (DROP) {
+      if (fa.keep_x0) fa.keep_x0[((int64_t)tile_id * 4 + w) * 64 + lane] = k3;
+    }
 #pragma unroll 4
     for (int r = 0; r < 16; ++r) {
       const int row = 16 * w + r;
@@ -199,12 +207,24 @@
   return CB_OK;
 }
 
+extern "C" size_t cb_front_keep_x0_bytes(int64_t M) { return M > 0 ? (size_t)((M + kTM - 1) / kTM) * 4 * 64 * sizeof(uint64_t) : 0; }
+extern "C" size_t cb_front_keep_x_bytes(int64_t M) { return M > 0 ? (size_t)((M + kTM - 1) / kTM) * 256 * sizeof(uint32_t) : 0; }
+
 extern "C" int cb_trunk_front_f32(const float* x, int64_t ld_x, int64_t M, int64_t K, const void* image_in, const float* bias_in, const void* image_0,
                                   const float* rowscale, const float* addend, int64_t ld_add, float* x0, int64_t ld_x0, uint64_t* relu_bits,
                                   float* x0_drop, int64_t ld_drop, float* z0, int64_t ld_z, float drop_p, uint64_t seed_x, uint64_t seed_x0,
                                   const uint64_t* seed_dev, int64_t row0, void* stream) {
+  return cb_trunk_front_words_f32(x, ld_x, M, K, image_in, bias_in, image_0, rowscale, addend, ld_add, x0, ld_x0, relu_bits, x0_drop, ld_drop, z0, ld_z, drop_p,
+                                  seed_x, seed_x0, seed_dev, row0, nullptr, nullptr, stream);
+}
+
+extern "C" int cb_trunk_front_words_f32(const float* x, int64_t ld_x, int64_t M, int64_t K, const void* image_in, const float* bias_in, const void* image_0,
+                                        const float* rowscale, const float* addend, int64_t ld_add, float* x0, int64_t ld_x0, uint64_t* relu_bits,
+                                        float* x0_drop, int64_t ld_drop, float* z0, int64_t ld_z, float drop_p, uint64_t seed_x, uint64_t seed_x0,
+                                        const uint64_t* seed_dev, int64_t row0, uint64_t* keep_x0, uint32_t* keep_x, void* stream) {
   CB_CHECK_ARG(M >= 0 && cb_front_image_bytes(K) > 0 && drop_p >= 0.f && drop_p < 1.f && row0 >= 0, CB_E_INVALID,
                "cb_trunk_front_f32: bad size (K must be 64 or 128; hidden width 256) or p");
+  CB_CHECK_ARG((uintptr_t)keep_x0 % 8 == 0 && (uintptr_t)keep_x % 4 == 0, CB_E_INVALID, "cb_trunk_front_words_f32: misaligned keep words");
   CB_CHECK_ARG(M < ((int64_t)1 << 31) * kTM / 2, CB_E_RANGE, "cb_trunk_front_f32: size out of range");
   if (M == 0) return CB_OK;
   CB_CHECK_ARG(x && image_in && image_0 && x0 && z0, CB_E_INVALID, "cb_trunk_front_f32: null pointer");
@@ -218,6 +238,7 @@
   fa.keep_scale = 1.f / (1.f - drop_p);
   fa.seed_x = seed_x; fa.seed_x0 = seed_x0; fa.seed_dev = seed_dev; fa.row0 = row0;
   fa.n_tiles = (int)((M + kTM - 1) / kTM);
+  fa.keep_x0 = (unsigned long long*)keep_x0; fa.keep_x = keep_x;
   int dev = 0, n_cu = 0;
   if (hipGetDevice(&dev) != hipSuccess || hipDeviceGetAttribute(&n_cu, hipDeviceAttributeMultiprocessorCount, dev) != hipSuccess || n_cu <= 0) n_cu = 256;
   const int blocks = fa.n_tiles < 2 * n_cu ? fa.n_tiles : 2 * n_cu;
diff --git a/gnn-tail-generalization_amd/csrc/cb_gemm.hip b/gnn-tail-generalization_amd/csrc/cb_gemm.hip
--- a/gnn-tail-generalization_amd/csrc/cb_gemm.hip
+++ b/gnn-tail-generalization_amd/csrc/cb_gemm.hip
@@ -430,6 +430,15 @@
 extern "C" int cb_gemm_tn_instage_f32(const float* g, const float* mfold, const uint64_t* x0_bits, const float* X, int64_t ldx, float* C, float* colsum, int64_t M,
                                       int64_t K2, float g_drop_p, uint64_t g_seed, float x_drop_p, uint64_t x_seed, const uint64_t* seed_dev, int64_t row0, void* ws,
                                       size_t ws_bytes, void* stream) {
+  return cb_gemm_tn_instage_words_f32(g, mfold, x0_bits, X, ldx, C, colsum, M, K2, g_drop_p, g_seed, x_drop_p, x_seed, seed_dev, row0, nullptr, nullptr, ws, ws_bytes,
+                                      stream);
+}
+
+extern "C" int cb_gemm_tn_instage_words_f32(const float* g, const float* mfold, const uint64_t* x0_bits, const float* X, int64_t ldx, float* C, float* colsum,
+                                            int64_t M, int64_t K2, float g_drop_p, uint64_t g_seed, float x_drop_p, uint64_t x_seed, const uint64_t* seed_dev,
+                                            int64_t row0, const uint64_t* keep_x0, const uint32_t* keep_x, void* ws, size_t ws_bytes, void* stream) {
+  CB_CHECK_ARG((!keep_x0 == !keep_x) && (!keep_x0 || (K2 == 128 && (uintptr_t)keep_x0 % 8 == 0 && (uintptr_t)keep_x % 4 == 0)), CB_E_INVALID,
+               "cb_gemm_tn_instage_words_f32: keep words for both masks or for neither; 128 features; aligned words");
   CB_CHECK_ARG(M > 0 && K2 > 0 && g_drop_p > 0.f && g_drop_p < 1.f && x_drop_p > 0.f && x_drop_p < 1.f && row0 >= 0, CB_E_INVALID,
                "cb_gemm_tn_instage_f32: bad size or p (both dropouts must be active)");
   CB_CHECK_ARG(g && mfold && x0_bits && X && C && colsum && (uintptr_t)x0_bits % 8 == 0, CB_E_INVALID, "cb_gemm_tn_instage_f32: null or misaligned pointer");
@@ -439,8 +448,8 @@
   const int nsplit = instage_splits(M);
   int64_t rows_per_split = (M + nsplit - 1) / nsplit;
   rows_per_split = (rows_per_split + 31) / 32 * 32;
-  const DropSpec xd{dropout_threshold(x_drop_p), 1.f / (1.f - x_drop_p), x_seed, seed_dev, row0, K2};
-  const DropSpec gd{dropout_threshold(g_drop_p), 1.f / (1.f - g_drop_p), g_seed, seed_dev, row0, 256};
+  const DropSpec xd{dropout_threshold(x_drop_p), 1.f / (1.f - x_drop_p), x_seed, seed_dev, row0, K2, keep_x};
+  const DropSpec gd{dropout_threshold(g_drop_p), 1.f / (1.f - g_drop_p), g_seed, seed_dev, row0, 256, keep_x0};
   float* partial = (float*)ws;
   float* cs_partial = partial + (size_t)nsplit * 256 * K2;
   const int rc = launch_tn_instage(g, mfold, x0_bits, X, ldx, partial, cs_partial, M, K2, nsplit, rows_per_split, st, xd, gd);
@@ -493,3 +502,17 @@
   const DropSpec ad{dropout_threshold(a_drop_p), 1.f / (1.f - a_drop_p), a_seed, seed_dev, row0, K1};
   return launch_tn<2, 2>(A, lda, G, ldg, rowscale, C, M, K1, K2, (float*)ws, st, nullptr, &ad);
 }
+
+extern "C" int cb_gemm_tn_kdrop_supported(const float* A, int64_t lda, const float* G, int64_t ldg, int64_t M, int64_t K1, int64_t K2) {
+  return use_limb3() && K1 == 256 && K2 == 256 && M > 0 && tn_splits(M, 4) >= 256 && limb3_tn_eligible(A, lda, G, ldg, K1, K2) ? 1 : 0;
+}
+
+extern "C" int cb_gemm_tn_kdrop_f32(const float* A, int64_t lda, const float* G, int64_t ldg, const float* rowscale, float* C, int64_t M, int64_t K1, int64_t K2,
+                                    float a_drop_p, const uint64_t* keep_x0, void* ws, size_t ws_bytes, void* stream) {
+  CB_CHECK_ARG(M > 0 && a_drop_p > 0.f && a_drop_p < 1.f, CB_E_INVALID, "cb_gemm_tn_kdrop_f32: bad size or p");
+  CB_CHECK_ARG(A && G && C && keep_x0 && (uintptr_t)keep_x0 % 8 == 0 && lda >= K1 && ldg >= K2, CB_E_INVALID, "cb_gemm_tn_kdrop_f32: null / misaligned pointer or bad ld");
+  CB_CHECK_ARG(cb_gemm_tn_kdrop_supported(A, lda, G, ldg, M, K1, K2), CB_E_INVALID, "cb_gemm_tn_kdrop_f32: shape outside the eight-wavefront tile (cb_gemm_tn_kdrop_supported)");
+  CB_CHECK_ARG(ws && ws_bytes >= cb_gemm_tn_workspace_bytes(M, K1, K2), CB_E_WORKSPACE, "cb_gemm_tn_kdrop_f32: workspace too small");
+  const DropSpec ad{dropout_threshold(a_drop_p), 1.f / (1.f - a_drop_p), 0ull, nullptr, 0, K1, keep_x0};
+  return launch_tn<2, 2>(A, lda, G, ldg, rowscale, C, M, K1, K2, (float*)ws, (hipStream_t)stream, nullptr, &ad);
+}
diff --git a/gnn-tail-generalization_amd/csrc/cb_gemm_core.h b/gnn-tail-generalization_amd/csrc/cb_gemm_core.h
--- a/gnn-tail-generalization_amd/csrc/cb_gemm_core.h
+++ b/gnn-tail-generalization_amd/csrc/cb_gemm_core.h
@@ -16,6 +16,7 @@
   const uint64_t* seed_dev;
   int64_t row0;
   int64_t width;
+  const void* words = nullptr;
 };
 
 struct GemmEpilogue {
diff --git a/gnn-tail-generalization_amd/csrc/cb_gemm_limb.hip b/gnn-tail-generalization_amd/csrc/cb_gemm_limb.hip
--- a/gnn-tail-generalization_amd/csrc/cb_gemm_limb.hip
+++ b/gnn-tail-generalization_amd/csrc/cb_gemm_limb.hip
@@ -51,7 +51,7 @@
   nn_epilogue<WM, WN, WTN, OUT_BF16, EPI>(acc, reinterpret_cast<float*>(smem), Cv, ldc, m0, n0, M, N, ep, c_vec_ok, t);
 }
 
-template <int WM, int WN, bool SCALED, int WTN = 2, int PD = 1, bool GDROP = false, bool ADROP = false>
+template <int WM, int WN, bool SCALED, int WTN = 2, int PD = 1, bool GDROP = false, int ADROP = 0>
 __global__ void __launch_bounds__((LTile<WM, WN, WTN, PD>::NTHR), (LTile<WM, WN, WTN, PD>::MINW)) k_gemm_tn_l3(const float* __restrict__ A, int64_t lda,
                                                                                  const float* __restrict__ G, int64_t ldg,
                                                                                  const float* __restrict__ rowscale,
@@ -78,7 +78,8 @@
   oa.init(lda, K1 - i0, t);
   ob.init(ldg, K2 - j0, t);
   if constexpr (GDROP) ob.set_drop(gd, r_begin, r_end - r_begin, j0, t);
-  if constexpr (ADROP) oa.set_drop(gd, r_begin, r_end - r_begin, i0, t);
+  if constexpr (ADROP == kDropDraw) oa.set_drop(gd, r_begin, r_end - r_begin, i0, t);
+  if constexpr (ADROP == kDropWordsX0) oa.set_words(gd, r_begin, r_end - r_begin, t);
   const uint32_t aaddr[2] = {OA::frag_addr(wr * 64, lane), OA::frag_addr(wr * 64 + 32, lane)};
   uint32_t baddr[WTN];
 #pragma unroll
@@ -101,13 +102,14 @@
     }
 }
 
+template <bool WORDS>
 __global__ void __launch_bounds__(512, 2) k_gemm_tn_instage(const float* __restrict__ g, const float* __restrict__ mfold,
                                                             const unsigned long long* __restrict__ x0_bits, const float* __restrict__ X, int64_t ldx,
                                                             float* __restrict__ partial, float* __restrict__ cs_partial, int64_t M, int K2,
                                                             int64_t rows_per_split, int nsplit, DropSpec xd, DropSpec gd) {
   using T = LTile<4, 2, 2>;
-  using OA = ColOperandInStage<T::NTHR>;
-  using OB = ColOperand<T::BN, false, true, T::NTHR>;
+  using OA = ColOperandInStage<T::NTHR, WORDS>;
+  using OB = ColOperand<T::BN, false, WORDS ? kDropWordsX : kDropDraw, T::NTHR>;
   constexpr int K1 = 256;
   __shared__ __attribute__((aligned(16))) char smem[2 * (OA::BYTES + OB::BYTES)];
   const int split = blockIdx.x;
@@ -123,7 +125,8 @@
   oa.init(K1, K1, t);
   ob.init(ldx, K2, t);
   oa.set_stage(g, mfold, x0_bits + r_begin * 4, gd, r_begin, r_end - r_begin, t);
-  ob.set_drop(xd, r_begin, r_end - r_begin, 0, t);
+  if constexpr (WORDS) ob.set_words(xd, r_begin, r_end - r_begin, t);
+  else ob.set_drop(xd, r_begin, r_end - r_begin, 0, t);
   const uint32_t aaddr[2] = {OA::frag_addr(wr * 64, lane), OA::frag_addr(wr * 64 + 32, lane)};
   uint32_t baddr[2];
 #pragma unroll
@@ -158,8 +161,14 @@
 
 int launch_tn_instage(const float* g, const float* mfold, const uint64_t* x0_bits, const float* X, int64_t ldx, float* partial, float* cs_partial, int64_t M, int64_t K2,
                       int nsplit, int64_t rows_per_split, hipStream_t st, const DropSpec& xd, const DropSpec& gd) {
-  hipLaunchKernelGGL(k_gemm_tn_instage, dim3((unsigned)nsplit), dim3(512), 0, st, g, mfold, (const unsigned long long*)x0_bits, X, ldx, partial, cs_partial, M, (int)K2,
-                     rows_per_split, nsplit, xd, gd);
+  CB_CHECK_ARG(rows_per_split % 32 == 0 && (!gd.words == !xd.words) && (!gd.words || K2 == 128), CB_E_INVALID,
+               "input-stage TN contraction: slabs of whole 32-row groups; keep words for both masks or neither, 128 features");
+  if (gd.words)
+    hipLaunchKernelGGL(k_gemm_tn_instage<true>, dim3((unsigned)nsplit), dim3(512), 0, st, g, mfold, (const unsigned long long*)x0_bits, X, ldx, partial, cs_partial, M,
+                       (int)K2, rows_per_split, nsplit, xd, gd);
+  else
+    hipLaunchKernelGGL(k_gemm_tn_instage<false>, dim3((unsigned)nsplit), dim3(512), 0, st, g, mfold, (const unsigned long long*)x0_bits, X, ldx, partial, cs_partial, M,
+                       (int)K2, rows_per_split, nsplit, xd, gd);
   CB_LAUNCH_CHECK();
   return CB_OK;
 }
@@ -239,7 +248,8 @@
                      (int)K2, rows_per_split, tj, ti * tj, nsplit, gd.thresh ? gd : ad)
   if (gd.thresh) CB_TN_LAUNCH(false, true, false);
   else if (ad.thresh) {
-    if constexpr (WM == 2 && WN == 2 && WTN == 2) { if (rowscale) CB_TN_LAUNCH(true, false, true); else CB_TN_LAUNCH(false, false, true); }
+    if constexpr (WM == 2 && WN == 2 && WTN == 2) { if (rowscale) CB_TN_LAUNCH(true, false, kDropDraw); else CB_TN_LAUNCH(false, false, kDropDraw); }
+    if constexpr (WM == 4 && WN == 2 && WTN == 4) { if (rowscale) CB_TN_LAUNCH(true, false, kDropWordsX0); else CB_TN_LAUNCH(false, false, kDropWordsX0); }
   } else if (rowscale) CB_TN_LAUNCH(true, false, false);
   else CB_TN_LAUNCH(false, false, false);
 #undef CB_TN_LAUNCH
@@ -256,10 +266,12 @@
   CB_CHECK_ARG(!gd.thresh || (!rowscale && gd.width % 4 == 0 && !ad.thresh), CB_E_INVALID,
                "TN contraction: dropout of the G operand needs width %% 4 == 0, no row scale and no dropout of A");
   CB_CHECK_ARG(!ad.thresh || (ad.width % 4 == 0 && bm == 128), CB_E_INVALID, "TN contraction: dropout of the A operand needs width %% 4 == 0 and the 128-row tile");
+  CB_CHECK_ARG(!ad.words || (ad.thresh && K1 == 256 && K2 == 256 && nsplit >= 256 && rows_per_split % 32 == 0), CB_E_INVALID,
+               "TN contraction: keep words of the A operand exist for the 256 x 256 tile of eight wavefronts only (cb_gemm_tn_kdrop_supported)");
   if (bm == 64) launch_tn_l3_t<1, 4>(A, lda, G, ldg, rowscale, partial, M, K1, K2, nsplit, rows_per_split, st, gd, ad);
   else if (bm == 256) launch_tn_l3_t<4, 1>(A, lda, G, ldg, rowscale, partial, M, K1, K2, nsplit, rows_per_split, st, gd, ad);
   else {
-    if (!ad.thresh && !gd.thresh && K1 == 256 && K2 == 256 && nsplit >= 256) {
+    if ((!ad.thresh || ad.words) && !gd.thresh && K1 == 256 && K2 == 256 && nsplit >= 256) {
       launch_tn_l3_t<4, 2, 4>(A, lda, G, ldg, rowscale, partial, M, K1, K2, nsplit, rows_per_split, st, gd, ad);
       CB_LAUNCH_CHECK();
       return CB_OK;
diff --git a/gnn-tail-generalization_amd/csrc/cb_limb_core.h b/gnn-tail-generalization_amd/csrc/cb_limb_core.h
--- a/gnn-tail-generalization_amd/csrc/cb_limb_core.h
+++ b/gnn-tail-generalization_amd/csrc/cb_limb_core.h
@@ -153,7 +153,8 @@
   static __device__ __forceinline__ bf16x8 frag(const char* __restrict__ S, uint32_t addr, int plane) { return RowOperand<R>::frag(S, addr, plane); }
 };
 
-template <int C, bool SCALED, bool DROP = false, int NT = 256>
+constexpr int kDropDraw = 1, kDropWordsX0 = 2, kDropWordsX = 3;
+template <int C, bool SCALED, int DROP = 0, int NT = 256>
 struct ColOperand {
   static constexpr int ROWB = C * 2, PLANE = 16 * ROWB, BYTES = 3 * PLANE;
   static constexpr int TPR = C / 4, KPP = NT / TPR, NV = 16 / KPP;
@@ -180,6 +181,18 @@
     dwidth = d.width;
     dcol = j0 + (t % TPR) * 4;
   }
+  const void* kwords;
+  unsigned long long kword;
+  int kw;
+  __device__ __forceinline__ void set_words(const DropSpec& d, int64_t r_begin, int64_t total, int t) {
+    static_assert(DROP < kDropWordsX0 || (NT == 512 && C == (DROP == kDropWordsX0 ? 256 : 128)), "keep words: the front kernel's lane map");
+    dscale = d.scale;
+    drow = r_begin;
+    dtot = total;
+    kw = __builtin_amdgcn_readfirstlane(t / 64);
+    if constexpr (DROP == kDropWordsX0) kwords = reinterpret_cast<const unsigned long long*>(d.words) + (r_begin >> 4) * 64 + (t & 63);
+    else kwords = reinterpret_cast<const uint32_t*>(d.words) + (t & 255);
+  }
   __device__ __forceinline__ void init(int64_t ld, int cols_left, int t) {
     const int k = t / TPR, nq = t % TPR;
     cok = nq * 4 < cols_left;
@@ -194,18 +207,27 @@
     const bool kin = k < k_left;
     f[J] = *reinterpret_cast<const float4*>(base + (kin ? voff[J] : 0u));
     if constexpr (SCALED) sc[J] = kscale[kin ? k : 0];
+    if constexpr (DROP == kDropWordsX0 && J == NV - 1) kword = reinterpret_cast<const unsigned long long*>(kwords)[((dtot - k_left) >> 4) * 64];
+    if constexpr (DROP == kDropWordsX) kword = reinterpret_cast<const uint32_t*>(kwords)[((drow + (dtot - k_left)) >> 6) * 256];
   }
   template <int J>
   __device__ __forceinline__ void stage(const float4 (&f)[NV], char* __restrict__ S, int64_t k_left, int t) const {
     const bool live = cok && t / TPR + KPP * J < k_left;
     const float m = SCALED ? sc[SCALED ? J : 0] : 1.f;
     float v[4] = {live ? f[J].x * m : 0.f, live ? f[J].y * m : 0.f, live ? f[J].z * m : 0.f, live ? f[J].w * m : 0.f};
-    if constexpr (DROP) {
+    if constexpr (DROP == kDropDraw) {
       static_assert(!SCALED, "dropout of a row-scaled operand is not needed anywhere");
       float mk[4];
       keep4(dseed, ((drow + KPP * J + (dtot - k_left)) * dwidth + dcol) >> 2, dthresh, dscale, mk);
 #pragma unroll
       for (int i = 0; i < 4; ++i) v[i] = mul_rounded(v[i], mk[i]);
+    }
+    if constexpr (DROP >= kDropWordsX0) {
+      static_assert(!SCALED && (DROP == kDropWordsX0 || NV == 1), "keep words");
+      const int sh = DROP == kDropWordsX0 ? 4 * (kw + KPP * J) : 4 * ((int)(((drow + (dtot - k_left)) >> 3) & 7) + (kw >> 2));
+      const uint32_t nib = (uint32_t)(kword >> sh);
+#pragma unroll
+      for (int i = 0; i < 4; ++i) v[i] = mul_rounded(v[i], (nib >> i) & 1u ? dscale : 0.f);
     }
     uint2 pl[3];
     split4(v, pl);
@@ -226,7 +248,7 @@
   }
 };
 
-template <int NT = 512>
+template <int NT = 512, bool WORDS = false>
 struct ColOperandInStage {
   static constexpr int C = 256;
   static constexpr int ROWB = C * 2, PLANE = 16 * ROWB, BYTES = 3 * PLANE;
@@ -249,10 +271,13 @@
   int64_t drow, dtot, dwidth;
   int dcol, kw;
   float cs[4];
+  const unsigned long long* kwords;
+  unsigned long long kword;
   __device__ __forceinline__ void set_stage(const float* g, const float* mfold, const unsigned long long* bits_block, const DropSpec& d, int64_t r_begin, int64_t total,
                                             int t) {
     mdelta = mfold - g;
     bits = bits_block;
+    if constexpr (WORDS) kwords = reinterpret_cast<const unsigned long long*>(d.words) + (r_begin >> 4) * 64 + (t & 63);
     dseed = d.seed_dev ? d.seed + *d.seed_dev : d.seed;
     dthresh = d.thresh;
     dscale = d.scale;
@@ -281,13 +306,20 @@
     const unsigned long long* b = bits + ((dtot - k_left) + (kin ? k : 0)) * 4;
 #pragma unroll
     for (int i = 0; i < 4; ++i) bw[J][i] = b[i];
+    if constexpr (WORDS && J == NV - 1) kword = kwords[((dtot - k_left) >> 4) * 64];
   }
   template <int J>
   __device__ __forceinline__ void stage(const float4 (&f)[NV], char* __restrict__ S, int64_t k_left, int t) {
     const bool live = cok && kw + KPP * J < k_left;
     const int lane = t & 63;
     float mk[4];
-    keep4(dseed, ((drow + KPP * J + (dtot - k_left)) * dwidth + dcol) >> 2, dthresh, dscale, mk);
+    if constexpr (WORDS) {
+      const uint32_t nib = (uint32_t)(kword >> (4 * (kw + KPP * J)));
+#pragma unroll
+      for (int i = 0; i < 4; ++i) mk[i] = (nib >> i) & 1u ? dscale : 0.f;
+    } else {
+      keep4(dseed, ((drow + KPP * J + (dtot - k_left)) * dwidth + dcol) >> 2, dthresh, dscale, mk);
+    }
     const float gv[4] = {f[J].x, f[J].y, f[J].z, f[J].w}, mv[4] = {fm[J].x, fm[J].y, fm[J].z, fm[J].w};
     float v[4];
 #pragma unroll
diff --git a/gnn-tail-generalization_amd/gemm.py b/gnn-tail-generalization_amd/gemm.py
--- a/gnn-tail-generalization_amd/gemm.py
+++ b/gnn-tail-generalization_amd/gemm.py
@@ -139,7 +139,7 @@
     return (y, bits) if want_bits else y
 
 
-def trunk_front(x, w_in, b_in, w0, rowscale, addend, p, seed_x, seed_x0, row0=0, want_bits=False, want_drop=False, z_out=None):
+def trunk_front(x, w_in, b_in, w0, rowscale, addend, p, seed_x, seed_x0, row0=0, want_bits=False, want_drop=False, z_out=None, want_words=False):
     import ctypes
     from . import ops
     lib = _lib.load()
@@ -163,14 +163,41 @@
     z0 = z_out if z_out is not None else torch.empty((M, 256), dtype=torch.float32, device=dev)
     bits = torch.empty((M, 1, 4), dtype=torch.int64, device=dev) if want_bits else None
     xd = torch.empty((M, 256), dtype=torch.float32, device=dev) if want_drop else None
+    words = None
+    if want_words and p > 0 and M > 0:
+        words = (torch.empty((lib.cb_front_keep_x0_bytes(M) // 2048, 4, 64), dtype=torch.int64, device=dev),
+                 torch.empty((lib.cb_front_keep_x_bytes(M) // 1024, 256), dtype=torch.int32, device=dev))
     with torch.cuda.device(dev):
         _lib.check(lib.cb_front_image_f32(_lib.ptr(w_in), _ld(w_in), K, 1, _lib.ptr(img_in), nb_in, _lib.stream_ptr()), 'cb_front_image_f32')
         _lib.check(lib.cb_agg_gemm_image_f32(_lib.ptr(w0), _ld(w0), 256, 256, 0, _lib.ptr(img0), nb0, _lib.stream_ptr()), 'cb_agg_gemm_image_f32')
-        _lib.check(lib.cb_trunk_front_f32(_lib.ptr(x), _ld(x), M, K, _lib.ptr(img_in), _lib.ptr(b_in), _lib.ptr(img0), _lib.ptr(rowscale),
-                                          _lib.ptr(addend), _ld(addend) if addend is not None else 0, _lib.ptr(x0), 256, _lib.ptr(bits),
-                                          _lib.ptr(xd), 256, _lib.ptr(z0), 256, float(p), ctypes.c_uint64(seed_x), ctypes.c_uint64(seed_x0),
-                                          ops.seed_dev_ptr(), int(row0), _lib.stream_ptr()), 'cb_trunk_front_f32')
-    return x0, bits, xd, z0
+        _lib.check(lib.cb_trunk_front_words_f32(_lib.ptr(x), _ld(x), M, K, _lib.ptr(img_in), _lib.ptr(b_in), _lib.ptr(img0), _lib.ptr(rowscale),
+                                                _lib.ptr(addend), _ld(addend) if addend is not None else 0, _lib.ptr(x0), 256, _lib.ptr(bits),
+                                                _lib.ptr(xd), 256, _lib.ptr(z0), 256, float(p), ctypes.c_uint64(seed_x), ctypes.c_uint64(seed_x0),
+                                                ops.seed_dev_ptr(), int(row0), _lib.ptr(words[0]) if words else None,
+                                                _lib.ptr(words[1]) if words else None, _lib.stream_ptr()), 'cb_trunk_front_words_f32')
+    return (x0, bits, xd, z0, words) if want_words else (x0, bits, xd, z0)
+
+
+def mm_tn_kdrop_supported(M):
+    return bool(_lib.load().cb_gemm_tn_kdrop_supported(None, 256, None, 256, int(M), 256, 256))
+
+
+def mm_tn_kdrop(a, g, p, keep_x0, rowscale=None):
+    lib = _lib.load()
+    _lib.require_device(a, g, rowscale, keep_x0)
+    a, g = _rowmajor(a), _rowmajor(g)
+    M, K1 = a.shape
+    M2, K2 = g.shape
+    if (M != M2 or not (0.0 < p < 1.0) or keep_x0.dtype != torch.int64 or not keep_x0.is_contiguous() or keep_x0.numel() != (M + 63) // 64 * 256
+            or not lib.cb_gemm_tn_kdrop_supported(_lib.ptr(a), _ld(a), _lib.ptr(g), _ld(g), M, K1, K2)):
+        return None
+    out = torch.empty((K1, K2), dtype=torch.float32, device=a.device)
+    wsb = lib.cb_gemm_tn_workspace_bytes(M, K1, K2)
+    ws = torch.empty(max(wsb, 16), dtype=torch.uint8, device=a.device)
+    with torch.cuda.device(a.device):
+        _lib.check(lib.cb_gemm_tn_kdrop_f32(_lib.ptr(a), _ld(a), _lib.ptr(g), _ld(g), _lib.ptr(rowscale), _lib.ptr(out), M, K1, K2, float(p), _lib.ptr(keep_x0),
+                                            _lib.ptr(ws), wsb, _lib.stream_ptr()), 'cb_gemm_tn_kdrop_f32')
+    return out
 
 
 def mm_tn_adrop(a, g, p, a_seed, row0=0, rowscale=None):
@@ -218,7 +245,7 @@
             and bool(lib.cb_gemm_tn_instage_supported(_lib.ptr(g_like), _lib.ptr(g_like), _lib.ptr(x), _ld(x), int(M), int(x.shape[1]))))
 
 
-def mm_tn_instage(g, mfold, x0_bits, x, p_g, g_seed, p_x, x_seed, row0=0):
+def mm_tn_instage(g, mfold, x0_bits, x, p_g, g_seed, p_x, x_seed, row0=0, words=None):
     import ctypes
     from . import ops
     lib = _lib.load()
@@ -227,14 +254,21 @@
     if (tuple(g.shape) != (M, 256) or tuple(mfold.shape) != (M, 256) or not g.is_contiguous() or not mfold.is_contiguous() or x0_bits.numel() != 4 * M
             or not x0_bits.is_contiguous() or x0_bits.dtype != torch.int64):
         raise ValueError('mm_tn_instage: contiguous [M, 256] gradients, [M, 1, 4] int64 mask words and [M, F] features expected')
+    if words is not None:
+        n_tiles = (M + 63) // 64
+        if (K2 != 128 or words[0].dtype != torch.int64 or words[0].numel() != 256 * n_tiles or words[1].dtype != torch.int32 or words[1].numel() != 256 * n_tiles
+                or not words[0].is_contiguous() or not words[1].is_contiguous()):
+            raise ValueError('mm_tn_instage: keep words of a 128-feature front on the same rows expected')
+        _lib.require_device(*words)
     out = torch.empty((256, K2), dtype=torch.float32, device=g.device)
     colsum = torch.empty(256, dtype=torch.float32, device=g.device)
     wsb = lib.cb_gemm_tn_instage_workspace_bytes(M, K2)
     ws = torch.empty(max(wsb, 16), dtype=torch.uint8, device=g.device)
     with torch.cuda.device(g.device):
-        _lib.check(lib.cb_gemm_tn_instage_f32(_lib.ptr(g), _lib.ptr(mfold), _lib.ptr(x0_bits), _lib.ptr(x), _ld(x), _lib.ptr(out), _lib.ptr(colsum), M, K2,
-                                              float(p_g), ctypes.c_uint64(g_seed), float(p_x), ctypes.c_uint64(x_seed), ops.seed_dev_ptr(), int(row0),
-                                              _lib.ptr(ws), wsb, _lib.stream_ptr()), 'cb_gemm_tn_instage_f32')
+        _lib.check(lib.cb_gemm_tn_instage_words_f32(_lib.ptr(g), _lib.ptr(mfold), _lib.ptr(x0_bits), _lib.ptr(x), _ld(x), _lib.ptr(out), _lib.ptr(colsum), M, K2,
+                                                    float(p_g), ctypes.c_uint64(g_seed), float(p_x), ctypes.c_uint64(x_seed), ops.seed_dev_ptr(), int(row0),
+                                                    _lib.ptr(words[0]) if words else None, _lib.ptr(words[1]) if words else None,
+                                                    _lib.ptr(ws), wsb, _lib.stream_ptr()), 'cb_gemm_tn_instage_words_f32')
     return out, colsum
 
 
diff --git a/gnn-tail-generalization_amd/trunk.py b/gnn-tail-generalization_amd/trunk.py
--- a/gnn-tail-generalization_amd/trunk.py
+++ b/gnn-tail-generalization_amd/trunk.py
@@ -458,6 +458,7 @@
         self.row0, self.a = int(getattr(graph, 'row_offset', 0)), graph.norm_out
         self.bwd = bool(cfg.track) and any(ctx.needs_input_grad)
         self.z_ready = self.out_head = self.out_rows = self.h_last = self.h_below = None
+        self.words, self.kdrop = None, False
 
     def run(self):
         cfg, graph = self.cfg, self.graph
@@ -484,13 +485,18 @@
     def _front(self):
         c, x, w_in, b_in, row0, bwd, p, seeds = self.cfg, self.x, self.w_in, self.b_in, self.row0, self.bwd, self.cfg.p, self.cfg.seeds
         indrop = p > 0 and _switch('CB_TRUNK_INDROP', '1') != '0'
-        copy = _switch('CB_TRUNK_X0_COPY', '1') == '1'
+        copy_sw = _switch('CB_TRUNK_X0_COPY', None)
+        copy = copy_sw in (None, '1')
         if (indrop or p == 0) and not c.agg_bf16 and c.L >= 1 and w_in.shape[0] == 256 and _switch('CB_TRUNK_FRONT', '1') != '0':
             w0, _b0, le0 = self.layers[0]
-            fr = gemm.trunk_front(x, w_in, b_in, w0, self.a, le0, p, seeds[0], seeds[1], row0, want_bits=bwd, want_drop=bwd and p > 0 and copy,
-                                  z_out=_exchanged(self.graph, x.shape[0]) if hasattr(self.graph, 'part') else None)
+            sharded = hasattr(self.graph, 'part')
+            kdrop = bwd and p > 0 and copy_sw is None and not sharded and gemm.mm_tn_kdrop_supported(x.shape[0])
+            fr = gemm.trunk_front(x, w_in, b_in, w0, self.a, le0, p, seeds[0], seeds[1], row0, want_bits=bwd, want_drop=bwd and p > 0 and copy and not kdrop,
+                                  z_out=_exchanged(self.graph, x.shape[0]) if sharded else None, want_words=bwd)
             if fr is not None:
-                x0, x0_bits, cur, z_front = fr
+                x0, x0_bits, cur, z_front = fr[:4]
+                self.words = fr[4] if bwd else None
+                self.kdrop = kdrop and self.words is not None
                 return (x, x0, x0_bits, x0 if p == 0 else cur, z_front), True
         if indrop:
             wb = bwd and w_in.shape[0] == 256
@@ -609,10 +615,11 @@
     def forward(ctx, graph, cfg, x, w_in, b_in, w_out, b_out, *layer_params):
         f = _Forward(ctx, graph, cfg, x, w_in, b_in, w_out, b_out, layer_params)
         out = f.run()
-        ctx.graph, ctx.cfg, ctx.row0, ctx.indrop, ctx.n_layer_params = graph, cfg, f.row0, f.indrop, len(layer_params)
+        ctx.graph, ctx.cfg, ctx.row0, ctx.indrop, ctx.n_layer_params, ctx.kdrop = graph, cfg, f.row0, f.indrop, len(layer_params), f.kdrop
         if f.bwd:
+            kx0, kx = f.words if f.words is not None else (None, None)
             _save(ctx, xd=f.xd, x0=f.x0, w_in=w_in, w_out=w_out, saved_in=f.saved_in, saved_bits=f.saved_bits, layer_params=layer_params,
-                  h_last=f.h_last, h_below=f.h_below, x0_bits=f.x0_bits)
+                  h_last=f.h_last, h_below=f.h_below, x0_bits=f.x0_bits, keep_x0=kx0, keep_x=kx)
             ro = f.ro
             ctx.saved_rows = SavedRows('S0' if (ro.plan is not None or ro.sharded is not None) else 'all',
                                        'absent' if f.h_last is not None else 'S1' if (ro.plan is not None and ro.below is not None) else 'all')
@@ -644,6 +651,7 @@
         self.xd, self.x0, self.w_in, self.w_out = sv['xd'], sv['x0'], sv['w_in'], sv['w_out']
         self.saved_in, self.saved_bits, self.x0_bits = sv['saved_in'], sv['saved_bits'], sv['x0_bits']
         self.h_last, self.h_below = sv['h_last'], sv['h_below']
+        self.words, self.kdrop = (sv['keep_x0'], sv['keep_x']) if sv['keep_x0'] is not None else None, ctx.kdrop
         self.lp, self.where = _layers(sv['layer_params']), ctx.saved_rows
         self.a, self.bnorm = graph.norm_out, graph.norm_in
         self.need = ctx.needs_input_grad
@@ -680,7 +688,13 @@
     def _dw(self, l, x_in, gz):
         if x_in is not None:
             return gemm.mm_tn(x_in, gz, rowscale=self.a)
-        return _dw_regen(self.x0, gz, self.p, self.seed(1), self.row0, self.a)
+        dw = gemm.mm_tn_kdrop(self.x0, gz, self.p, self.words[0], rowscale=self.a) if self.kdrop else None
+        return dw if dw is not None else _dw_regen(self.x0, gz, self.p, self.seed(1), self.row0, self.a)
+
+    def _x_in(self, l):
+        if l == 0 and self.saved_in[0] is None and self.kdrop:
+            return ops._dropout_raw(self.x0, self.p, self.seed(1), self.row0 * self.x0.shape[1])
+        return self.saved_in[l]
 
     def _second(self, below, g_above, pos_above=None):
         if not self.residual or g_above is None:
@@ -780,7 +794,7 @@
         del t
         if self.need_w(l):
             x_agg = (self.h_last if (self.where.x_below == 'absent' and l == self.L - 1) else self.h_below if (self.h_below is not None and l == self.L - 2)
-                     else fwd_j.spmm(self.saved_in[l], col_scale=self.a))
+                     else fwd_j.spmm(self._x_in(l), col_scale=self.a))
             self.grads_layers[3 * l] = gemm.mm_tn(x_agg, gr)
         return None, g_new, fused
 
@@ -792,7 +806,7 @@
         if self.need_w(l):
             if dst is not None:
                 on_s1 = self.where.x_below == 'S1' and l == self.L - 1
-                x_rows = self.saved_in[l] if on_s1 else ops.gather_rows_by_index(self.saved_in[l], dst.idx)
+                x_rows = self.saved_in[l] if on_s1 else ops.gather_rows_by_index(self._x_in(l), dst.idx)
                 self.grads_layers[3 * l] = gemm.mm_tn(x_rows, gz, rowscale=dst.a)
             else:
                 self.grads_layers[3 * l] = self._dw(l, self.saved_in[l], gz)
@@ -849,7 +863,7 @@
         fwd_j = plan.fwd[j] if (level is not None and j < len(plan.fwd)) else None
         source_side = ((self.where.x_below == 'absent' and l == L - 1) or (self.h_below is not None and l == L - 2)
                        or (T.rowsparse_loss_side and fwd_j is not None and not self.need_le(l)
-                           and not (self.need_w(l) and self.saved_in[l] is None)
+                           and not (self.need_w(l) and self.saved_in[l] is None and not self.kdrop)
                            and not (self.where.x_below == 'S1' and l == L - 1)))
         if source_side:
             _gz, g_new, fused = self._layer_source_side(l, c.gr, level, fwd_j)
@@ -912,7 +926,8 @@
         graph, p, need, xd, row0 = self.graph, self.p, self.need, self.xd, self.row0
         g, c.g = c.g, None
         if self.mfold is not None:
-            d_w_in, d_b_in = gemm.mm_tn_instage(g, self.mfold, self.x0_bits, xd, p, self.seed(1), p, self.seeds[0], row0)
+            d_w_in, d_b_in = gemm.mm_tn_instage(g, self.mfold, self.x0_bits, xd, p, self.seed(1), p, self.seeds[0], row0,
+                                                words=self.words if xd.shape[1] == 128 else None)
             del g
             self.gx0 = self.g_mix = self.mfold = None
             graph.instage_folds = getattr(graph, 'instage_folds', 0) + 1
diff --git a/include/coldbrew_hip.h b/include/coldbrew_hip.h
--- a/include/coldbrew_hip.h
+++ b/include/coldbrew_hip.h
@@ -197,6 +197,12 @@
                        const float* rowscale, const float* addend, int64_t ld_add, float* x0, int64_t ld_x0, uint64_t* relu_bits, float* x0_drop,
                        int64_t ld_drop, float* z0, int64_t ld_z, float drop_p, uint64_t seed_x, uint64_t seed_x0, const uint64_t* seed_dev,
                        int64_t row0, void* stream);
+size_t cb_front_keep_x0_bytes(int64_t M);
+size_t cb_front_keep_x_bytes(int64_t M);
+int cb_trunk_front_words_f32(const float* x, int64_t ld_x, int64_t M, int64_t K, const void* image_in, const float* bias_in, const void* image_0,
+                             const float* rowscale, const float* addend, int64_t ld_add, float* x0, int64_t ld_x0, uint64_t* relu_bits, float* x0_drop,
+                             int64_t ld_drop, float* z0, int64_t ld_z, float drop_p, uint64_t seed_x, uint64_t seed_x0, const uint64_t* seed_dev,
+                             int64_t row0, uint64_t* keep_x0, uint32_t* keep_x, void* stream);
 
 int cb_spmm_csr_weighted_f32(const int32_t* rowptr, const int32_t* col, const float* w, int64_t N, int64_t E, const float* h, int64_t ld_h,
                              int64_t d, const float* row_scale, const float* bias, int relu, float* out, int64_t ld_out, void* stream);
@@ -222,6 +228,12 @@
 int cb_gemm_tn_instage_f32(const float* g, const float* mfold, const uint64_t* x0_bits, const float* X, int64_t ldx, float* C, float* colsum, int64_t M, int64_t K2,
                            float g_drop_p, uint64_t g_seed, float x_drop_p, uint64_t x_seed, const uint64_t* seed_dev, int64_t row0, void* ws, size_t ws_bytes,
                            void* stream);
+int cb_gemm_tn_instage_words_f32(const float* g, const float* mfold, const uint64_t* x0_bits, const float* X, int64_t ldx, float* C, float* colsum, int64_t M,
+                                 int64_t K2, float g_drop_p, uint64_t g_seed, float x_drop_p, uint64_t x_seed, const uint64_t* seed_dev, int64_t row0,
+                                 const uint64_t* keep_x0, const uint32_t* keep_x, void* ws, size_t ws_bytes, void* stream);
+int cb_gemm_tn_kdrop_supported(const float* A, int64_t lda, const float* G, int64_t ldg, int64_t M, int64_t K1, int64_t K2);
+int cb_gemm_tn_kdrop_f32(const float* A, int64_t lda, const float* G, int64_t ldg, const float* rowscale, float* C, int64_t M, int64_t K1, int64_t K2,
+                         float a_drop_p, const uint64_t* keep_x0, void* ws, size_t ws_bytes, void* stream);
 
 int cb_spmm_gemm_store_rows_f32(const cb_csr_view* g, const float* h, int64_t ld_h, int64_t d, const float* col_scale, float* out, int64_t ld_out,
                                 const void* image, const float* g_rowscale, const float* bias, const int64_t* row_ids, const cb_trunk_store* store,
```
